# leggedrobotics/open3d_slam

Hardware: NVIDIA H100
Metric: scan-to-map ICP registrations/sec (64x1024-pt clouds) (higher is better)
Workload: dtype f64

## Files before the change

### include/b2s.h

```cpp
#ifndef B2S_H_
#define B2S_H_

#include <stddef.h>
#include <stdint.h>

#ifdef __cplusplus
extern "C" {
#endif
#if defined(__GNUC__)
#pragma GCC visibility push(default)
#endif

#define B2S_OK 0
#define B2S_E_INVALID (-1)
#define B2S_E_CUDA (-2)
#define B2S_E_EMPTY (-3)
#define B2S_E_NO_NORMALS (-4)
#define B2S_E_CAPACITY (-5)
#define B2S_E_UNSUPPORTED (-6)

typedef struct b2s_handle b2s_handle;
typedef struct b2s_cloud b2s_cloud;
typedef struct b2s_submap b2s_submap;

// ... 15 lines not shown
  int32_t knn;
  double knn_radius;
  double rel_fitness, rel_rmse;
} b2s_icp_params;

typedef struct b2s_scan_params {
  double voxel_size;
  double downsampling_ratio;
  uint32_t seed;
  b2s_cropper map_builder_cropper;
  b2s_cropper scan_matcher_cropper;
} b2s_scan_params;

typedef struct b2s_config {
  b2s_icp_params icp;
  b2s_scan_params scan;
  double map_voxel_size;
  double dense_voxel_size;
  double nn_cell_size;
  int32_t icp_cluster_ctas;
  int32_t reserved_;
} b2s_config;

typedef struct b2s_result {
  double T[16];
  double fitness;
  double inlier_rmse;
  int32_t n_corr;
  int32_t iters;
} b2s_result;

void b2s_default_config(b2s_config* cfg);

int32_t b2s_create(const b2s_config* cfg, int32_t device, void* cuda_stream_or_null, b2s_handle** out);
void b2s_destroy(b2s_handle* h);
int32_t b2s_set_config(b2s_handle* h, const b2s_config* cfg);
int32_t b2s_synchronize(b2s_handle* h);
const char* b2s_last_error(void);
const char* b2s_version(void);
int32_t b2s_device_count(void);
int64_t b2s_launch_count(const b2s_handle* h);
int64_t b2s_graph_capture_count(const b2s_handle* h);

#define B2S_PROFILE_KINDS 8
int32_t b2s_profile_enable(b2s_handle* h, int32_t on);
int32_t b2s_profile_read(b2s_handle* h, double* ms_by_kind, int64_t* count_by_kind, int32_t n_kinds);
int32_t b2s_debug_icp_clocks(b2s_handle* h, int32_t enable, long long* out_1024);

int32_t b2s_cloud_create(b2s_handle* h, b2s_cloud** out);
void b2s_cloud_destroy(b2s_cloud* c);
int32_t b2s_cloud_upload_f64(b2s_handle* h, b2s_cloud* c, const double* xyz, const double* normals_or_null, size_t n);
int32_t b2s_cloud_upload_f32(b2s_handle* h, b2s_cloud* c, const void* xyz, size_t n, size_t stride_bytes);
int32_t b2s_cloud_size(b2s_handle* h, const b2s_cloud* c, size_t* n, int32_t* has_normals);
int32_t b2s_cloud_download(b2s_handle* h, const b2s_cloud* c, double* xyz, double* normals_or_null, size_t capacity, size_t* n);
int32_t b2s_cloud_copy(b2s_handle* h, const b2s_cloud* src, b2s_cloud* dst);

int32_t b2s_crop(b2s_handle* h, const b2s_cloud* in, const b2s_cropper* cropper, b2s_cloud* out);
int32_t b2s_voxel_down_sample(b2s_handle* h, const b2s_cloud* in, double voxel_size, b2s_cloud* out);
int32_t b2s_estimate_normals(b2s_handle* h, b2s_cloud* cloud, int32_t knn, double radius);
int32_t b2s_debug_estimate_normals(b2s_handle* h, b2s_cloud* cloud, int32_t knn, double radius, double cell_hint, const int32_t* flags_host,
                                   int32_t with_prior, double* rec_out, int32_t* path_out, double* sel_out);
int32_t b2s_random_down_sample(b2s_handle* h, const b2s_cloud* in, double ratio, uint32_t seed, b2s_cloud* out);
int32_t b2s_transform(b2s_handle* h, const b2s_cloud* in, const double T[16], b2s_cloud* out);
int32_t b2s_process_scan(b2s_handle* h, const b2s_cloud* raw, b2s_cloud* merge, b2s_cloud* match);
int32_t b2s_register(b2s_handle* h, const b2s_cloud* source, const b2s_cloud* target, const double init[16], b2s_result* out);
int32_t b2s_register_batch(b2s_handle* h, int32_t n, const b2s_cloud* const* sources, const b2s_cloud* const* targets,
                           const double* inits , b2s_result* out );
int32_t b2s_nearest_neighbors(b2s_handle* h, const b2s_cloud* queries, const b2s_cloud* target, double max_correspondence_distance,
                              const double T_or_null[16], int32_t* index_out, double* d2_out_or_null, size_t capacity, size_t* n_queries);
int32_t b2s_register_host(b2s_handle* h, const double* src_xyz, size_t n_src, const double* tgt_xyz, const double* tgt_normals,
                          size_t n_tgt, const double init[16], b2s_result* out);

int32_t b2s_submap_create(b2s_handle* h, size_t capacity_points, b2s_submap** out);
void b2s_submap_destroy(b2s_submap* sm);
int32_t b2s_submap_insert(b2s_handle* h, b2s_submap* sm, const b2s_cloud* preprocessed_scan, const double map_to_sensor[16]);
typedef struct b2s_carving_params {
  double voxel_size;
  double max_raytracing_length;
  double truncation_distance;
  double min_dot_product_with_normal;
  double neighborhood_radius_dense_map;
} b2s_carving_params;
int32_t b2s_submap_carve(b2s_handle* h, b2s_submap* sm, const b2s_cloud* raw_scan, const double map_to_sensor[16],
                         const double cropper_pose[16], const b2s_carving_params* params, size_t* n_removed);
int32_t b2s_undistort(b2s_handle* h, const b2s_cloud* in, const double linear_velocity[3], const double angular_velocity_rpy[3],
                      double scan_duration, int32_t is_spinning_clockwise, b2s_cloud* out);
int32_t b2s_overlap(b2s_handle* h, const b2s_cloud* source, const b2s_cloud* target, const double source_to_target[16], double voxel_size,
                    int32_t min_points_per_voxel, b2s_cloud* source_overlap, b2s_cloud* target_overlap);
int32_t b2s_information_matrix(b2s_handle* h, const b2s_cloud* source, const b2s_cloud* target, double max_correspondence_distance,
                               const double transformation[16], double info_out[36]);
int32_t b2s_dense_carve(b2s_handle* h, b2s_submap* sm, const b2s_cloud* scan, const double sensor_position[3],
                        const b2s_carving_params* params, size_t* n_removed);
int32_t b2s_submap_insert_dense(b2s_handle* h, b2s_submap* sm, const b2s_cloud* raw_scan, const double map_to_sensor[16],
                                const b2s_cropper* dense_cropper);
int32_t b2s_dense_query(b2s_handle* h, const b2s_submap* sm, const b2s_cloud* points, int32_t* counts, double* means_xyz, size_t capacity);
int32_t b2s_dense_remove(b2s_handle* h, b2s_submap* sm, const b2s_cloud* points);
int32_t b2s_dense_size(b2s_handle* h, const b2s_submap* sm, size_t* n_voxels);
int32_t b2s_dense_clear(b2s_handle* h, b2s_submap* sm);
int32_t b2s_submap_transform(b2s_handle* h, b2s_submap* sm, const double T[16]);
int32_t b2s_cloud_transform_inplace(b2s_handle* h, b2s_cloud* c, const double T[16]);
int32_t b2s_submap_size(b2s_handle* h, const b2s_submap* sm, size_t* n);
int32_t b2s_submap_download(b2s_handle* h, const b2s_submap* sm, double* xyz, double* normals, size_t capacity, size_t* n);
int32_t b2s_submap_to_cloud(b2s_handle* h, const b2s_submap* sm, b2s_cloud* out);
int32_t b2s_submap_dense_download(b2s_handle* h, const b2s_submap* sm, double* xyz, double* normals, int32_t* keys, size_t capacity,
                                  size_t* n);
int32_t b2s_submap_set_cloud(b2s_handle* h, b2s_submap* sm, const b2s_cloud* cloud);
int32_t b2s_register_to_submap(b2s_handle* h, const b2s_cloud* scan, const b2s_submap* sm, const double map_to_sensor[16],
                               const double init[16], b2s_result* out);

int32_t b2s_submap_set_pose(b2s_handle* h, b2s_submap* sm, const double map_to_sensor[16]);
int32_t b2s_submap_get_pose(b2s_handle* h, const b2s_submap* sm, double map_to_sensor[16]);
int32_t b2s_mapper_step_async(b2s_handle* h, b2s_submap* sm, const b2s_cloud* raw_scan, const double odometry_motion[16],
                              double min_refinement_fitness, int32_t ignore_min_fitness, int32_t slot );
int32_t b2s_scan_result_fetch(b2s_handle* h, int32_t slot, b2s_result* out);
int32_t b2s_mapper_step_host(b2s_handle* h, b2s_submap* sm, const void* xyz_f32, size_t n, size_t stride_bytes,
                             const double odometry_motion[16], double min_refinement_fitness, int32_t ignore_min_fitness,
                             b2s_result* out);
int32_t b2s_mapper_step_host_async(b2s_handle* h, b2s_submap* sm, const void* xyz_f32, size_t n, size_t stride_bytes,
                                   const double odometry_motion[16], double min_refinement_fitness, int32_t ignore_min_fitness,
                                   b2s_result* out_pinned);
int32_t b2s_mapper_graph_enable(b2s_handle* h, b2s_submap* sm, size_t raw_capacity_points, double min_refinement_fitness,
                                int32_t ignore_min_fitness, b2s_cloud** staging_out);

typedef struct b2s_mapper_options {
  double min_movement_between_mapping_steps;
  int32_t carve_enabled;
  int32_t carve_every_n_scans;
  b2s_carving_params carving;
  int32_t dense_enabled;
  int32_t dense_carve_every_n_scans;
  b2s_carving_params dense_carving;
  b2s_cropper dense_cropper;
} b2s_mapper_options;
void b2s_default_mapper_options(b2s_mapper_options* o);
int32_t b2s_submap_set_mapper_options(b2s_handle* h, b2s_submap* sm, const b2s_mapper_options* o);
typedef struct b2s_mapper_counters {
  int64_t steps;
  int64_t accepted;
  int64_t inserted_map;
  int64_t inserted_dense;
  int64_t carve_runs;
  int64_t carved_points_total;
  int64_t dense_carve_runs;
  int64_t carved_voxels_total;
} b2s_mapper_counters;
int32_t b2s_submap_get_mapper_counters(b2s_handle* h, const b2s_submap* sm, b2s_mapper_counters* out);

int32_t b2s_submap_set_initial_map(b2s_handle* h, b2s_submap* sm, const b2s_cloud* cloud, double map_voxel_size);
int32_t b2s_submap_set_initial_transform(b2s_handle* h, b2s_submap* sm, const double map_to_sensor[16]);
int32_t b2s_submap_set_merge_scans(b2s_handle* h, b2s_submap* sm, int32_t on);
int32_t b2s_debug_nn_index(b2s_handle* h, double origin_cell[4], int32_t dims_n[5], int32_t* cell_start, size_t cap_cells, int32_t* orig,
                           size_t cap_pts);
int32_t b2s_debug_submap_bbox(b2s_handle* h, const b2s_submap* sm, double box[6]);

typedef struct b2s_global_localization_params {
  double x_min, x_max, y_min, y_max;
  double step;
  double z0, z_step;
  int32_t n_z;
  int32_t n_yaw;
  double yaw0, yaw_step;
  double roll, pitch;
  double score_voxel;
  int32_t n_candidates;
  int32_t reserved_;
  double nms_distance, nms_yaw;
} b2s_global_localization_params;
void b2s_default_global_localization_params(b2s_global_localization_params* p);
typedef struct b2s_global_localization_candidate {
  double T_hypothesis[16];
  int32_t hypothesis;
  int32_t hits;
  b2s_result icp;
} b2s_global_localization_candidate;
typedef struct b2s_global_localization_result {
  double T[16];
  double fitness, inlier_rmse;
  double runner_up_fitness;
  int64_t n_hypotheses;
  int32_t found;
  int32_t winner_rank;
  int32_t n_query;
  int32_t n_candidates;
} b2s_global_localization_result;
int32_t b2s_submap_global_localization(b2s_handle* h, const b2s_submap* sm, const b2s_cloud* raw_scan, const b2s_global_localization_params* p,
                                       double min_refinement_fitness, b2s_global_localization_candidate* candidates_or_null, int32_t capacity,
                                       b2s_global_localization_result* out);
int32_t b2s_debug_global_localization_scores(b2s_handle* h, const b2s_submap* sm, const b2s_cloud* raw_scan, const b2s_global_localization_params* p,
                                             int32_t* hits_out, size_t capacity, size_t* n_hypotheses, double* query_out_or_null,
                                             size_t query_capacity, size_t* n_query);

int32_t b2s_submaps_global_localization(b2s_handle* h, const b2s_submap* const* sms, int32_t n_submaps, const double* centers,
                                        const b2s_cloud* raw_scan, const b2s_global_localization_params* p, double min_refinement_fitness,
                                        b2s_global_localization_candidate* candidates_or_null, int32_t capacity,
                                        int32_t* candidate_submaps_or_null, b2s_global_localization_result* out, int32_t* winner_submap);
int32_t b2s_debug_submaps_global_localization_scores(b2s_handle* h, const b2s_submap* const* sms, int32_t n_submaps, const b2s_cloud* raw_scan,
                                                     const b2s_global_localization_params* p, int32_t* hits_out, size_t capacity,
                                                     size_t* n_hypotheses, double* query_out_or_null, size_t query_capacity, size_t* n_query);

typedef struct b2s_odometry_params {
  b2s_icp_params icp;
  double voxel_size;
  double downsampling_ratio;
  uint32_t seed;
  b2s_cropper cropper;
  double min_fitness;
  int32_t buffer_size;
} b2s_odometry_params;
void b2s_default_odometry_params(b2s_odometry_params* p);
enum { B2S_ODOM_INIT = 0, B2S_ODOM_OK = 1, B2S_ODOM_FAILED = 2, B2S_ODOM_FAILED_KEPT_PREV = 3 };
typedef struct b2s_odometry b2s_odometry;
int32_t b2s_odometry_create(b2s_handle* h, const b2s_odometry_params* p, size_t capacity_points, b2s_odometry** out);
void b2s_odometry_destroy(b2s_odometry* od);
int32_t b2s_odometry_set_params(b2s_handle* h, b2s_odometry* od, const b2s_odometry_params* p);
int32_t b2s_odometry_set_initial_transform(b2s_handle* h, b2s_odometry* od, const double T[16]);
int32_t b2s_odometry_step_async(b2s_handle* h, b2s_odometry* od, const b2s_cloud* raw, int64_t t, int32_t slot);
typedef struct b2s_odometry_result {
  b2s_result registration;
  double odom_to_range_sensor[16];
  int32_t outcome;
  int32_t n_preprocessed;
} b2s_odometry_result;
int32_t b2s_odometry_result_fetch(b2s_handle* h, b2s_odometry* od, int32_t slot, b2s_odometry_result* out);
int32_t b2s_odometry_lookup(b2s_handle* h, const b2s_odometry* od, int64_t t, double T[16], int32_t* has);
int32_t b2s_odometry_preprocessed(b2s_handle* h, const b2s_odometry* od, b2s_cloud* out);

typedef struct b2s_slam_result {
  b2s_odometry_result odometry;
  b2s_result mapper;
  int32_t odom_used;
  int32_t mapper_accepted;
} b2s_slam_result;
int32_t b2s_slam_step_async(b2s_handle* h, b2s_submap* sm, b2s_odometry* od, const b2s_cloud* raw, int64_t t, double min_refinement_fitness,
                            int32_t ignore_min_fitness, int32_t slot);
int32_t b2s_slam_result_fetch(b2s_handle* h, b2s_odometry* od, int32_t slot, b2s_slam_result* out);
int32_t b2s_slam_step_host_async(b2s_handle* h, b2s_submap* sm, b2s_odometry* od, const void* xyz_f32, size_t n, size_t stride_bytes, int64_t t,
                                 double min_refinement_fitness, int32_t ignore_min_fitness, b2s_slam_result* out_pinned);
int32_t b2s_slam_graph_enable(b2s_handle* h, b2s_odometry* od, size_t raw_capacity_points, b2s_cloud** staging_out);

typedef struct b2s_motion_compensation_params {
  int32_t enabled;
  int32_t spinning_clockwise;
  double scan_duration;
  int32_t num_poses_velocity_estimation;
} b2s_motion_compensation_params;
void b2s_default_motion_compensation_params(b2s_motion_compensation_params* p);
int32_t b2s_odometry_set_motion_compensation(b2s_handle* h, b2s_odometry* od, const b2s_motion_compensation_params* p);
int32_t b2s_slam_map_pose_push(b2s_handle* h, b2s_odometry* od, int64_t t, const double T[16]);
int32_t b2s_slam_map_lookup(b2s_handle* h, const b2s_odometry* od, int64_t t, double T[16], int32_t* has);
typedef struct b2s_motion_compensation_result {
  double odometry_linear_velocity[3];
  double odometry_angular_velocity_rpy[3];
  double map_linear_velocity[3];
  double map_angular_velocity_rpy[3];
  int32_t odometry_applied;
  int32_t map_applied;
} b2s_motion_compensation_result;
int32_t b2s_slam_motion_fetch(b2s_handle* h, b2s_odometry* od, int32_t slot, b2s_motion_compensation_result* out);
int32_t b2s_slam_undistorted(b2s_handle* h, const b2s_odometry* od, b2s_cloud* odo_out, b2s_cloud* map_out);

#define B2S_VOXEL_MAP_LAYERS 4
typedef struct b2s_voxel_map b2s_voxel_map;
int32_t b2s_voxel_map_create(b2s_handle* h, const double voxel_size[3], size_t capacity_voxels, b2s_voxel_map** out);
void b2s_voxel_map_destroy(b2s_voxel_map* vm);
int32_t b2s_voxel_map_clear(b2s_handle* h, b2s_voxel_map* vm);
int32_t b2s_voxel_map_insert_cloud(b2s_handle* h, b2s_voxel_map* vm, int32_t layer, const b2s_cloud* cloud);
int32_t b2s_voxel_map_size(b2s_handle* h, const b2s_voxel_map* vm, size_t* n_voxels);
int32_t b2s_voxel_map_has_voxel(b2s_handle* h, const b2s_voxel_map* vm, const b2s_cloud* points, const double T_or_null[16],
                                int32_t* flags_or_null, size_t capacity, size_t* n_hits);
int32_t b2s_voxel_map_indices_in_voxel(b2s_handle* h, const b2s_voxel_map* vm, int32_t layer, const b2s_cloud* points, int32_t* offsets,
                                       size_t offsets_capacity, int32_t* indices, size_t indices_capacity, size_t* n_indices);
int32_t b2s_mapper_processed_scan(b2s_handle* h, b2s_cloud* merge_out, b2s_cloud* match_out);

#define B2S_FEATURE_DIM 33
#define B2S_FEATURE_MAX_KNN 128
typedef struct b2s_feature b2s_feature;
int32_t b2s_feature_create(b2s_handle* h, b2s_feature** out);
void b2s_feature_destroy(b2s_feature* f);
int32_t b2s_feature_size(b2s_handle* h, const b2s_feature* f, size_t* n);
int32_t b2s_feature_download(b2s_handle* h, const b2s_feature* f, double* data, size_t capacity_points, size_t* n);
int32_t b2s_feature_upload(b2s_handle* h, b2s_feature* f, const double* data, size_t n);
int32_t b2s_compute_fpfh(b2s_handle* h, const b2s_cloud* cloud, double radius, int32_t knn, b2s_feature* feature);

typedef struct b2s_feature_params {
  double feature_voxel_size;
  double normal_estimation_radius;
  int32_t normal_knn;
  double feature_radius;
  int32_t feature_knn;
} b2s_feature_params;
void b2s_default_feature_params(b2s_feature_params* p);
int32_t b2s_submap_compute_features(b2s_handle* h, b2s_submap* sm, const b2s_feature_params* params, b2s_cloud* sparse_out,
                                    b2s_feature* feature_out);

#define B2S_RANSAC_MAX_N 8
typedef struct b2s_ransac_params {
  int32_t mutual_filter;
  int32_t ransac_n;
  double max_correspondence_distance;
  double checker_distance;
  double checker_edge_length;
  int64_t max_iteration;
  double confidence;
  uint64_t seed;
} b2s_ransac_params;
void b2s_default_ransac_params(b2s_ransac_params* p);
// ... 183 lines not shown
```

### open3d_slam_b200/_lib.py

```python
from __future__ import annotations

import ctypes as C
import os

_HERE = os.path.dirname(os.path.abspath(__file__))
LIB_PATH = os.environ.get("B2S_LIB") or os.path.join(_HERE, "libb2s.so")

OK, E_INVALID, E_CUDA, E_EMPTY, E_NO_NORMALS, E_CAPACITY, E_UNSUPPORTED = 0, -1, -2, -3, -4, -5, -6
CROP_NONE, CROP_MAX_RADIUS, CROP_MIN_RADIUS, CROP_MINMAX_RADIUS, CROP_CYLINDER = 0, 1, 2, 3, 4
CROPPER_NAMES = {"None": 0, "MaxRadius": 1, "MinRadius": 2, "MinMaxRadius": 3, "Cylinder": 4}
REG_POINT_TO_PLANE, REG_POINT_TO_POINT, REG_GENERALIZED = 0, 1, 2


class Cropper(C.Structure):
    _fields_ = [("kind", C.c_int32), ("invert", C.c_int32), ("rmin", C.c_double), ("rmax", C.c_double),
                ("zmin", C.c_double), ("zmax", C.c_double), ("center", C.c_double * 3)]


class IcpParams(C.Structure):
    _fields_ = [("reg_type", C.c_int32), ("max_iter", C.c_int32), ("max_corr_dist", C.c_double), ("knn", C.c_int32),
                ("knn_radius", C.c_double), ("rel_fitness", C.c_double), ("rel_rmse", C.c_double)]


class ScanParams(C.Structure):
# ... 6 lines not shown
                ("nn_cell_size", C.c_double), ("icp_cluster_ctas", C.c_int32), ("reserved_", C.c_int32)]


class Result(C.Structure):
    _fields_ = [("T", C.c_double * 16), ("fitness", C.c_double), ("inlier_rmse", C.c_double), ("n_corr", C.c_int32),
                ("iters", C.c_int32)]


class CarvingParams(C.Structure):
    _fields_ = [("voxel_size", C.c_double), ("max_raytracing_length", C.c_double), ("truncation_distance", C.c_double),
                ("min_dot_product_with_normal", C.c_double), ("neighborhood_radius_dense_map", C.c_double)]


class MapperOptions(C.Structure):
    _fields_ = [("min_movement_between_mapping_steps", C.c_double), ("carve_enabled", C.c_int32), ("carve_every_n_scans", C.c_int32),
                ("carving", CarvingParams), ("dense_enabled", C.c_int32), ("dense_carve_every_n_scans", C.c_int32),
                ("dense_carving", CarvingParams), ("dense_cropper", Cropper)]


class FeatureParams(C.Structure):
    _fields_ = [("feature_voxel_size", C.c_double), ("normal_estimation_radius", C.c_double), ("normal_knn", C.c_int32),
                ("feature_radius", C.c_double), ("feature_knn", C.c_int32)]


class RansacParams(C.Structure):
    _fields_ = [("mutual_filter", C.c_int32), ("ransac_n", C.c_int32), ("max_correspondence_distance", C.c_double),
                ("checker_distance", C.c_double), ("checker_edge_length", C.c_double), ("max_iteration", C.c_int64),
                ("confidence", C.c_double), ("seed", C.c_uint64)]


class RansacResult(C.Structure):
    _fields_ = [("result", Result), ("hypotheses", C.c_int64), ("validations", C.c_int64), ("best_hypothesis", C.c_int64), ("n_feature_corr", C.c_int32),
                ("used_mutual", C.c_int32)]


class OdometryParams(C.Structure):
    _fields_ = [("icp", IcpParams), ("voxel_size", C.c_double), ("downsampling_ratio", C.c_double), ("seed", C.c_uint32), ("cropper", Cropper),
                ("min_fitness", C.c_double), ("buffer_size", C.c_int32)]


class OdometryResult(C.Structure):
    _fields_ = [("registration", Result), ("odom_to_range_sensor", C.c_double * 16), ("outcome", C.c_int32), ("n_preprocessed", C.c_int32)]


class SlamResult(C.Structure):
    _fields_ = [("odometry", OdometryResult), ("mapper", Result), ("odom_used", C.c_int32), ("mapper_accepted", C.c_int32)]


class MotionCompensationParams(C.Structure):
    _fields_ = [("enabled", C.c_int32), ("spinning_clockwise", C.c_int32), ("scan_duration", C.c_double),
                ("num_poses_velocity_estimation", C.c_int32)]


class MotionCompensationResult(C.Structure):
    _fields_ = [("odometry_linear_velocity", C.c_double * 3), ("odometry_angular_velocity_rpy", C.c_double * 3),
                ("map_linear_velocity", C.c_double * 3), ("map_angular_velocity_rpy", C.c_double * 3),
                ("odometry_applied", C.c_int32), ("map_applied", C.c_int32)]


ODOM_INIT, ODOM_OK, ODOM_FAILED, ODOM_FAILED_KEPT_PREV = 0, 1, 2, 3


class OdometryConstraintParams(C.Structure):
    _fields_ = [("map_voxel_size", C.c_double), ("voxel_if_zero", C.c_double), ("overlap_factor", C.c_double), ("icp_factor", C.c_double),
                ("min_points_per_voxel", C.c_int32), ("refine", C.c_int32), ("max_iter", C.c_int32), ("rel_fitness", C.c_double),
                ("rel_rmse", C.c_double)]


class OdometryConstraint(C.Structure):
    _fields_ = [("T", C.c_double * 16), ("information", C.c_double * 36), ("n_source_overlap", C.c_int64), ("n_target_overlap", C.c_int64),
                ("refined", C.c_int32), ("icp", Result)]


class LoopClosureRefinementParams(C.Structure):
    _fields_ = [("map_voxel_size", C.c_double), ("voxel_if_zero", C.c_double), ("overlap_factor", C.c_double), ("min_points_per_voxel", C.c_int32),
                ("max_iter", C.c_int32), ("max_corr_dist", C.c_double), ("rel_fitness", C.c_double), ("rel_rmse", C.c_double),
                ("min_refinement_fitness", C.c_double), ("reg_type", C.c_int32)]


class LoopClosureRefinement(C.Structure):
    _fields_ = [("icp", Result), ("information", C.c_double * 36), ("n_source_overlap", C.c_int64), ("n_target_overlap", C.c_int64),
                ("accepted", C.c_int32)]


class PoseGraphEdge(C.Structure):
    _fields_ = [("source", C.c_int32), ("target", C.c_int32), ("uncertain", C.c_int32), ("reserved_", C.c_int32), ("T", C.c_double * 16),
                ("information", C.c_double * 36)]


class GlobalOptimizationParams(C.Structure):
    _fields_ = [("max_correspondence_distance", C.c_double), ("edge_prune_threshold", C.c_double), ("preference_loop_closure", C.c_double),
                ("reference_node", C.c_int32), ("max_iteration", C.c_int32), ("min_relative_increment", C.c_double),
                ("min_relative_residual_increment", C.c_double), ("min_right_term", C.c_double), ("min_residual", C.c_double),
                ("max_iteration_lm", C.c_int32), ("reserved_", C.c_int32), ("upper_scale_factor", C.c_double), ("lower_scale_factor", C.c_double)]


class GlobalOptimizationStats(C.Structure):
    _fields_ = [("valid", C.c_int32), ("n_edges", C.c_int32), ("outer_iterations", C.c_int32), ("lm_tries", C.c_int32), ("accepted_steps", C.c_int32),
                ("stop_reason", C.c_int32), ("initial_residual", C.c_double), ("final_residual", C.c_double), ("final_lambda", C.c_double)]


LM_STOP_REASONS = ["none", "right_term", "relative_increment", "relative_residual_increment", "max_iteration_lm", "residual", "max_iteration"]


class MapperCounters(C.Structure):
    _fields_ = [(n, C.c_int64) for n in ("steps", "accepted", "inserted_map", "inserted_dense", "carve_runs", "carved_points_total",
                                         "dense_carve_runs", "carved_voxels_total")]


class GlobalLocalizationParams(C.Structure):
    _fields_ = [("x_min", C.c_double), ("x_max", C.c_double), ("y_min", C.c_double), ("y_max", C.c_double), ("step", C.c_double),
                ("z0", C.c_double), ("z_step", C.c_double), ("n_z", C.c_int32), ("n_yaw", C.c_int32), ("yaw0", C.c_double),
                ("yaw_step", C.c_double), ("roll", C.c_double), ("pitch", C.c_double), ("score_voxel", C.c_double),
                ("n_candidates", C.c_int32), ("reserved_", C.c_int32), ("nms_distance", C.c_double), ("nms_yaw", C.c_double)]


class GlobalLocalizationCandidate(C.Structure):
    _fields_ = [("T_hypothesis", C.c_double * 16), ("hypothesis", C.c_int32), ("hits", C.c_int32), ("icp", Result)]


class GlobalLocalizationResult(C.Structure):
    _fields_ = [("T", C.c_double * 16), ("fitness", C.c_double), ("inlier_rmse", C.c_double), ("runner_up_fitness", C.c_double),
                ("n_hypotheses", C.c_int64), ("found", C.c_int32), ("winner_rank", C.c_int32), ("n_query", C.c_int32),
                ("n_candidates", C.c_int32)]


SYMBOLS = [
    "b2s_default_config", "b2s_create", "b2s_destroy", "b2s_set_config", "b2s_synchronize", "b2s_last_error", "b2s_version",
    "b2s_device_count", "b2s_launch_count", "b2s_graph_capture_count", "b2s_cloud_create", "b2s_cloud_destroy", "b2s_cloud_upload_f64", "b2s_cloud_upload_f32",
    "b2s_cloud_size", "b2s_cloud_download", "b2s_cloud_copy", "b2s_crop", "b2s_voxel_down_sample", "b2s_estimate_normals",
    "b2s_random_down_sample", "b2s_transform", "b2s_process_scan", "b2s_register", "b2s_register_batch", "b2s_register_host",
    "b2s_submap_create", "b2s_submap_destroy", "b2s_submap_insert", "b2s_submap_insert_dense", "b2s_submap_size", "b2s_submap_download",
    "b2s_submap_dense_download", "b2s_submap_set_cloud", "b2s_register_to_submap", "b2s_submap_set_pose", "b2s_submap_get_pose",
    "b2s_mapper_step_async", "b2s_scan_result_fetch", "b2s_profile_enable", "b2s_profile_read", "b2s_mapper_graph_enable", "b2s_debug_icp_clocks",
    "b2s_mapper_step_host", "b2s_mapper_step_host_async", "b2s_submap_carve", "b2s_overlap", "b2s_information_matrix", "b2s_undistort",
    "b2s_dense_query", "b2s_dense_remove", "b2s_dense_size", "b2s_dense_clear", "b2s_dense_carve", "b2s_submap_transform",
    "b2s_default_mapper_options", "b2s_submap_set_mapper_options", "b2s_submap_get_mapper_counters",
    "b2s_voxel_map_create", "b2s_voxel_map_destroy", "b2s_voxel_map_clear", "b2s_voxel_map_insert_cloud", "b2s_voxel_map_size",
    "b2s_voxel_map_has_voxel", "b2s_voxel_map_indices_in_voxel", "b2s_mapper_processed_scan",
    "b2s_cloud_export_device", "b2s_cloud_import_device", "b2s_submap_to_cloud", "b2s_nearest_neighbors",
    "b2s_feature_create", "b2s_feature_destroy", "b2s_feature_size", "b2s_feature_download", "b2s_feature_upload", "b2s_compute_fpfh",
    "b2s_default_feature_params", "b2s_submap_compute_features",
    "b2s_default_ransac_params", "b2s_ransac_feature_matching", "b2s_feature_correspondences",
    "b2s_default_odometry_params", "b2s_odometry_create", "b2s_odometry_destroy", "b2s_odometry_set_params", "b2s_odometry_set_initial_transform",
    "b2s_odometry_step_async", "b2s_odometry_result_fetch", "b2s_odometry_lookup", "b2s_odometry_preprocessed",
    "b2s_slam_step_async", "b2s_slam_result_fetch", "b2s_slam_step_host_async", "b2s_slam_graph_enable",
    "b2s_default_motion_compensation_params", "b2s_odometry_set_motion_compensation", "b2s_slam_map_pose_push", "b2s_slam_map_lookup",
    "b2s_slam_motion_fetch", "b2s_slam_undistorted",
    "b2s_default_odometry_constraint_params", "b2s_submap_odometry_constraints",
    "b2s_default_loop_closure_refinement_params", "b2s_submap_loop_closure_refinement",
    "b2s_default_global_optimization_params", "b2s_global_optimization", "b2s_cloud_transform_inplace",
    "b2s_submap_set_initial_map", "b2s_submap_set_initial_transform", "b2s_submap_set_merge_scans", "b2s_debug_nn_index",
    "b2s_assemble_map", "b2s_assemble_colored_map", "b2s_debug_pose_graph_solve", "b2s_debug_pose_graph_linearize",
    "b2s_debug_estimate_normals", "b2s_debug_submap_bbox",
    "b2s_default_global_localization_params", "b2s_submap_global_localization", "b2s_debug_global_localization_scores",
    "b2s_submaps_global_localization", "b2s_debug_submaps_global_localization_scores",
    "b2s_assemble_dense_maps",
    "b2s_submaps_export_state", "b2s_submap_import_state", "b2s_odometry_export_state", "b2s_odometry_import_state",
]
FEATURE_DIM, FEATURE_MAX_KNN = 33, 128
ASSEMBLY_MAX_SUBMAPS = 65535
STATE_VERSION, STATE_BYTE_ORDER = 1, 0x0102030405060708
STATE_MAGIC_SUBMAP, STATE_MAGIC_ODOMETRY = 0x314D425553533242, 0x314D4F444F533242
STATE_HEADER_BYTES, STATE_MSTATE_WORDS, STATE_POSE_SLOTS = 256, 32, 8
STATE_W_MAGIC, STATE_W_VERSION, STATE_W_BYTE_ORDER, STATE_W_TOTAL_BYTES, STATE_W_MAP_VOXEL, STATE_W_N_SECTIONS, STATE_W_SECTIONS, STATE_W_PARAMS = \
    0, 1, 2, 3, 4, 5, 6, 20
STATE_SUBMAP_SECTIONS = ["pose", "options", "mstate", "bbox", "map_xyz", "map_normals", "vnext", "pstamp", "wflag", "dups", "wlist", "voxels",
                         "dense_used", "dense"]
STATE_SUBMAP_PARAMS = ["capacity", "vcap", "stage_cap", "dense_cap", "dense_voxel", "flags", "dn", "n_voxels", "n_dups", "n_wlist", "n_dense"]
STATE_ODOMETRY_SECTIONS = ["params", "motion", "state", "ring_times", "ring_poses", "map_times", "map_poses", "prev_xyz", "prev_normals"]
STATE_ODOMETRY_PARAMS = ["capacity", "buffer_size", "n_prev", "host_step", "has_t", "last_t"]
STATE_F_HAS_NORMALS, STATE_F_NO_NORMALS, STATE_F_MERGE_SCANS, STATE_F_DENSE_HAS_NORMALS = 1, 2, 4, 8


class StateVoxelRecord(C.Structure):
    _fields_ = [("key", C.c_uint64), ("slot", C.c_int32), ("head", C.c_int32), ("stamp", C.c_int32), ("reserved_", C.c_int32)]


class StateDenseRecord(C.Structure):
    _fields_ = [("key", C.c_uint64), ("sum", C.c_double * 6), ("slot", C.c_int32), ("count", C.c_int32)]
PROFILE_KINDS = ["icp", "normals", "radix_sort", "nn_grid_build", "voxel", "fuse", "select", "crop"]

_lib = None


class B2SError(RuntimeError):

    def __init__(self, code, msg):
        super().__init__(f"b2s error {code}: {msg}")
        self.code = code


def lib():
    global _lib
    if _lib is None:
        if not os.path.exists(LIB_PATH):
            raise ImportError(f"{LIB_PATH} is missing: build it with __graft_entry__.build() (nvcc, sm_90a). "
                              "There is no CPU fallback.")
        L = C.CDLL(LIB_PATH)
        L.b2s_last_error.restype = C.c_char_p
        L.b2s_version.restype = C.c_char_p
        L.b2s_launch_count.restype = C.c_int64
        L.b2s_launch_count.argtypes = [C.c_void_p]
        L.b2s_graph_capture_count.restype = C.c_int64
        L.b2s_graph_capture_count.argtypes = [C.c_void_p]
        L.b2s_destroy.restype = None
        L.b2s_cloud_destroy.restype = None
        L.b2s_submap_destroy.restype = None
        L.b2s_default_config.restype = None
        L.b2s_default_mapper_options.restype = None
        L.b2s_default_feature_params.restype = None
        L.b2s_default_ransac_params.restype = None
        L.b2s_destroy.argtypes = [C.c_void_p]
        L.b2s_cloud_destroy.argtypes = [C.c_void_p]
        L.b2s_submap_destroy.argtypes = [C.c_void_p]
        L.b2s_voxel_map_destroy.restype = None
        L.b2s_voxel_map_destroy.argtypes = [C.c_void_p]
        L.b2s_feature_destroy.restype = None
        L.b2s_feature_destroy.argtypes = [C.c_void_p]
        L.b2s_odometry_destroy.restype = None
        L.b2s_odometry_destroy.argtypes = [C.c_void_p]
        L.b2s_default_odometry_params.restype = None
        L.b2s_default_motion_compensation_params.restype = None
        L.b2s_default_odometry_constraint_params.restype = None
        L.b2s_default_loop_closure_refinement_params.restype = None
        L.b2s_default_global_optimization_params.restype = None
        L.b2s_default_global_localization_params.restype = None
        _lib = L
    return _lib


def check(code):
    if code != OK:
        raise B2SError(code, lib().b2s_last_error().decode("utf-8", "replace"))
```

### open3d_slam_b200/csrc/c_api.cu

```cuda
#include <math.h>
#include <stdlib.h>

#include "common.cuh"

using namespace b2s;

namespace b2s {
int32_t pose_to_device(b2s_handle* h, const double* T, double* dst);
int32_t dense_to_cloud(b2s_handle* h, b2s_submap* sm, double* d_xyz, int32_t* d_keys, int32_t* d_out_n);

__global__ void f32_to_f64_kernel(const unsigned char* __restrict__ src, size_t stride, int n, double* __restrict__ dst) {
  pdl_wait();
  for (int i = blockIdx.x * blockDim.x + threadIdx.x; i < n; i += gridDim.x * blockDim.x) {
    const float* p = reinterpret_cast<const float*>(src + (size_t)i * stride);
    dst[3 * i] = (double)p[0]; dst[3 * i + 1] = (double)p[1]; dst[3 * i + 2] = (double)p[2];
  }
}

__global__ void write_i32_kernel(int32_t* p, int32_t v) {
  pdl_wait(); *p = v; }

__global__ void empty_check_kernel(const int32_t* a, const int32_t* b, uint32_t* status) {
  pdl_wait();
  if (*a <= 0 || *b <= 0) atomicOr(status, ST_EMPTY);
}

__global__ void compose_kernel(const double* __restrict__ A, const double* __restrict__ B, double* __restrict__ C, const int32_t* __restrict__ ms) {
  pdl_wait();
  const int i = threadIdx.x >> 2, j = threadIdx.x & 3;
  const bool hold = ms[MS_NEWINIT] || ms[MS_IGNODOM];
  if (threadIdx.x < 16) {
    double s = 0.0;
    for (int k = 0; k < 4; k++) s += A[4 * i + k] * B[4 * k + j];
    C[4 * i + j] = hold ? A[4 * i + j] : s;
  }
}

struct GateArgs {
  double min_fitness, min_move;
  int ignore_fitness, carve_on, carve_n, dense_on, dcarve_n, merge_on;
};
__global__ void mapper_gate_kernel(const b2s_result* __restrict__ res, GateArgs a, double* pose, int32_t* ms, const int32_t* __restrict__ map_n,
                                   b2s_result* slots, const int32_t* __restrict__ gstate) {
  pdl_wait();
  if (threadIdx.x != 0) return;
  const int init = ms[MS_NEWINIT];
  ms[MS_NEWINIT] = 0; ms[MS_IGNODOM] = init; ms[MS_INITSTEP] = init;
  const bool accepted = init || a.ignore_fitness || !(res->fitness < a.min_fitness);
  if (accepted && !init) for (int i = 0; i < 16; i++) pose[i] = res->T[i];
  bool insert = accepted && !init && a.merge_on;
  if (insert && a.min_move > 0.0) {
    const double* L = pose + 5 * 16;
    const double* P = pose;
    double it[3], m[3];
    for (int i = 0; i < 3; i++) it[i] = -(L[i] * L[3] + L[4 + i] * L[7] + L[8 + i] * L[11]);
    for (int i = 0; i < 3; i++) m[i] = (L[i] * P[3] + L[4 + i] * P[7] + L[8 + i] * P[11]) + it[i];
    const double moved = sqrt(m[0] * m[0] + m[1] * m[1] + m[2] * m[2]);
    insert = !(moved < a.min_move);
  }
  const bool carve = insert && a.carve_on && a.carve_n > 0 && *map_n > 0 && (ms[MS_NINS] % a.carve_n == 1);
  const bool dense = accepted && a.dense_on;
  const bool dcarve = dense && a.dcarve_n > 0 && (ms[MS_NDENSE] % a.dcarve_n == 1);
  ms[MS_ACCEPT] = accepted; ms[MS_INSERT] = insert; ms[MS_CARVE] = carve; ms[MS_DENSE] = dense; ms[MS_DCARVE] = dcarve;
  ms[MS_NSTEPS] += 1; ms[MS_NACCEPT] += accepted ? 1 : 0;
  if (slots) slots[gstate[1]] = *res;
}
__global__ void mapper_post_kernel(int32_t* ms) {
  pdl_wait();
  if (threadIdx.x == 0 && ms[MS_DENSE]) ms[MS_NDENSE] += 1;
}

double nn_cell(const b2s_handle* h, double max_corr) {
  if (h->cfg.nn_cell_size > 0.0) return h->cfg.nn_cell_size;
  return max_corr * 0.25;
}

int32_t check_icp_params(const b2s_icp_params& p) {
  B2S_REQUIRE(p.reg_type == B2S_REG_POINT_TO_PLANE || p.reg_type == B2S_REG_POINT_TO_POINT || p.reg_type == B2S_REG_GENERALIZED,
              B2S_E_UNSUPPORTED, "unknown registration type %d", (int)p.reg_type);
  B2S_REQUIRE(p.max_corr_dist > 0.0, B2S_E_INVALID, "[RegistrationICP] Invalid max_correspondence_distance.");
  B2S_REQUIRE(p.max_iter >= 0, B2S_E_INVALID, "max_iter must be >= 0");
  return B2S_OK;
}

size_t icp_work_bytes(size_t n) { return (n + 1) * 24 + (n + 1) * 4 + 16; }

void fill_problem(IcpProblem* P, const b2s_icp_params& icp, const b2s_cloud* src, const GridIndex* g, const b2s_cloud* tgt, const double* init_host,
                  const double* init_dev, double* work, b2s_result* out_dev) {
  memset(P, 0, sizeof(*P));
  P->src_xyz = src->xyz.as<double>();
  P->src_n = src->dn.as<int32_t>();
  P->ghdr = g->hdr.as<GridHeader>();
  P->cell_start = grid_starts(g);
  P->tgt_pts = g->pts.as<double>();
  P->tgt_nrm = tgt->has_normals ? tgt->nrm.as<double>() : nullptr;
  P->work_xyz = work;
  P->work_prev = reinterpret_cast<int32_t*>(work + 3 * (src->n_max + 1));
  P->init_dev = init_dev;
  if (init_host) memcpy(P->init, init_host, 128);
  P->max_corr = icp.max_corr_dist;
  P->rel_fitness = icp.rel_fitness;
  P->rel_rmse = icp.rel_rmse;
  P->max_iter = icp.max_iter;
  P->src_n_max = (int32_t)src->n_max;
  P->estimator = icp.reg_type;
  P->src_nrm = src->has_normals ? src->nrm.as<double>() : nullptr;
  P->gicp_eps = 1e-3;
  P->out = out_dev;
}

int32_t preprocess_scan(b2s_handle* h, const b2s_cloud* raw, const b2s_cropper& cropper, double voxel_size, double ratio, uint32_t seed,
                        const b2s_icp_params& icp, b2s_cloud* t0, b2s_cloud* out) {
  b2s_cropper c0 = cropper;
  c0.center[0] = c0.center[1] = c0.center[2] = 0.0;
  CropDev wide = make_crop(&c0);
  const bool has_crop = c0.kind != B2S_CROP_NONE || c0.invert;
  if (voxel_size > 0.0) B2S_TRY(op_voxel_down_sample(h, raw, has_crop ? &wide : nullptr, voxel_size, t0));
  else if (has_crop) B2S_TRY(op_crop(h, raw, wide, t0));
  else B2S_TRY(op_voxel_down_sample(h, raw, nullptr, 0.0, t0));
  static const double cell_factor = getenv("B2S_NORMALS_CELL_FACTOR") ? atof(getenv("B2S_NORMALS_CELL_FACTOR")) : 4.0;
  const double cell_hint = voxel_size > 0.0 ? cell_factor * voxel_size : 0.0;
  if (ratio < 1.0) {
    B2S_REQUIRE(ratio >= 0.0, B2S_E_INVALID, "[RandomDownSample] sampling_ratio must be in [0, 1]");
    B2S_TRY(select_flags(h, t0, ratio, seed));
    B2S_TRY(op_estimate_normals(h, t0, icp.knn, icp.knn_radius, cell_hint, h->flags.as<int32_t>()));
    B2S_TRY(select_compact(h, t0, ratio, out));
  } else {
    B2S_TRY(op_estimate_normals(h, t0, icp.knn, icp.knn_radius, cell_hint));
    B2S_TRY(op_random_down_sample(h, t0, ratio, seed, out));
  }
  return B2S_OK;
}

int32_t process_scan_impl(b2s_handle* h, const b2s_cloud* raw, b2s_cloud* merge, b2s_cloud* match) {
  const b2s_scan_params& sp = h->cfg.scan;
  B2S_TRY(preprocess_scan(h, raw, sp.map_builder_cropper, sp.voxel_size, sp.downsampling_ratio, sp.seed, h->cfg.icp, h->t0.get(), merge));
  b2s_cropper c1 = sp.scan_matcher_cropper;
  c1.center[0] = c1.center[1] = c1.center[2] = 0.0;
  B2S_TRY(op_crop(h, merge, make_crop(&c1), match));
  launch_pdl(empty_check_kernel, 1, 1, 0, h->stream, merge->dn.as<int32_t>(), match->dn.as<int32_t>(), h->status.as<uint32_t>());
  h->launches++;
  return B2S_OK;
}

__global__ void graph_begin_kernel(const double* __restrict__ ring, int32_t* gstate, double* __restrict__ odom) {
  pdl_wait();
  const int step = gstate[0];
  if (threadIdx.x < 16) odom[threadIdx.x] = ring[(step & 63) * 16 + threadIdx.x];
  __syncthreads();
  if (threadIdx.x == 0) { gstate[0] = step + 1; gstate[1] = step & 255; }
}

int32_t mapper_chain_tail(b2s_handle* h, b2s_submap* sm, const b2s_cloud* raw_scan, const b2s_cloud* merge, const b2s_result* res,
                          double min_fitness, int ignore_fitness, b2s_result* slots, const int32_t* gstate) {
  const b2s_mapper_options& o = sm->opts;
  double* pose_state = sm->pose.as<double>();
  int32_t* ms = sm->mstate.as<int32_t>();
  GateArgs ga;
  ga.min_fitness = min_fitness; ga.min_move = o.min_movement_between_mapping_steps; ga.ignore_fitness = ignore_fitness;
  ga.carve_on = o.carve_enabled; ga.carve_n = o.carve_every_n_scans; ga.dense_on = o.dense_enabled; ga.dcarve_n = o.dense_carve_every_n_scans;
  ga.merge_on = sm->merge_scans ? 1 : 0;
  launch_pdl(mapper_gate_kernel, 1, 32, 0, h->stream, res, ga, pose_state, ms, sm->cloud[0]->dn.as<int32_t>(), slots, gstate);
  h->launches++;
  if (sm->merge_scans) {
    if (o.carve_enabled) {
      B2S_REQUIRE(o.carving.voxel_size > 0.0, B2S_E_INVALID, "carving voxel size must be > 0");
      CropDev crop = make_crop(&h->cfg.scan.map_builder_cropper, pose_state + 5 * 16);
      B2S_TRY(op_submap_carve(h, sm, raw_scan, pose_state, crop, o.carving, nullptr, ms + MS_CARVE));
    }
    B2S_TRY(op_submap_insert(h, sm, merge, pose_state, ms + MS_INSERT));
  }
  if (o.dense_enabled) {
    if (sm->dense_cap == 0) {
      B2S_REQUIRE(h->cfg.dense_voxel_size > 0.0, B2S_E_INVALID, "dense_voxel_size must be > 0");
      B2S_TRY(dense_init(h, sm, (size_t)1 << 22, h->cfg.dense_voxel_size));
    }
    B2S_TRY(op_dense_insert(h, sm, raw_scan, nullptr, pose_state, &o.dense_cropper, ms + MS_DENSE));
    if (o.dense_carve_every_n_scans > 0)
      B2S_TRY(op_dense_carve(h, sm, raw_scan, nullptr, pose_state, o.dense_carving.neighborhood_radius_dense_map, o.dense_carving.truncation_distance,
                             o.dense_carving.max_raytracing_length, ms + MS_TMP + 1, ms + MS_DCARVE));
    launch_pdl(mapper_post_kernel, 1, 32, 0, h->stream, ms);
    h->launches++;
  }
  return B2S_OK;
}

static int32_t mapper_chain_graphable(void* ctx) {
  b2s_submap* sm = static_cast<b2s_submap*>(ctx);
  b2s_handle* h = sm->h;
  double* pose_state = sm->pose.as<double>();
  double* odom = pose_state + 32;
  double* guess = pose_state + 48;
  int32_t* gstate = sm->gstate.as<int32_t>();
  b2s_result* res = h->results.as<b2s_result>();
  double* ring_dev = nullptr;
  B2S_CUDA(cudaHostGetDevicePointer(&ring_dev, sm->odom_ring.p, 0));
  launch_pdl(graph_begin_kernel, 1, 32, 0, h->stream, ring_dev, gstate, odom);
  h->launches++;
  B2S_TRY(process_scan_impl(h, sm->staging.get(), h->t1.get(), h->t2.get()));
  launch_pdl(compose_kernel, 1, 32, 0, h->stream, pose_state, odom, guess, static_cast<const int32_t*>(sm->mstate.as<int32_t>()));
  h->launches++;
  B2S_TRY(register_to_submap_async(h, h->t2.get(), sm, nullptr, pose_state, nullptr, guess, res));
  return mapper_chain_tail(h, sm, sm->staging.get(), h->t1.get(), res, sm->g_min_fitness, sm->g_ignore_fitness, h->slots.as<b2s_result>(), gstate);
}

static std::mutex g_live_mu;
static std::unordered_set<unsigned long long> g_live_submaps;
void submap_register(unsigned long long uid) { std::lock_guard<std::mutex> lk(g_live_mu); g_live_submaps.insert(uid); }
void submap_forget(unsigned long long uid) { std::lock_guard<std::mutex> lk(g_live_mu); g_live_submaps.erase(uid); }
bool submap_alive(unsigned long long uid) { std::lock_guard<std::mutex> lk(g_live_mu); return g_live_submaps.count(uid) != 0; }

int32_t graph_drop(b2s_handle* h, GraphCache* g) {
  if (!g->exec) return B2S_OK;
  B2S_CUDA(cudaStreamSynchronize(h->stream));
  cudaGraphExecDestroy(g->exec);
  g->exec = nullptr;
  g->warm = 1;
  return B2S_OK;
}

int32_t graph_step(b2s_handle* h, GraphCache* g, unsigned long long key, int32_t (*chain)(void*), void* ctx) {
  if (g->alloc_gen != __atomic_load_n(&g_alloc_generation, __ATOMIC_RELAXED) || g->cfg_gen != h->cfg_gen || g->key != key) B2S_TRY(graph_drop(h, g));
  if (g->exec) {
    B2S_CUDA(cudaGraphLaunch(g->exec, h->stream));
    h->launches += g->kernels;
    return B2S_OK;
  }
  if (g->warm > 0) {
    g->warm--;
    return chain(ctx);
  }
  const int64_t l0 = h->launches;
  g_capturing = true; g_capture_broken = false;
  cudaError_t ce = cudaStreamBeginCapture(h->stream, cudaStreamCaptureModeThreadLocal);
  int32_t rc = B2S_E_CUDA;
  cudaGraph_t graph = nullptr;
  if (ce == cudaSuccess) {
    rc = chain(ctx);
    ce = cudaStreamEndCapture(h->stream, &graph);
  }
  g_capturing = false;
  const int64_t captured_kernels = h->launches - l0;
  h->launches = l0;
  if (ce != cudaSuccess || rc != B2S_OK || g_capture_broken || !graph) {
    if (graph) cudaGraphDestroy(graph);
    cudaGetLastError();
    g->warm = 1 << 30;
    return chain(ctx);
  }
  ce = cudaGraphInstantiate(&g->exec, graph, 0);
  cudaGraphDestroy(graph);
  if (ce != cudaSuccess) { g->exec = nullptr; g->warm = 1 << 30; cudaGetLastError(); return chain(ctx); }
  g->kernels = captured_kernels;
  h->captures++;
  g->alloc_gen = __atomic_load_n(&g_alloc_generation, __ATOMIC_RELAXED);
  g->cfg_gen = h->cfg_gen;
  g->key = key;
  B2S_CUDA(cudaGraphLaunch(g->exec, h->stream));
  h->launches += g->kernels;
  return B2S_OK;
}

static int32_t mapper_step_graph(b2s_handle* h, b2s_submap* sm, const b2s_cloud* raw_scan, const double* odometry_motion, int32_t slot) {
  B2S_REQUIRE(raw_scan == sm->staging.get(), B2S_E_INVALID, "graph mode: the scan must be uploaded into the staging cloud of b2s_mapper_graph_enable");
  B2S_REQUIRE(slot == (int32_t)(sm->host_step & 255), B2S_E_INVALID, "graph mode: slot must be (step count %% 256) = %d", (int)(sm->host_step & 255));
  B2S_TRY(h->results.ensure(sizeof(b2s_result), h->stream));
  if ((sm->host_step & 31) == 0) B2S_CUDA(cudaStreamSynchronize(h->stream));
  memcpy(sm->odom_ring.as<double>() + (sm->host_step & 63) * 16, odometry_motion, 128);
  sm->host_step++;
  return graph_step(h, &sm->graph, 0, mapper_chain_graphable, sm);
}

static int32_t make_cloud(b2s_handle* h, size_t capacity, bool normals, bool fixed, bool tracked, b2s_cloud** out) {
  return create_object(out, [&](b2s_cloud* c) -> int32_t {
    c->h = h;
    c->device = h->device;
    c->xyz.tracked = c->nrm.tracked = c->dn.tracked = tracked;
    if (fixed) c->fixed_cap = capacity;
    B2S_TRY(cloud_reserve(h, c, capacity, normals));
    return cloud_set_count(h, c, 0);
  });
// ... 977 lines not shown
    B2S_REQUIRE(nts[k] == tgt_fs[k]->n, B2S_E_INVALID, "target %d: the feature has %zu points, its cloud %zu", k, tgt_fs[k]->n, nts[k]);
  }
  if (n == 0) return B2S_OK;
  B2S_TRY(op_ransac(h, src, ns, src_f, n, tgts, nts.data(), tgt_fs, *p, out));
  return check_status(h);
}

int32_t b2s_feature_correspondences(b2s_handle* h, const b2s_feature* src_f, const b2s_feature* tgt_f, int32_t* s2t, size_t s_cap, int32_t* t2s,
                                    size_t t_cap) {
  B2S_REQUIRE(h && src_f && tgt_f && (s2t || src_f->n == 0) && (t2s || tgt_f->n == 0), B2S_E_INVALID, "null argument");
  B2S_REQUIRE(src_f->h == h && tgt_f->h == h, B2S_E_INVALID, "the feature belongs to another handle");
  B2S_REQUIRE(src_f->n <= s_cap && tgt_f->n <= t_cap, B2S_E_CAPACITY, "output arrays hold %zu / %zu entries, the features have %zu / %zu points",
              s_cap, t_cap, src_f->n, tgt_f->n);
  LOCK(h);
  B2S_TRY(h->tmp_i32.ensure((src_f->n + tgt_f->n + 1) * 4, h->stream));
  int32_t* d_s2t = h->tmp_i32.as<int32_t>();
  int32_t* d_t2s = d_s2t + src_f->n;
  B2S_TRY(op_feature_correspondences(h, src_f, 1, &tgt_f, &d_s2t, &d_t2s));
  if (src_f->n) B2S_CUDA(cudaMemcpyAsync(s2t, d_s2t, src_f->n * 4, cudaMemcpyDeviceToHost, h->stream));
  if (tgt_f->n) B2S_CUDA(cudaMemcpyAsync(t2s, d_t2s, tgt_f->n * 4, cudaMemcpyDeviceToHost, h->stream));
  return check_status(h);
}

void b2s_default_odometry_constraint_params(b2s_odometry_constraint_params* p) {
  memset(p, 0, sizeof(*p));
  p->map_voxel_size = 0.1; p->voxel_if_zero = 0.04; p->overlap_factor = 20.0; p->icp_factor = 1.5; p->min_points_per_voxel = 1;
  p->refine = 0; p->max_iter = 100; p->rel_fitness = 1e-6; p->rel_rmse = 1e-6;
}

int32_t b2s_submap_odometry_constraints(b2s_handle* h, int32_t n, const b2s_submap* const* sources, const b2s_submap* const* targets,
                                        const b2s_odometry_constraint_params* p, b2s_cloud* const* so, b2s_cloud* const* to,
                                        b2s_odometry_constraint* out) {
  B2S_REQUIRE(h && p && n >= 0, B2S_E_INVALID, "bad argument");
  if (n == 0) return B2S_OK;
  B2S_REQUIRE(sources && targets && out, B2S_E_INVALID, "null argument");
  const double voxel = fabs(p->map_voxel_size) <= 1e-3 ? p->voxel_if_zero : p->map_voxel_size;
  B2S_REQUIRE(voxel > 0.0, B2S_E_INVALID, "map voxel size %g after getMapVoxelSize: must be > 0", voxel);
  B2S_REQUIRE(p->overlap_factor > 0.0 && p->icp_factor > 0.0, B2S_E_INVALID, "overlap_factor and icp_factor must be > 0");
  B2S_REQUIRE(p->min_points_per_voxel >= 1, B2S_E_INVALID, "minNumPointsPerVoxel must be >= 1");
  B2S_REQUIRE(p->max_iter >= 0, B2S_E_INVALID, "max_iter must be >= 0");
  for (int32_t k = 0; k < n; k++) {
    B2S_REQUIRE(sources[k] && targets[k], B2S_E_INVALID, "null submap in pair %d", k);
    B2S_REQUIRE(sources[k]->h == h && targets[k]->h == h, B2S_E_INVALID, "pair %d: a submap belongs to another handle", k);
    for (b2s_cloud* const* c : {so, to})
      if (c) {
        B2S_REQUIRE(c[k] && c[k]->h == h, B2S_E_INVALID, "pair %d: an overlap cloud is null or belongs to another handle", k);
        B2S_REQUIRE(!c[k]->fixed_cap, B2S_E_INVALID, "pair %d: an overlap cloud must not be a fixed-capacity staging cloud", k);
      }
    B2S_REQUIRE(!so || !to || so[k] != to[k], B2S_E_INVALID, "pair %d: the two overlap clouds are the same object", k);
  }
  for (int32_t k = 0; k < n; k++)
    B2S_REQUIRE(!p->refine || !targets[k]->no_normals, B2S_E_NO_NORMALS,
                "[RegistrationICP] pair %d: TransformationEstimationPointToPlane requires target normals, the child map has none", k);
  LOCK(h);
  return op_odometry_constraints(h, n, sources, targets, *p, voxel, so, to, out);
}

void b2s_default_loop_closure_refinement_params(b2s_loop_closure_refinement_params* p) {
  memset(p, 0, sizeof(*p));
  p->map_voxel_size = 0.1; p->voxel_if_zero = 0.04; p->overlap_factor = 20.0; p->min_points_per_voxel = 1; p->max_iter = 100;
  p->max_corr_dist = 0.3; p->rel_fitness = 1e-6; p->rel_rmse = 1e-6; p->min_refinement_fitness = 0.7;
  p->reg_type = B2S_REG_POINT_TO_PLANE;
}

int32_t b2s_submap_loop_closure_refinement(b2s_handle* h, const b2s_submap* source, int32_t n, const b2s_submap* const* targets, const double* inits,
                                           const b2s_loop_closure_refinement_params* p, b2s_cloud* const* so, b2s_cloud* const* to,
                                           b2s_loop_closure_refinement* out) {
  B2S_REQUIRE(h && source && p && n >= 0, B2S_E_INVALID, "bad argument");
  B2S_REQUIRE(source->h == h, B2S_E_INVALID, "the source submap belongs to another handle");
  if (n == 0) return B2S_OK;
  B2S_REQUIRE(targets && inits && out, B2S_E_INVALID, "null argument");
  const double voxel = fabs(p->map_voxel_size) <= 1e-3 ? p->voxel_if_zero : p->map_voxel_size;
  B2S_REQUIRE(voxel > 0.0, B2S_E_INVALID, "map voxel size %g after getMapVoxelSize: must be > 0", voxel);
  B2S_REQUIRE(p->overlap_factor > 0.0, B2S_E_INVALID, "overlap_factor must be > 0");
  B2S_REQUIRE(p->max_corr_dist > 0.0, B2S_E_INVALID, "[RegistrationICP] Invalid max_correspondence_distance.");
  B2S_REQUIRE(p->min_points_per_voxel >= 1, B2S_E_INVALID, "minNumPointsPerVoxel must be >= 1");
  B2S_REQUIRE(p->max_iter >= 0, B2S_E_INVALID, "max_iter must be >= 0");
  for (int32_t k = 0; k < n; k++) {
    B2S_REQUIRE(targets[k], B2S_E_INVALID, "null target submap %d", k);
    B2S_REQUIRE(targets[k]->h == h, B2S_E_INVALID, "target %d belongs to another handle", k);
    for (b2s_cloud* const* c : {so, to})
      if (c) {
        B2S_REQUIRE(c[k] && c[k]->h == h, B2S_E_INVALID, "target %d: an overlap cloud is null or belongs to another handle", k);
        B2S_REQUIRE(!c[k]->fixed_cap, B2S_E_INVALID, "target %d: an overlap cloud must not be a fixed-capacity staging cloud", k);
      }
    B2S_REQUIRE(!so || !to || so[k] != to[k], B2S_E_INVALID, "target %d: the two overlap clouds are the same object", k);
  }
  B2S_REQUIRE(p->reg_type == B2S_REG_POINT_TO_PLANE || p->reg_type == B2S_REG_POINT_TO_POINT || p->reg_type == B2S_REG_GENERALIZED,
              B2S_E_UNSUPPORTED, "unknown registration type %d", (int)p->reg_type);
  B2S_REQUIRE(p->reg_type != B2S_REG_GENERALIZED || !source->no_normals, B2S_E_NO_NORMALS,
              "GeneralizedIcp on the device derives the covariances from normals: the source map has none");
  for (int32_t k = 0; k < n; k++)
    B2S_REQUIRE(p->reg_type == B2S_REG_POINT_TO_POINT || !targets[k]->no_normals, B2S_E_NO_NORMALS,
                "[RegistrationICP] target %d: the %s estimator requires target normals, the map has none", k,
                p->reg_type == B2S_REG_GENERALIZED ? "GeneralizedIcp" : "TransformationEstimationPointToPlane");
  LOCK(h);
  return op_loop_closure_refinement(h, source, n, targets, inits, *p, voxel, so, to, out);
}

void b2s_default_global_optimization_params(b2s_global_optimization_params* p) {
  memset(p, 0, sizeof(*p));
  p->max_correspondence_distance = 1000.0; p->edge_prune_threshold = 0.2; p->preference_loop_closure = 2.0; p->reference_node = 0;
  p->max_iteration = 100; p->min_relative_increment = 1e-6; p->min_relative_residual_increment = 1e-6; p->min_right_term = 1e-6;
  p->min_residual = 1e-6; p->max_iteration_lm = 20; p->upper_scale_factor = 2.0 / 3.0; p->lower_scale_factor = 1.0 / 3.0;
}

int32_t b2s_global_optimization(b2s_handle* h, int32_t n_nodes, double* node_poses, int32_t n_edges, const b2s_pose_graph_edge* edges,
                                const b2s_global_optimization_params* p, int32_t* edge_kept_out, double* edge_confidence_out,
                                b2s_global_optimization_stats* stats_out) {
  B2S_REQUIRE(h && p && node_poses, B2S_E_INVALID, "null argument");
  B2S_REQUIRE(n_nodes >= 1 && n_edges >= 0, B2S_E_INVALID, "n_nodes %d must be >= 1 and n_edges %d >= 0", (int)n_nodes, (int)n_edges);
  B2S_REQUIRE(n_edges == 0 || edges, B2S_E_INVALID, "null edges");
  B2S_REQUIRE(p->min_relative_increment > 0.0 && p->min_relative_residual_increment > 0.0 && p->min_right_term > 0.0 && p->min_residual > 0.0,
              B2S_E_INVALID, "the convergence tolerances must be > 0");
  B2S_REQUIRE(p->max_iteration >= 1 && p->max_iteration_lm >= 1, B2S_E_INVALID, "max_iteration and max_iteration_lm must be >= 1");
  for (int32_t e = 0; e < n_edges; e++)
    B2S_REQUIRE(edges[e].source >= 0 && edges[e].source < n_nodes && edges[e].target >= 0 && edges[e].target < n_nodes, B2S_E_INVALID,
                "edge %d: node ids (%d, %d) outside [0, %d)", (int)e, (int)edges[e].source, (int)edges[e].target, (int)n_nodes);
  LOCK(h);
  return op_global_optimization(h, n_nodes, node_poses, n_edges, edges, *p, edge_kept_out, edge_confidence_out, stats_out);
}

int32_t b2s_debug_pose_graph_solve(b2s_handle* h, int32_t n_nodes, const double* A, const double* b, double lambda, double* delta_out,
                                   double* d_out, double* L_out) {
  B2S_REQUIRE(h && A && b && delta_out, B2S_E_INVALID, "null argument");
  B2S_REQUIRE(n_nodes >= 1, B2S_E_INVALID, "n_nodes %d must be >= 1", (int)n_nodes);
  LOCK(h);
  return op_debug_pose_graph_solve(h, n_nodes, A, b, lambda, delta_out, d_out, L_out);
}

int32_t b2s_debug_pose_graph_linearize(b2s_handle* h, int32_t n_nodes, const double* poses, int32_t n_edges, const b2s_pose_graph_edge* edges,
                                       const b2s_global_optimization_params* p, const double* conf_in, double* conf_out, double* H_out,
                                       double* b_out, double rec_out[4]) {
  B2S_REQUIRE(h && poses && p && H_out && b_out && rec_out, B2S_E_INVALID, "null argument");
  B2S_REQUIRE(n_nodes >= 1 && n_edges >= 0, B2S_E_INVALID, "n_nodes %d must be >= 1 and n_edges %d >= 0", (int)n_nodes, (int)n_edges);
  B2S_REQUIRE(n_edges == 0 || (edges && conf_in && conf_out), B2S_E_INVALID, "null edges or confidences");
  for (int32_t e = 0; e < n_edges; e++)
    B2S_REQUIRE(edges[e].source >= 0 && edges[e].source < n_nodes && edges[e].target >= 0 && edges[e].target < n_nodes, B2S_E_INVALID,
                "edge %d: node ids (%d, %d) outside [0, %d)", (int)e, (int)edges[e].source, (int)edges[e].target, (int)n_nodes);
  LOCK(h);
  return op_debug_pose_graph_linearize(h, n_nodes, poses, n_edges, edges, *p, conf_in, conf_out, H_out, b_out, rec_out);
}

int32_t b2s_debug_submap_bbox(b2s_handle* h, const b2s_submap* sm, double box[6]) {
  B2S_REQUIRE(h && sm && box, B2S_E_INVALID, "null argument");
  B2S_REQUIRE(sm->h == h, B2S_E_INVALID, "the submap belongs to another handle");
  LOCK(h);
  unsigned long long w[6];
  const int32_t rc = read_back(h, {{w, sm->bbox.p, sizeof(w)}});
  for (int d = 0; d < 6; d++) box[d] = ord_decode(w[d]);
  return rc;
}

static int32_t check_assembly_args(b2s_handle* h, int32_t n, const b2s_submap* const* submaps, const b2s_cloud* out) {
  B2S_REQUIRE(h && out, B2S_E_INVALID, "null argument");
  B2S_REQUIRE(n >= 0, B2S_E_INVALID, "n_submaps must be >= 0");
  B2S_REQUIRE(n == 0 || submaps, B2S_E_INVALID, "null submap array");
  B2S_REQUIRE(out->h == h, B2S_E_INVALID, "the output cloud belongs to another handle");
  B2S_REQUIRE(!out->fixed_cap, B2S_E_INVALID, "the output cloud must not be a fixed-capacity staging cloud");
  for (int32_t k = 0; k < n; k++) {
    B2S_REQUIRE(submaps[k], B2S_E_INVALID, "null submap %d", k);
    B2S_REQUIRE(submaps[k]->h == h, B2S_E_INVALID, "submap %d belongs to another handle", k);
  }
  B2S_REQUIRE(n <= B2S_ASSEMBLY_MAX_SUBMAPS, B2S_E_UNSUPPORTED, "%d submaps: one assembly takes at most %d", n, B2S_ASSEMBLY_MAX_SUBMAPS);
  return B2S_OK;
}

int32_t b2s_assemble_map(b2s_handle* h, int32_t n, const b2s_submap* const* submaps, double voxel_size, b2s_cloud* out) {
  B2S_TRY(check_assembly_args(h, n, submaps, out));
  LOCK(h);
  return op_assemble_map(h, n, submaps, voxel_size, out, false, nullptr, 0, nullptr);
}

int32_t b2s_assemble_colored_map(b2s_handle* h, int32_t n, const b2s_submap* const* submaps, double voxel_size, b2s_cloud* out, double* rgb,
                                 size_t capacity, size_t* n_out) {
  B2S_TRY(check_assembly_args(h, n, submaps, out));
  LOCK(h);
  return op_assemble_map(h, n, submaps, voxel_size, out, true, rgb, capacity, n_out);
}

int32_t b2s_assemble_dense_maps(b2s_handle* h, int32_t n, const b2s_submap* const* submaps, b2s_cloud* out, int64_t* offsets) {
  B2S_TRY(check_assembly_args(h, n, submaps, out));
  LOCK(h);
  return op_assemble_dense_maps(h, n, submaps, out, offsets);
}

int32_t b2s_debug_nn_index(b2s_handle* h, double origin_cell[4], int32_t dims_n[5], int32_t* cell_start, size_t cap_cells, int32_t* orig,
                           size_t cap_pts) {
  B2S_REQUIRE(h && origin_cell && dims_n, B2S_E_INVALID, "null argument");
  LOCK(h);
  B2S_REQUIRE(h->grid_a.hdr.p, B2S_E_INVALID, "no NN index has been built yet");
  GridHeader gh;
  B2S_TRY(read_back(h, {{&gh, h->grid_a.hdr.p, sizeof(gh)}}));
  for (int d = 0; d < 3; d++) { origin_cell[d] = gh.origin[d]; dims_n[d] = gh.dims[d]; }
  origin_cell[3] = gh.cell; dims_n[3] = gh.ncell; dims_n[4] = gh.n;
  if (cell_start && cap_cells >= (size_t)gh.ncell + 1)
    B2S_CUDA(cudaMemcpy(cell_start, grid_starts(&h->grid_a), ((size_t)gh.ncell + 1) * 4, cudaMemcpyDeviceToHost));
  if (orig && cap_pts >= (size_t)gh.n && gh.n > 0) {
    std::vector<double> p4((size_t)gh.n * 4);
    B2S_CUDA(cudaMemcpy(p4.data(), h->grid_a.pts.p, p4.size() * 8, cudaMemcpyDeviceToHost));
    for (int32_t k = 0; k < gh.n; k++) { long long v; memcpy(&v, &p4[4 * (size_t)k + 3], 8); orig[k] = (int32_t)v; }
  }
  return B2S_OK;
}

}
```

### open3d_slam_b200/csrc/common.cuh

```cuda
#pragma once
#include <cuda_runtime.h>
#include <stdint.h>
#include <stdio.h>
#include <string.h>
#include <memory>
#include <mutex>
#include <unordered_set>
#include <new>
#include <string>
#include <utility>
#include <vector>

#include "../../include/b2s.h"

namespace b2s {

void set_error(const char* fmt, ...);
const char* get_error();

#define B2S_CUDA(expr)                                                                            \
  do {                                                                                            \
    cudaError_t _e = (expr);                                                                      \
    if (_e != cudaSuccess) {                                                                      \
      ::b2s::set_error("CUDA error %s at %s:%d: %s", cudaGetErrorName(_e), __FILE__, __LINE__, cudaGetErrorString(_e)); \
// ... 186 lines not shown
  DevBuf tables;
  DevBuf slots;
  DevBuf labels;
  DevBuf rgb;
  PinnedBuf stage;
  b2s_cloud cloud;
  VoxelScratch vox;
  DevBuf blob;
  AssemblyScratch() {
    for (DevBuf* b : {&tables, &slots, &labels, &rgb, &cloud.xyz, &cloud.nrm, &cloud.dn, &blob}) b->tracked = false;
  }
};
}

struct b2s_feature {
  b2s_handle* h = nullptr;
  int device = 0;
  b2s::DevBuf data;
  size_t n = 0;
  b2s::DevBuf nb_idx, nb_d2, nb_cnt, spfh;
};

namespace b2s {
enum MapperStateWord {
  MS_ACCEPT = 0,
  MS_INSERT = 1,
  MS_CARVE = 2,
  MS_DENSE = 3,
  MS_DCARVE = 4,
  MS_NINS = 5,
  MS_NDENSE = 6,
  MS_NSTEPS = 7, MS_NACCEPT = 8, MS_NCARVE = 9, MS_CARVED = 10, MS_NDCARVE = 11, MS_DCARVED = 12,
  MS_CARVE_N = 13,
  MS_TMP = 14,
  MS_NDEAD = 16,
  MS_STAMP = 17,
  MS_NTOUCHED = 18,
  MS_DUPSEL = 19,
  MS_NDUP = 20,
  MS_VUSED = 22,
  MS_TICKET2 = 23,
  MS_WSEL = 24,
  MS_NW = 25,
  MS_NEWINIT = 27,
  MS_IGNODOM = 28,
  MS_INITSTEP = 29,
  MS_WORDS = 32
};
extern unsigned long long g_alloc_generation;
enum ProfKind { PK_ICP = 0, PK_NORMALS, PK_SORT, PK_GRID, PK_VOXEL, PK_FUSE, PK_SELECT, PK_CROP, PK_COUNT };
struct ProfRec { int kind; cudaEvent_t a, b; };
}

namespace b2s {
extern thread_local bool g_capturing;
extern thread_local bool g_capture_broken;
}

struct b2s_handle {
  ~b2s_handle() {
    for (auto& r : prof_recs) { cudaEventDestroy(r.a); cudaEventDestroy(r.b); }
    for (cudaEvent_t e : prof_pool) cudaEventDestroy(e);
    if (own_stream && stream) cudaStreamDestroy(stream);
  }
  bool prof_enabled = false;
  b2s::DevBuf icp_dbg;
  std::vector<b2s::ProfRec> prof_recs;
  std::vector<cudaEvent_t> prof_pool;
  int device = 0;
  cudaStream_t stream = nullptr;
  bool own_stream = false;
  std::recursive_mutex mu;
  b2s_config cfg;
  unsigned long long cfg_gen = 1;
  int64_t launches = 0;
  int64_t captures = 0;

  b2s::DevBuf status;
  b2s::ScanScratch scan;
  b2s::SortScratch sort;
  b2s::GridIndex grid_a, grid_b;
  b2s::DevBuf keys, vals, flags, offs, tmp_i32, tmp_f64, misc, work_xyz;
  b2s::DevBuf problems;
  b2s::DevBuf results;
  b2s::DevBuf slots;
  b2s::DevBuf poses;
  b2s::PinnedBuf pinned;
  std::unique_ptr<b2s_cloud> t0, t1, t2, t3;
  std::vector<std::unique_ptr<b2s::GridIndex>> batch_grids;
  b2s::DevBuf batch_jobs;
  std::vector<unsigned char> batch_jobs_host;
  b2s::DevBuf lc;
  b2s::DevBuf odo, odo_info;
  b2s::PinnedBuf odo_stage;
  std::vector<std::unique_ptr<b2s_cloud>> odo_clouds;
  b2s::DevBuf pg_A, pg_F, pg_W, pg_vec, pg_nodes, pg_edges;
  int32_t pg_edge_cap = 0;
  b2s::GraphCache pg_graph;
  b2s::AssemblyScratch assembly;
};

#define LOCK(h) std::lock_guard<std::recursive_mutex> _lk((h)->mu); cudaSetDevice((h)->device)

namespace b2s {

enum StatusWord : int { SW_REMOVED = 8, SW_DENSE_SIZE = 12, SW_NN_CHUNK = 14 };
enum PoseSlot : int { PS_VOXEL_MAP = 61, PS_CALL = 62, PS_TRANSFORM = 63 };

struct ProfScope {
  b2s_handle* h; int idx;
  ProfScope(b2s_handle* h_, int kind);
  ~ProfScope();
};
int32_t check_status(b2s_handle* h);
struct ReadBack { void* dst; const void* src; size_t bytes; };
int32_t read_back(b2s_handle* h, std::initializer_list<ReadBack> copies);

struct Layout {
  unsigned char* base = nullptr;
  size_t size = 0;
  size_t off(size_t bytes) { const size_t o = size; size += (bytes + 255) & ~(size_t)255; return o; }
  template <typename T>
  T* take(size_t count) { const size_t o = off(count * sizeof(T)); return base ? reinterpret_cast<T*>(base + o) : nullptr; }
};
template <typename F>
int32_t carve(DevBuf& buf, cudaStream_t s, F&& place) {
  Layout L;
  place(L);
  B2S_TRY(buf.ensure(L.size, s));
  L = Layout{buf.as<unsigned char>()};
  place(L);
  return B2S_OK;
}

int32_t scan_exclusive_i32(b2s_handle* h, const int32_t* in, int32_t* out, const int32_t* d_n, size_t n_max, int32_t* d_total,
                           DevBuf* state = nullptr);
void scan_bind_state(Layout& L, ScanJob& j, size_t n_max);
int32_t scan_exclusive_i32_batch(b2s_handle* h, const ScanJob* jobs_dev, int njobs, size_t n_max);
int32_t radix_sort_pairs_u32(b2s_handle* h, uint32_t*& keys, uint32_t*& vals, uint32_t*& keys_alt, uint32_t*& vals_alt,
                             const int32_t* d_n, size_t n_max, int key_bits, VoxelScratch* own = nullptr);
int32_t radix_sort_pairs_u64(b2s_handle* h, uint64_t*& keys, uint32_t*& vals, uint64_t*& keys_alt, uint32_t*& vals_alt,
                             const int32_t* d_n, size_t n_max, int key_bits, VoxelScratch* own = nullptr);
inline const int32_t* grid_starts(const GridIndex* g) { return g->cell_start.as<int32_t>() + g->cap_cells + 4; }

struct CropDev {
  int32_t kind, invert;
  double rmin, rmax, zmin, zmax;
  double cx, cy, cz;
  const double* pose_dev;
};
CropDev make_crop(const b2s_cropper* c, const double* pose_dev = nullptr);
int32_t grid_build(b2s_handle* h, GridIndex* g, const b2s_cloud* cloud, double cell, const CropDev* patch, const int32_t* orig = nullptr,
                   const unsigned long long* map_box = nullptr, const CropDev* map_crop = nullptr);
int32_t box_reset(b2s_handle* h, unsigned long long* box);
bool tile_patch_usable(const b2s_submap* sm, const CropDev& crop);
int32_t tile_patch_build(b2s_handle* h, b2s_submap* sm, const CropDev& crop, double cell, GridIndex* g);
int32_t tile_drop(b2s_handle* h, b2s_submap* sm);
constexpr double TILE_EDGE = 2.0;
constexpr int TILE_MARGIN = 1;
int32_t grid_build_batch(b2s_handle* h, GridIndex* const* g, const b2s_cloud* const* clouds, int n, double cell);

int32_t pose_to_device(b2s_handle* h, const double* T, double* dst);
int32_t cloud_reserve(b2s_handle* h, b2s_cloud* c, size_t n, bool normals);
int32_t cloud_set_count(b2s_handle* h, b2s_cloud* c, size_t n);

int32_t op_crop(b2s_handle* h, const b2s_cloud* in, const CropDev& crop, b2s_cloud* out);
int32_t op_voxel_down_sample(b2s_handle* h, const b2s_cloud* in, const CropDev* crop, double voxel, b2s_cloud* out, int fixed_key_bits = 0,
                             VoxelScratch* own = nullptr, const int32_t* labels = nullptr, const double* palette = nullptr,
                             double* rgb_out = nullptr);
int voxel_key_bits(double extent, double voxel);
int32_t bbox_reduce(b2s_handle* h, const double* xyz, const int32_t* d_n, size_t n_max, const CropDev* crop, unsigned long long* bbox);
int32_t op_assemble_map(b2s_handle* h, int n, const b2s_submap* const* submaps, double voxel, b2s_cloud* out, bool colored, double* rgb,
                        size_t capacity, size_t* n_out);
int32_t op_assemble_dense_maps(b2s_handle* h, int n, const b2s_submap* const* submaps, b2s_cloud* out, int64_t* offsets);
struct NormalsDebug { double* rec; int32_t* path; double* sel; };
int32_t op_estimate_normals(b2s_handle* h, b2s_cloud* c, int knn, double radius, double cell_hint, const int32_t* flags = nullptr,
                            bool with_prior = false, const NormalsDebug* dbg = nullptr);
int32_t select_flags(b2s_handle* h, const b2s_cloud* in, double ratio, uint32_t seed);
int32_t select_compact(b2s_handle* h, const b2s_cloud* in, double ratio, b2s_cloud* out);
int32_t op_random_down_sample(b2s_handle* h, const b2s_cloud* in, double ratio, uint32_t seed, b2s_cloud* out);
int32_t op_transform(b2s_handle* h, const b2s_cloud* in, const double* T_host, b2s_cloud* out);

struct IcpProblem {
  const double* src_xyz;
  const int32_t* src_n;
  const GridHeader* ghdr;
  const int32_t* cell_start;
  const double* tgt_pts;
  const double* tgt_nrm;
  double* work_xyz;
  int32_t* work_prev;
  const double* init_dev;
  double init[16];
  double max_corr;
  double rel_fitness, rel_rmse;
  int32_t max_iter;
  int32_t src_n_max;
  int32_t estimator;
  int32_t pad;
  b2s_result* out;
  double* info_out;
  const double* src_nrm;
  double gicp_eps;
  int32_t* corr_index;
  double* corr_d2;
};
constexpr int EST_INFORMATION = 3;
constexpr int EST_CORRESPONDENCES = 4;
int32_t icp_launch(b2s_handle* h, const IcpProblem* single_host, const IcpProblem* problems_dev, int n_problems, size_t max_src_points,
                   int batch_estimator = -1);

int32_t op_submap_insert(b2s_handle* h, b2s_submap* sm, const b2s_cloud* scan, const double* T_dev, const int32_t* gate_dev);
constexpr int FUSE_STAGE_BASE = 1 << 30;
constexpr int FUSE_DUP_CAP = 1 << 16;
int32_t fuse_reserve(b2s_handle* h, b2s_submap* sm);
int32_t fuse_rehash(b2s_handle* h, b2s_submap* sm, const int32_t* enable_dev = nullptr);
int32_t dense_init(b2s_handle* h, b2s_submap* sm, size_t cap, double voxel);
size_t fuse_table_slots(const b2s_submap* sm);
int32_t submap_init(b2s_handle* h, b2s_submap* sm, size_t capacity);
int32_t submap_compact_view(b2s_handle* h, b2s_submap* sm, b2s_cloud** view);
int32_t op_dense_query(b2s_handle* h, const b2s_submap* sm, const b2s_cloud* pts, int32_t* count_dev, double* mean_dev);
int32_t op_dense_remove(b2s_handle* h, b2s_submap* sm, const b2s_cloud* pts);
int32_t op_dense_count(b2s_handle* h, const b2s_submap* sm, int32_t* out_dev);
int32_t op_dense_carve(b2s_handle* h, b2s_submap* sm, const b2s_cloud* scan, const double* sensor, const double* sensor_dev, double radius,
                       double trunc, double max_len, int32_t* removed_dev, const int32_t* enable_dev = nullptr);
int32_t op_submap_transform(b2s_handle* h, b2s_submap* sm, const double* T_host);
int32_t op_cloud_transform(b2s_handle* h, b2s_cloud* c, const double* T_host);
int32_t op_undistort(b2s_handle* h, const b2s_cloud* in, const double* lin_vel, const double* ang_vel_rpy, double scan_duration, int clockwise,
                     b2s_cloud* out);
int32_t op_overlap(b2s_handle* h, const b2s_cloud* source, const b2s_cloud* target, const double* T_dev, double voxel, int min_pts,
                   b2s_cloud* source_overlap, b2s_cloud* target_overlap);
struct OverlapTables { size_t jobs, scan, T, end; };
OverlapTables overlap_tables(Layout& stage, int n);
int32_t op_overlap_batch(b2s_handle* h, int n, const b2s_submap* const* maps, const double* inits, double voxel, int min_pts,
                         b2s_cloud* const* outs, unsigned char* stage, const OverlapTables& tb);
int32_t op_odometry_constraints(b2s_handle* h, int n, const b2s_submap* const* sources, const b2s_submap* const* targets,
                                const b2s_odometry_constraint_params& p, double voxel, b2s_cloud* const* so_out, b2s_cloud* const* to_out,
                                b2s_odometry_constraint* out);
int32_t op_loop_closure_refinement(b2s_handle* h, const b2s_submap* source, int n, const b2s_submap* const* targets, const double* inits,
                                   const b2s_loop_closure_refinement_params& p, double voxel, b2s_cloud* const* so_out, b2s_cloud* const* to_out,
                                   b2s_loop_closure_refinement* out);
int32_t op_global_optimization(b2s_handle* h, int n_nodes, double* poses, int n_edges, const b2s_pose_graph_edge* edges,
                               const b2s_global_optimization_params& p, int32_t* kept_out, double* conf_out, b2s_global_optimization_stats* stats);
int32_t op_debug_pose_graph_solve(b2s_handle* h, int n_nodes, const double* A, const double* b, double lambda, double* delta_out, double* d_out,
                                  double* L_out);
int32_t op_debug_pose_graph_linearize(b2s_handle* h, int n_nodes, const double* poses, int n_edges, const b2s_pose_graph_edge* edges,
                                      const b2s_global_optimization_params& p, const double* conf_in, double* conf_out, double* H_out,
                                      double* b_out, double* rec_out);
int32_t op_compute_fpfh(b2s_handle* h, const b2s_cloud* c, size_t n, double radius, int knn, b2s_feature* f);
int32_t op_feature_correspondences(b2s_handle* h, const b2s_feature* src, int n, const b2s_feature* const* tgts, int32_t* const* s2t,
                                   int32_t* const* t2s);
int32_t op_ransac(b2s_handle* h, const b2s_cloud* src, size_t ns, const b2s_feature* src_f, int n, const b2s_cloud* const* tgts, const size_t* nts,
                  const b2s_feature* const* tgt_fs, const b2s_ransac_params& p, b2s_ransac_result* out);
int32_t op_submap_carve(b2s_handle* h, b2s_submap* sm, const b2s_cloud* raw_scan, const double* T_dev, const CropDev& crop,
                        const b2s_carving_params& prm, int32_t* removed_dev, const int32_t* enable_dev = nullptr);
int32_t op_dense_insert(b2s_handle* h, b2s_submap* sm, const b2s_cloud* raw, const double* T_host, const double* T_dev, const b2s_cropper* crop,
                        const int32_t* enable_dev = nullptr);

int32_t check_icp_params(const b2s_icp_params& p);
double nn_cell(const b2s_handle* h, double max_corr);
size_t icp_work_bytes(size_t n);
void fill_problem(IcpProblem* P, const b2s_icp_params& icp, const b2s_cloud* src, const GridIndex* g, const b2s_cloud* tgt, const double* init_host,
                  const double* init_dev, double* work, b2s_result* out_dev);
int32_t preprocess_scan(b2s_handle* h, const b2s_cloud* raw, const b2s_cropper& cropper, double voxel_size, double ratio, uint32_t seed,
                        const b2s_icp_params& icp, b2s_cloud* scratch, b2s_cloud* out);
int32_t process_scan_impl(b2s_handle* h, const b2s_cloud* raw, b2s_cloud* merge, b2s_cloud* match);
int32_t register_to_submap_async(b2s_handle* h, const b2s_cloud* scan, const b2s_submap* sm, const double* sensor_pose_host,
                                 const double* sensor_pose_dev, const double* init_host, const double* init_dev, b2s_result* out_dev);
int32_t mapper_chain_tail(b2s_handle* h, b2s_submap* sm, const b2s_cloud* raw_scan, const b2s_cloud* merge, const b2s_result* res,
                          double min_fitness, int ignore_fitness, b2s_result* slots, const int32_t* gstate);
int32_t make_cloud(b2s_handle* h, size_t capacity, bool normals, bool fixed, std::unique_ptr<b2s_cloud>* out);
int32_t graph_step(b2s_handle* h, GraphCache* g, unsigned long long key, int32_t (*chain)(void*), void* ctx);
int32_t graph_drop(b2s_handle* h, GraphCache* g);

int device_sms();
int grid_cap();
struct WideGridScope {
  explicit WideGridScope(size_t n);
  ~WideGridScope();
  bool on;
};
inline int grid_for(size_t n, int threads, int max_blocks = 0) {
  if (max_blocks <= 0) max_blocks = grid_cap();
  size_t b = (n + (size_t)threads - 1) / (size_t)threads;
  if (b < 1) b = 1;
  if (b > (size_t)max_blocks) b = (size_t)max_blocks;
  return (int)b;
}

bool pdl_enabled();
struct PdlScope {
  PdlScope();
  ~PdlScope();
};

#ifdef __CUDACC__
template <typename... KArgs, typename... Args>
inline void launch_pdl(void (*kernel)(KArgs...), dim3 grid, dim3 block, size_t smem, cudaStream_t stream, Args&&... args) {
  cudaLaunchConfig_t cfg;
  memset(&cfg, 0, sizeof(cfg));
  cfg.gridDim = grid; cfg.blockDim = block; cfg.dynamicSmemBytes = smem; cfg.stream = stream;
  cudaLaunchAttribute attr[1];
  attr[0].id = cudaLaunchAttributeProgrammaticStreamSerialization;
  attr[0].val.programmaticStreamSerializationAllowed = 1;
  cfg.attrs = attr;
  cfg.numAttrs = pdl_enabled() ? 1 : 0;
  (void)cudaLaunchKernelEx(&cfg, kernel, KArgs(static_cast<Args&&>(args))...);
}
#endif

}

#ifdef __CUDACC__
namespace b2s {

__device__ __forceinline__ void pdl_wait() { asm volatile("griddepcontrol.wait;" ::: "memory"); }

__host__ __device__ inline unsigned long long ord_encode(double v) {
  unsigned long long u;
#ifdef __CUDA_ARCH__
  u = (unsigned long long)__double_as_longlong(v);
#else
  memcpy(&u, &v, 8);
#endif
  return (u & 0x8000000000000000ull) ? ~u : (u | 0x8000000000000000ull);
}
__host__ __device__ inline double ord_decode(unsigned long long u) {
  u = (u & 0x8000000000000000ull) ? (u & 0x7FFFFFFFFFFFFFFFull) : ~u;
#ifdef __CUDA_ARCH__
  return __longlong_as_double((long long)u);
// ... 392 lines not shown
```

### open3d_slam_b200/csrc/grid_index.cu

```cuda
#include <stdlib.h>

#include "common.cuh"

namespace b2s {

constexpr int GB_THREADS = 256;

__global__ void grid_bbox_init_kernel(unsigned long long* bbox) {
  pdl_wait();
  int t = threadIdx.x;
  if (t < 3) bbox[t] = ord_encode(INFINITY);
  else if (t < 6) bbox[t] = ord_encode(-INFINITY);
}

__device__ __forceinline__ void grid_bbox_body(const double* __restrict__ xyz, const int32_t* __restrict__ d_n, const CropDev& crop,
                                               int use_crop, unsigned long long* bbox) {
  const int n = *d_n;
  double mn[3] = {INFINITY, INFINITY, INFINITY}, mx[3] = {-INFINITY, -INFINITY, -INFINITY};
  for (int i = blockIdx.x * blockDim.x + threadIdx.x; i < n; i += gridDim.x * blockDim.x) {
    double x = xyz[3 * i], y = xyz[3 * i + 1], z = xyz[3 * i + 2];
    if (use_crop && !crop_within(crop, x, y, z)) continue;
    if (!(x == x && y == y && z == z)) continue;
    mn[0] = fmin(mn[0], x); mn[1] = fmin(mn[1], y); mn[2] = fmin(mn[2], z);
    mx[0] = fmax(mx[0], x); mx[1] = fmax(mx[1], y); mx[2] = fmax(mx[2], z);
// ... 26 lines not shown
  hdr->inv_cell = 1.0 / cell;
  hdr->ncell = dims[0] * dims[1] * dims[2];
  hdr->n = 0;
}

__device__ void grid_header_body(const unsigned long long* bbox, double cell, int cap_cells, GridHeader* hdr) {
  double mn[3], mx[3];
  for (int d = 0; d < 3; d++) { mn[d] = ord_decode(bbox[d]); mx[d] = ord_decode(bbox[3 + d]); }
  grid_header_of(mn, mx, cell, cap_cells, hdr);
}

__global__ void grid_header_kernel(const unsigned long long* bbox, double cell, int cap_cells, GridHeader* hdr) {
  pdl_wait();
  if (threadIdx.x != 0 || blockIdx.x != 0) return;
  grid_header_body(bbox, cell, cap_cells, hdr);
}

__device__ __forceinline__ bool crop_aabb(const CropDev& crop, double* lo, double* hi) {
  double c[3] = {crop.cx, crop.cy, crop.cz};
  if (crop.pose_dev) { c[0] = crop.pose_dev[3]; c[1] = crop.pose_dev[7]; c[2] = crop.pose_dev[11]; }
  for (int d = 0; d < 3; d++) { lo[d] = c[d] - crop.rmax; hi[d] = c[d] + crop.rmax; }
  if (crop.kind == B2S_CROP_CYLINDER) { lo[2] = crop.zmin; hi[2] = crop.zmax; }
  return !crop.invert && (crop.kind == B2S_CROP_MAX_RADIUS || crop.kind == B2S_CROP_MINMAX_RADIUS || crop.kind == B2S_CROP_CYLINDER);
}

__device__ __forceinline__ int grid_cell_of(const GridHeader& g, double x, double y, double z) {
  return (grid_axis_cell(z, g.origin[2], g.inv_cell, g.dims[2]) * g.dims[1] + grid_axis_cell(y, g.origin[1], g.inv_cell, g.dims[1])) * g.dims[0] +
         grid_axis_cell(x, g.origin[0], g.inv_cell, g.dims[0]);
}

__global__ void grid_zero_kernel(const GridHeader* hdr, int32_t* counts) {
  pdl_wait();
  const int nc = hdr->ncell + 1;
  for (int i = blockIdx.x * blockDim.x + threadIdx.x; i < nc; i += gridDim.x * blockDim.x) counts[i] = 0;
}

__device__ __forceinline__ void grid_count_body(const double* __restrict__ xyz, const int32_t* __restrict__ d_n, const CropDev& crop,
                                                int use_crop, const GridHeader* __restrict__ hdr, int32_t* counts,
                                                int32_t* __restrict__ rank) {
  const int n = *d_n;
  __shared__ GridHeader g;
  if (threadIdx.x == 0) g = *hdr;
  __syncthreads();
  for (int i = blockIdx.x * blockDim.x + threadIdx.x; i < n; i += gridDim.x * blockDim.x) {
    double x = xyz[3 * i], y = xyz[3 * i + 1], z = xyz[3 * i + 2];
    int r = -1;
    if ((x == x && y == y && z == z) && (!use_crop || crop_within(crop, x, y, z))) r = atomicAdd(&counts[grid_cell_of(g, x, y, z)], 1);
    rank[i] = r;
  }
}

__global__ void __launch_bounds__(GB_THREADS) grid_count_kernel(const double* __restrict__ xyz, const int32_t* __restrict__ d_n,
                                                                CropDev crop, int use_crop, const GridHeader* __restrict__ hdr,
                                                                int32_t* counts, int32_t* __restrict__ rank) {
  pdl_wait();
  grid_count_body(xyz, d_n, crop, use_crop, hdr, counts, rank);
}

__device__ __forceinline__ void grid_scatter_body(const double* __restrict__ xyz, const int32_t* __restrict__ d_n, GridHeader* hdr,
                                                  const int32_t* __restrict__ cell_start, const int32_t* __restrict__ rank,
                                                  double4* __restrict__ pts, const int32_t* __restrict__ orig) {
  const int n = *d_n;
  __shared__ GridHeader g;
  if (threadIdx.x == 0) g = *hdr;
  __syncthreads();
  if (blockIdx.x == 0 && threadIdx.x == 0) hdr->n = cell_start[g.ncell];
  for (int i = blockIdx.x * blockDim.x + threadIdx.x; i < n; i += gridDim.x * blockDim.x) {
    int r = rank[i];
    if (r < 0) continue;
    double x = xyz[3 * i], y = xyz[3 * i + 1], z = xyz[3 * i + 2];
    int slot = cell_start[grid_cell_of(g, x, y, z)] + r;
    pts[slot] = make_double4(x, y, z, __longlong_as_double((long long)(orig ? orig[i] : i)));
  }
}

__global__ void __launch_bounds__(GB_THREADS) grid_scatter_kernel(const double* __restrict__ xyz, const int32_t* __restrict__ d_n,
                                                                  GridHeader* hdr, const int32_t* __restrict__ cell_start,
                                                                  const int32_t* __restrict__ rank, double4* __restrict__ pts,
                                                                  const int32_t* __restrict__ orig) {
  pdl_wait();
  grid_scatter_body(xyz, d_n, hdr, cell_start, rank, pts, orig);
}

__global__ void grid_header_box_kernel(const unsigned long long* __restrict__ map_box, CropDev crop, double cell, int cap_cells, GridHeader* hdr) {
  pdl_wait();
  if (threadIdx.x != 0 || blockIdx.x != 0) return;
  double mn[3], mx[3], lo[3], hi[3];
  for (int d = 0; d < 3; d++) { mn[d] = ord_decode(map_box[d]); mx[d] = ord_decode(map_box[3 + d]); }
  if (crop_aabb(crop, lo, hi))
    for (int d = 0; d < 3; d++) { mn[d] = fmax(mn[d], lo[d]); mx[d] = fmin(mx[d], hi[d]); }
  grid_header_of(mn, mx, cell, cap_cells, hdr);
}

struct GridJob {
  const double* xyz; const int32_t* d_n;
  unsigned long long* bbox; GridHeader* hdr; int32_t* counts; int32_t* starts; int32_t* rank; double4* pts;
  int32_t cap_cells; int32_t pad;
};

__global__ void gridb_init_kernel(const GridJob* __restrict__ jobs, int njobs) {
  pdl_wait();
  const int j = blockIdx.x * blockDim.x + threadIdx.x;
  if (j >= njobs * 6) return;
  const int t = j % 6;
  jobs[j / 6].bbox[t] = t < 3 ? ord_encode(INFINITY) : ord_encode(-INFINITY);
}
__global__ void __launch_bounds__(GB_THREADS) gridb_bbox_kernel(const GridJob* __restrict__ jobs) {
  pdl_wait();
  const GridJob j = jobs[blockIdx.y];
  CropDev none; none.kind = 0; none.invert = 0; none.pose_dev = nullptr;
  grid_bbox_body(j.xyz, j.d_n, none, 0, j.bbox);
}
__global__ void gridb_header_kernel(const GridJob* __restrict__ jobs, int njobs, double cell) {
  pdl_wait();
  const int j = blockIdx.x * blockDim.x + threadIdx.x;
  if (j < njobs) grid_header_body(jobs[j].bbox, cell, jobs[j].cap_cells, jobs[j].hdr);
}
__global__ void gridb_zero_kernel(const GridJob* __restrict__ jobs) {
  pdl_wait();
  const GridJob j = jobs[blockIdx.y];
  const int nc = j.hdr->ncell + 1;
  for (int i = blockIdx.x * blockDim.x + threadIdx.x; i < nc; i += gridDim.x * blockDim.x) j.counts[i] = 0;
}
__global__ void __launch_bounds__(GB_THREADS) gridb_count_kernel(const GridJob* __restrict__ jobs) {
  pdl_wait();
  const GridJob j = jobs[blockIdx.y];
  CropDev none; none.kind = 0; none.invert = 0; none.pose_dev = nullptr;
  grid_count_body(j.xyz, j.d_n, none, 0, j.hdr, j.counts, j.rank);
}
__global__ void __launch_bounds__(GB_THREADS) gridb_scatter_kernel(const GridJob* __restrict__ jobs) {
  pdl_wait();
  const GridJob j = jobs[blockIdx.y];
  grid_scatter_body(j.xyz, j.d_n, j.hdr, j.starts, j.rank, j.pts, nullptr);
}

int32_t box_reset(b2s_handle* h, unsigned long long* box) {
  launch_pdl(grid_bbox_init_kernel, 1, 32, 0, h->stream, box);
  h->launches++;
  B2S_CUDA(cudaGetLastError());
  return B2S_OK;
}

CropDev make_crop(const b2s_cropper* c, const double* pose_dev) {
  CropDev d;
  memset(&d, 0, sizeof(d));
  if (c) {
    d.kind = c->kind; d.invert = c->invert; d.rmin = c->rmin; d.rmax = c->rmax; d.zmin = c->zmin; d.zmax = c->zmax;
    d.cx = c->center[0]; d.cy = c->center[1]; d.cz = c->center[2];
  }
  d.pose_dev = pose_dev;
  return d;
}

int32_t grid_build(b2s_handle* h, GridIndex* g, const b2s_cloud* cloud, double cell, const CropDev* patch, const int32_t* orig,
                   const unsigned long long* map_box, const CropDev* map_crop) {
  B2S_REQUIRE(cell > 0.0, B2S_E_INVALID, "grid_build: cell size must be > 0");
  static const bool bbox_pass = getenv("B2S_GRID_BBOX_PASS") && atoi(getenv("B2S_GRID_BBOX_PASS")) != 0;
  const bool from_box = map_box && map_crop && !bbox_pass;
  const size_t n_max = cloud->n_max > 0 ? cloud->n_max : 1;
  size_t n_alloc = cloud->xyz.cap / 24;
  if (n_alloc < n_max) n_alloc = n_max;
  size_t want = n_alloc * 8 + 4096;
  if (want > (size_t)1 << 21) want = (size_t)1 << 21;
  if (want < (size_t)1 << 16) want = (size_t)1 << 16;
  if ((size_t)g->cap_cells < want) {
    B2S_TRY(g->cell_start.ensure((want + 8) * 4 * 2, h->stream));
    g->cap_cells = (int32_t)want;
  }
  B2S_TRY(g->hdr.ensure(sizeof(GridHeader), h->stream));
  B2S_TRY(g->bbox.ensure(64, h->stream));
  B2S_TRY(g->rank.ensure(n_alloc * 4, h->stream));
  B2S_TRY(g->pts.ensure(n_alloc * 32, h->stream));
  CropDev cd = patch ? *patch : make_crop(nullptr);
  const int use_crop = patch ? 1 : 0;
  const int blocks = grid_for(n_max, GB_THREADS);
  int32_t* counts = g->cell_start.as<int32_t>();
  int32_t* starts = counts + g->cap_cells + 4;
  const int32_t* d_n = cloud->dn.as<int32_t>();
  GridHeader* hdr = g->hdr.as<GridHeader>();
  ProfScope prof(h, PK_GRID);
  if (from_box) {
    launch_pdl(grid_header_box_kernel, 1, 32, 0, h->stream, map_box, *map_crop, cell, g->cap_cells, hdr);
    h->launches++;
  } else {
    launch_pdl(grid_bbox_init_kernel, 1, 32, 0, h->stream, g->bbox.as<unsigned long long>());
    launch_pdl(grid_bbox_kernel, blocks, GB_THREADS, 0, h->stream, cloud->xyz.as<double>(), d_n, cd, use_crop, g->bbox.as<unsigned long long>());
    launch_pdl(grid_header_kernel, 1, 32, 0, h->stream, g->bbox.as<unsigned long long>(), cell, g->cap_cells, hdr);
    h->launches += 3;
  }
  launch_pdl(grid_zero_kernel, 4 * device_sms(), 256, 0, h->stream, hdr, counts);
  launch_pdl(grid_count_kernel, blocks, GB_THREADS, 0, h->stream, cloud->xyz.as<double>(), d_n, cd, use_crop, hdr, counts, g->rank.as<int32_t>());
  h->launches += 2;
  B2S_TRY(scan_exclusive_i32(h, counts, starts, &hdr->ncell, (size_t)g->cap_cells, nullptr));
  launch_pdl(grid_scatter_kernel, blocks, GB_THREADS, 0, h->stream, cloud->xyz.as<double>(), d_n, hdr, starts, g->rank.as<int32_t>(),
             g->pts.as<double4>(), orig);
  h->launches++;
  B2S_CUDA(cudaGetLastError());
  return B2S_OK;
}


static int32_t grid_reserve(b2s_handle* h, GridIndex* g, const b2s_cloud* cloud, size_t* n_alloc_out) {
  const size_t n_max = cloud->n_max > 0 ? cloud->n_max : 1;
  size_t n_alloc = cloud->xyz.cap / 24;
  if (n_alloc < n_max) n_alloc = n_max;
  size_t want = n_alloc * 8 + 4096;
  if (want > (size_t)1 << 21) want = (size_t)1 << 21;
  if (want < (size_t)1 << 16) want = (size_t)1 << 16;
  if ((size_t)g->cap_cells < want) {
    B2S_TRY(g->cell_start.ensure((want + 8) * 4 * 2, h->stream));
    g->cap_cells = (int32_t)want;
  }
  B2S_TRY(g->hdr.ensure(sizeof(GridHeader), h->stream));
  B2S_TRY(g->bbox.ensure(64, h->stream));
  B2S_TRY(g->rank.ensure(n_alloc * 4, h->stream));
  B2S_TRY(g->pts.ensure(n_alloc * 32, h->stream));
  *n_alloc_out = n_alloc;
  return B2S_OK;
}

int32_t grid_build_batch(b2s_handle* h, GridIndex* const* g, const b2s_cloud* const* clouds, int n, double cell) {
  B2S_REQUIRE(cell > 0.0, B2S_E_INVALID, "grid_build: cell size must be > 0");
  if (n <= 0) return B2S_OK;
  size_t max_pts = 1, max_cells = 1;
  for (int i = 0; i < n; i++) {
    size_t n_alloc;
    B2S_TRY(grid_reserve(h, g[i], clouds[i], &n_alloc));
    if (clouds[i]->n_max > max_pts) max_pts = clouds[i]->n_max;
    if ((size_t)g[i]->cap_cells > max_cells) max_cells = (size_t)g[i]->cap_cells;
  }
  Layout T;
  const size_t o_jobs = T.off((size_t)n * sizeof(GridJob)), o_scan = T.off((size_t)n * sizeof(ScanJob)), staged = T.size;
  h->batch_jobs_host.assign(staged, 0);
  GridJob* gj = reinterpret_cast<GridJob*>(h->batch_jobs_host.data() + o_jobs);
  ScanJob* sj = reinterpret_cast<ScanJob*>(h->batch_jobs_host.data() + o_scan);
  size_t state_end = 0;
  B2S_TRY(carve(h->batch_jobs, h->stream, [&](Layout& D) {
    D.off(staged);
    for (int i = 0; i < n; i++) scan_bind_state(D, sj[i], max_cells);
    state_end = D.size;
  }));
  unsigned char* dev = h->batch_jobs.as<unsigned char>();
  for (int i = 0; i < n; i++) {
    int32_t* counts = g[i]->cell_start.as<int32_t>();
    int32_t* starts = counts + g[i]->cap_cells + 4;
    GridHeader* hdr = g[i]->hdr.as<GridHeader>();
    gj[i].xyz = clouds[i]->xyz.as<double>();
    gj[i].d_n = clouds[i]->dn.as<int32_t>();
    gj[i].bbox = g[i]->bbox.as<unsigned long long>();
    gj[i].hdr = hdr; gj[i].counts = counts; gj[i].starts = starts; gj[i].rank = g[i]->rank.as<int32_t>();
    gj[i].pts = g[i]->pts.as<double4>();
    gj[i].cap_cells = g[i]->cap_cells;
    sj[i].in = counts; sj[i].out = starts; sj[i].d_n = &hdr->ncell;
  }
  B2S_CUDA(cudaMemcpyAsync(dev, h->batch_jobs_host.data(), staged, cudaMemcpyHostToDevice, h->stream));
  B2S_CUDA(cudaMemsetAsync(dev + staged, 0, state_end - staged, h->stream));
  const GridJob* dj = reinterpret_cast<const GridJob*>(dev + o_jobs);
  const ScanJob* ds = reinterpret_cast<const ScanJob*>(dev + o_scan);
  int bx = grid_for(max_pts, GB_THREADS, 2 * device_sms());
  const dim3 gpts((unsigned)bx, (unsigned)n);
  ProfScope prof(h, PK_GRID);
  launch_pdl(gridb_init_kernel, (n * 6 + 127) / 128, 128, 0, h->stream, dj, n);
  launch_pdl(gridb_bbox_kernel, gpts, GB_THREADS, 0, h->stream, dj);
  launch_pdl(gridb_header_kernel, (n + 127) / 128, 128, 0, h->stream, dj, n, cell);
  launch_pdl(gridb_zero_kernel, dim3((unsigned)device_sms(), (unsigned)n), 256, 0, h->stream, dj);
  launch_pdl(gridb_count_kernel, gpts, GB_THREADS, 0, h->stream, dj);
  h->launches += 5;
  B2S_TRY(scan_exclusive_i32_batch(h, ds, n, max_cells));
  launch_pdl(gridb_scatter_kernel, gpts, GB_THREADS, 0, h->stream, dj);
  h->launches++;
  B2S_CUDA(cudaGetLastError());
  return B2S_OK;
}

__global__ void tile_zero_kernel(int32_t* n) {
  pdl_wait();
  if (threadIdx.x == 0) *n = 0;
}

__device__ __forceinline__ void tile_box(const GridHeader& g, const CropDev& crop, int* box) {
  double lo[3], hi[3];
  crop_aabb(crop, lo, hi);
  for (int d = 0; d < 3; d++) {
    const double a = fmax(floor((lo[d] - g.origin[d]) * g.inv_cell) - TILE_MARGIN, 0.0);
    const double b = fmin(floor((hi[d] - g.origin[d]) * g.inv_cell) + TILE_MARGIN, (double)(g.dims[d] - 1));
    const bool ok = a <= b;
    box[d] = ok ? (int)a : 1;
    box[3 + d] = ok ? (int)b : 0;
  }
}

__global__ void __launch_bounds__(GB_THREADS) tile_gather_kernel(const GridHeader* __restrict__ thdr, const int32_t* __restrict__ tstart,
                                                                 const double4* __restrict__ tpts, CropDev crop, double* __restrict__ out_xyz,
                                                                 int32_t* __restrict__ out_idx, int32_t* __restrict__ out_n) {
  pdl_wait();
  __shared__ GridHeader g;
  __shared__ int box[6];
  if (threadIdx.x == 0) { g = *thdr; tile_box(g, crop, box); }
  __syncthreads();
  if (box[0] > box[3] || box[1] > box[4] || box[2] > box[5]) return;
  const int ny = box[4] - box[1] + 1, nz = box[5] - box[2] + 1;
  const int lane = threadIdx.x & 31;
  for (int r = blockIdx.x; r < ny * nz; r += gridDim.x) {
    const int row = ((box[2] + r / ny) * g.dims[1] + (box[1] + r % ny)) * g.dims[0];
    const int s0 = tstart[row + box[0]], s1 = tstart[row + box[3] + 1];
    for (int j0 = s0; j0 < s1; j0 += blockDim.x) {
      const int j = j0 + threadIdx.x;
      double4 q = make_double4(0.0, 0.0, 0.0, 0.0);
      bool pass = false;
      if (j < s1) { q = tpts[j]; pass = crop_within(crop, q.x, q.y, q.z); }
      const unsigned m = __ballot_sync(0xffffffffu, pass);
      int base = 0;
      if (lane == 0 && m) base = atomicAdd(out_n, __popc(m));
      base = __shfl_sync(0xffffffffu, base, 0);
      if (pass) {
        const int o = base + __popc(m & ((1u << lane) - 1u));
        out_xyz[3 * o] = q.x; out_xyz[3 * o + 1] = q.y; out_xyz[3 * o + 2] = q.z;
        out_idx[o] = (int32_t)__double_as_longlong(q.w);
      }
    }
  }
}

bool tile_patch_usable(const b2s_submap* sm, const CropDev& crop) {
  static const bool full = getenv("B2S_PATCH_FULL") && atoi(getenv("B2S_PATCH_FULL")) != 0;
  const bool bounded = !crop.invert && (crop.kind == B2S_CROP_MAX_RADIUS || crop.kind == B2S_CROP_MINMAX_RADIUS || crop.kind == B2S_CROP_CYLINDER);
  return !full && !sm->merge_scans && bounded;
}

int32_t tile_drop(b2s_handle* h, b2s_submap* sm) {
  if (!sm->tile_valid) return B2S_OK;
  sm->tile_valid = false;
  sm->opts_gen++;
  return graph_drop(h, &sm->graph);
}

int32_t tile_patch_build(b2s_handle* h, b2s_submap* sm, const CropDev& crop, double cell, GridIndex* g) {
  const b2s_cloud* map = sm->cloud[0].get();
  const size_t map_alloc = map->xyz.cap / 24;
  if (!sm->patch) B2S_TRY(make_cloud(h, map_alloc, false, false, &sm->patch));
  b2s_cloud* pc = sm->patch.get();
  B2S_TRY(cloud_reserve(h, pc, map_alloc, false));
  B2S_TRY(sm->patch_idx.ensure(map_alloc * 4 + 16, h->stream));
  if (!sm->tile_valid) {
    B2S_TRY(grid_build(h, &sm->tile, map, TILE_EDGE, nullptr));
    sm->tile_valid = true;
  }
  pc->n_max = map->n_max; pc->n_known = -1; pc->has_normals = false;
  {
    launch_pdl(tile_zero_kernel, 1, 32, 0, h->stream, pc->dn.as<int32_t>());
    launch_pdl(tile_gather_kernel, 2 * device_sms(), GB_THREADS, 0, h->stream, static_cast<const GridHeader*>(sm->tile.hdr.as<GridHeader>()),
               grid_starts(&sm->tile), static_cast<const double4*>(sm->tile.pts.as<double4>()), crop, pc->xyz.as<double>(),
               sm->patch_idx.as<int32_t>(), pc->dn.as<int32_t>());
    h->launches += 2;
  }
  return grid_build(h, g, pc, cell, nullptr, sm->patch_idx.as<int32_t>(), sm->bbox.as<unsigned long long>(), &crop);
}

}
```

### open3d_slam_b200/csrc/normals.cu

```cuda
#include "common.cuh"

namespace b2s {

constexpr int NK_THREADS = 128;

__device__ __forceinline__ void cross3d(const double* a, const double* b, double* o) {
  o[0] = a[1] * b[2] - a[2] * b[1]; o[1] = a[2] * b[0] - a[0] * b[2]; o[2] = a[0] * b[1] - a[1] * b[0];
}
__device__ __forceinline__ double dot3d(const double* a, const double* b) { return a[0] * b[0] + a[1] * b[1] + a[2] * b[2]; }

__device__ void eigvec0_dev(const double* A, double eval0, double* out) {
  double row0[3] = {A[0] - eval0, A[1], A[2]}, row1[3] = {A[1], A[4] - eval0, A[5]}, row2[3] = {A[2], A[5], A[8] - eval0};
  double r01[3], r02[3], r12[3];
  cross3d(row0, row1, r01); cross3d(row0, row2, r02); cross3d(row1, row2, r12);
  const double d0 = dot3d(r01, r01), d1 = dot3d(r02, r02), d2 = dot3d(r12, r12);
  double dmax = d0; int imax = 0;
  if (d1 > dmax) { dmax = d1; imax = 1; }
  if (d2 > dmax) { imax = 2; }
  const double* v = imax == 0 ? r01 : (imax == 1 ? r02 : r12);
  const double s = sqrt(imax == 0 ? d0 : (imax == 1 ? d1 : d2));
  out[0] = v[0] / s; out[1] = v[1] / s; out[2] = v[2] / s;
}

__device__ void eigvec1_dev(const double* A, const double* e0, double eval1, double* out) {
// ... 290 lines not shown
        if (t < total) {
          int lo = 0, hi = side * side;
          while (lo < hi) { const int mid = (lo + hi) >> 1; if (s_rp[wib][mid] > t) hi = mid; else lo = mid + 1; }
          const int r = lo - 1;
          j = s_ra[wib][r] + (t - s_rp[wib][r]);
          const double4 p = pts[j];
          dd = dist2_exact(qx, qy, qz, p.x, p.y, p.z);
          ii = (int)__double_as_longlong(p.w);
        }
        const bool ok = j >= 0 && dd < lim2;
        const unsigned m = __ballot_sync(0xffffffffu, ok);
        const int pos = nc + __popc(m & lt_mask);
        if (ok && pos < NS2_CAP) { s_d[wib][pos] = dd; s_i[wib][pos] = ii; s_s[wib][pos] = j; }
        nc += __popc(m);
      }
      __syncwarp();
      if (nc > NS2_CAP) {
        if (kDebug && lane == 0) { dbg_path[s] = NPATH_OVER_CAPACITY; dbg_sel[4 * (size_t)s] = nc; dbg_sel[4 * (size_t)s + 1] = -1; dbg_sel[4 * (size_t)s + 2] = 0; dbg_sel[4 * (size_t)s + 3] = lim2; }
        break;
      }
      const int nch = (nc + 31) >> 5;
      double d[NS2_CHUNKS]; int idx[NS2_CHUNKS];
#pragma unroll
      for (int c = 0; c < NS2_CHUNKS; c++) {
        if (c >= nch) break;
        const int t = c * 32 + lane;
        d[c] = INFINITY; idx[c] = 0x7fffffff;
        if (t < nc) { d[c] = s_d[wib][t]; idx[c] = s_i[wib][t]; }
      }
      __syncwarp();
      need = min(knn, nc);
      double td = INFINITY; int ti = 0x7fffffff;
      int dbg_bin = -1, dbg_nb = 0;
      if (nc > knn) {
        const double scale = lim2 > 0.0 ? 32.0 / lim2 : 0.0;
        s_hist[wib][lane] = 0;
        __syncwarp();
#pragma unroll
        for (int c = 0; c < NS2_CHUNKS; c++) {
          if (c >= nch) break;
          if (c * 32 + lane < nc) atomicAdd(&s_hist[wib][min(31, (int)(d[c] * scale))], 1);
        }
        __syncwarp();
        int cumh = s_hist[wib][lane];
#pragma unroll
        for (int o = 1; o < 32; o <<= 1) { const int t = __shfl_up_sync(0xffffffffu, cumh, o); if (lane >= o) cumh += t; }
        const int B = __ffs(__ballot_sync(0xffffffffu, cumh >= need)) - 1;
        const int below = B > 0 ? __shfl_sync(0xffffffffu, cumh, B - 1) : 0;
        const int m = need - below;
        int nb = 0;
#pragma unroll
        for (int c = 0; c < NS2_CHUNKS; c++) {
          if (c >= nch) break;
          const bool in_bin = c * 32 + lane < nc && min(31, (int)(d[c] * scale)) == B;
          const unsigned bm = __ballot_sync(0xffffffffu, in_bin);
          if (in_bin) { const int pos = nb + __popc(bm & lt_mask); s_d[wib][pos] = d[c]; s_i[wib][pos] = idx[c]; }
          nb += __popc(bm);
        }
        __syncwarp();
        if (kDebug) { dbg_bin = B; dbg_nb = nb; }
        for (int base = 0; base < nb; base += 32) {
          const int t = base + lane;
          double md = INFINITY; int mi = 0x7fffffff, rank = -1;
          if (t < nb) {
            md = s_d[wib][t]; mi = s_i[wib][t]; rank = 0;
            for (int u = 0; u < nb; u++) { const double od = s_d[wib][u]; const int oi = s_i[wib][u]; rank += (od < md || (od == md && oi < mi)) ? 1 : 0; }
          }
          const unsigned hit = __ballot_sync(0xffffffffu, rank == m - 1);
          if (hit) { const int src = __ffs(hit) - 1; td = __shfl_sync(0xffffffffu, md, src); ti = __shfl_sync(0xffffffffu, mi, src); break; }
        }
        __syncwarp();
      }
      if (!(nc >= knn || b2 > r2)) {
        if (last_try) {
          if (kDebug && lane == 0) { dbg_path[s] = NPATH_NOT_CERTIFIED; dbg_sel[4 * (size_t)s] = nc; dbg_sel[4 * (size_t)s + 1] = dbg_bin; dbg_sel[4 * (size_t)s + 2] = dbg_nb; dbg_sel[4 * (size_t)s + 3] = lim2; }
          break;
        }
        continue;
      }
#pragma unroll
      for (int c = 0; c < NS2_CHUNKS; c++) {
        if (c >= nch) break;
        const int t = c * 32 + lane;
        if (t < nc && (d[c] < td || (d[c] == td && idx[c] <= ti))) {
          const double4 p = pts[s_s[wib][t]];
          c9[0] += p.x; c9[1] += p.y; c9[2] += p.z;
          c9[3] += p.x * p.x; c9[4] += p.x * p.y; c9[5] += p.x * p.z;
          c9[6] += p.y * p.y; c9[7] += p.y * p.z; c9[8] += p.z * p.z;
        }
      }
      warp_sum9_transposed(c9, lane);
      resolved = true;
      if (kDebug && lane == 0) { dbg_path[s] = R <= NS2_RMAX ? R : NPATH_FULL_BLOCK; dbg_sel[4 * (size_t)s] = nc; dbg_sel[4 * (size_t)s + 1] = dbg_bin; dbg_sel[4 * (size_t)s + 2] = dbg_nb; dbg_sel[4 * (size_t)s + 3] = lim2; }
    }
    if (!resolved) {
      if (lane == 0) { queue[atomicAdd(queue_n, 1)] = s; cum[10 * (size_t)tq + 9] = -1.0; }
      continue;
    }
    {
      const int slot = lane >> 1;
      if (!(lane & 1) && slot < 10) cum[10 * (size_t)tq + slot] = slot < 9 ? c9[0] : (double)need;
    }
  }
}

template <bool kDebug>
__global__ void __launch_bounds__(NK_THREADS) normals_finish_kernel(const GridHeader* __restrict__ hdr, const double4* __restrict__ pts,
                                                                    const int32_t* __restrict__ qlist, const int32_t* __restrict__ qcount,
                                                                    const double* __restrict__ cum, const double* prior_nrm, double* out_nrm,
                                                                    double* __restrict__ dbg_rec) {
  pdl_wait();
  const int nq = qlist ? *qcount : hdr->n;
  for (int tq = blockIdx.x * blockDim.x + threadIdx.x; tq < nq; tq += gridDim.x * blockDim.x) {
    const double kkd = cum[10 * (size_t)tq + 9];
    if (kkd < 0.0) continue;
    double c9[9];
#pragma unroll
    for (int t = 0; t < 9; t++) c9[t] = cum[10 * (size_t)tq + t];
    const double4 qp = pts[qlist ? qlist[tq] : tq];
    const size_t qi = (size_t)(int)__double_as_longlong(qp.w);
    if (kDebug) {
#pragma unroll
      for (int t = 0; t < 9; t++) dbg_rec[10 * qi + t] = c9[t];
      dbg_rec[10 * qi + 9] = kkd;
    }
    double nr[3];
    finish_normal(c9, (int)kkd, qp.x, qp.y, qp.z, prior_nrm ? prior_nrm + 3 * qi : nullptr, nr);
    out_nrm[3 * qi] = nr[0]; out_nrm[3 * qi + 1] = nr[1]; out_nrm[3 * qi + 2] = nr[2];
  }
}


__global__ void zero_i32_kernel(int32_t* p) {
  pdl_wait(); p[0] = 0; p[1] = 0; }

__global__ void __launch_bounds__(NK_THREADS) normals_qlist_kernel(const GridHeader* __restrict__ hdr, const double4* __restrict__ pts,
                                                                   const int32_t* __restrict__ flags, int32_t* __restrict__ qlist,
                                                                   int32_t* qcount) {
  pdl_wait();
  const int n = hdr->n;
  const int lane = threadIdx.x & 31;
  const int n_round = (n + 31) & ~31;
  for (int s = blockIdx.x * blockDim.x + threadIdx.x; s < n_round; s += gridDim.x * blockDim.x) {
    bool take = false;
    if (s < n) take = flags[(int)__double_as_longlong(pts[s].w)] != 0;
    const unsigned m = __ballot_sync(0xffffffffu, take);
    int base = 0;
    if (lane == 0 && m) base = atomicAdd(qcount, __popc(m));
    base = __shfl_sync(0xffffffffu, base, 0);
    if (take) qlist[base + __popc(m & ((1u << lane) - 1u))] = s;
  }
}

int32_t op_estimate_normals(b2s_handle* h, b2s_cloud* c, int knn, double radius, double cell_hint, const int32_t* flags, bool with_prior,
                            const NormalsDebug* dbg) {
  B2S_REQUIRE(radius > 0.0, B2S_E_INVALID, "maxRadiusNormalEstimation_ must be > 0");
  B2S_REQUIRE(knn > 0, B2S_E_INVALID, "knnNormalEstimation_ must be > 0");
  B2S_REQUIRE(knn <= 32, B2S_E_UNSUPPORTED, "knn > 32 is not supported by the register-resident k-best list yet");
  B2S_REQUIRE(!with_prior || c->has_normals, B2S_E_NO_NORMALS, "prior normals requested for a cloud without normals");
  double cell = cell_hint > 0.0 ? cell_hint : radius / 4.0;
  if (cell < radius / 16.0) cell = radius / 16.0;
  B2S_TRY(grid_build(h, &h->grid_b, c, cell, nullptr));
  const size_t n_max = c->n_max > 0 ? c->n_max : 1;
  B2S_TRY(c->nrm.ensure(n_max * 24, h->stream, with_prior));
  int blocks = (int)((n_max + NK_THREADS - 1) / NK_THREADS);
  if (blocks > 16 * device_sms()) blocks = 16 * device_sms();
  if (blocks < 1) blocks = 1;
  B2S_TRY(h->tmp_i32.ensure((2 * n_max + 64) * 4, h->stream));
  int32_t* qn = h->tmp_i32.as<int32_t>() + 8;
  int32_t* queue = h->tmp_i32.as<int32_t>() + 16;
  int32_t* qlist = flags ? queue + n_max : nullptr;
  const int32_t* qcount = flags ? qn + 1 : nullptr;
  ProfScope prof(h, PK_NORMALS);
  const GridHeader* hdr = h->grid_b.hdr.as<GridHeader>();
  const int32_t* cs = grid_starts(&h->grid_b);
  const double4* pts = h->grid_b.pts.as<double4>();
  double* out = c->nrm.as<double>();
  const double* prior = with_prior ? out : nullptr;
  launch_pdl(zero_i32_kernel, 1, 1, 0, h->stream, qn);
  if (flags) {
    launch_pdl(normals_qlist_kernel, blocks, NK_THREADS, 0, h->stream, hdr, pts, flags, qlist, qn + 1);
    h->launches++;
  }
  static const int ns2_grid_env = getenv("B2S_NS2_GRID") ? atoi(getenv("B2S_NS2_GRID")) : 0;
  const int ns2_cap = ns2_grid_env > 0 ? ns2_grid_env : 16 * device_sms();
  int wblocks = (int)((n_max + (NK_THREADS / 32) - 1) / (NK_THREADS / 32));
  if (wblocks > ns2_cap) wblocks = ns2_cap;
  if (wblocks < 1) wblocks = 1;
  B2S_TRY(h->tmp_f64.ensure((n_max + 1) * 80, h->stream));
  double* cum = h->tmp_f64.as<double>();
  if (dbg) launch_pdl(normals_select2_kernel<true>, wblocks, NK_THREADS, 0, h->stream, hdr, cs, pts, knn, radius, qlist, qcount, queue, qn,
                      cum, dbg->path, dbg->sel);
  else launch_pdl(normals_select2_kernel<false>, wblocks, NK_THREADS, 0, h->stream, hdr, cs, pts, knn, radius, qlist, qcount, queue, qn, cum,
                  nullptr, nullptr);
  if (dbg) launch_pdl(normals_finish_kernel<true>, blocks, NK_THREADS, 0, h->stream, hdr, pts, qlist, qcount, cum, prior, out, dbg->rec);
  else launch_pdl(normals_finish_kernel<false>, blocks, NK_THREADS, 0, h->stream, hdr, pts, qlist, qcount, cum, prior, out, nullptr);
  if (dbg) launch_pdl(normals_phase2_kernel<true>, 4 * device_sms(), NK_THREADS, 0, h->stream, hdr, cs, pts, knn, radius, queue, qn, prior, out,
                      dbg->rec);
  else launch_pdl(normals_phase2_kernel<false>, 4 * device_sms(), NK_THREADS, 0, h->stream, hdr, cs, pts, knn, radius, queue, qn, prior, out,
                  nullptr);
  h->launches += 4;
  c->has_normals = true;
  B2S_CUDA(cudaGetLastError());
  return B2S_OK;
}

}
```

### open3d_slam_b200/csrc/runtime.cu

```cuda
#include <cooperative_groups.h>
#include <stdarg.h>
#include <stdlib.h>

#include "common.cuh"

namespace b2s {

static thread_local char g_err[1024] = {0};

void set_error(const char* fmt, ...) {
  va_list ap;
  va_start(ap, fmt);
  vsnprintf(g_err, sizeof(g_err), fmt, ap);
  va_end(ap);
}
const char* get_error() { return g_err; }

unsigned long long g_alloc_generation = 1;
static int g_device_sms[64] = {0};
int device_sms() {
  int d = 0;
  if (cudaGetDevice(&d) != cudaSuccess || d < 0 || d >= 64) d = 0;
  int v = __atomic_load_n(&g_device_sms[d], __ATOMIC_RELAXED);
  if (v <= 0) {
// ... 110 lines not shown
  for (const ReadBack& c : copies) { memcpy(c.dst, stage, c.bytes); stage += c.bytes; }
  return rc;
}

constexpr int SCAN_THREADS = 256;
constexpr int SCAN_ITEMS = 16;
constexpr int SCAN_TILE = SCAN_THREADS * SCAN_ITEMS;
#define FLAG_AGG (1ull << 62)
#define FLAG_PREFIX (2ull << 62)

__device__ __forceinline__ void scan_lookback_body(const int32_t* __restrict__ in, int32_t* __restrict__ out,
                                                   const int32_t* __restrict__ d_n, int32_t n_host, unsigned long long* state,
                                                   int32_t* tile_counter, int32_t* d_total) {
  __shared__ int s_tile;
  __shared__ int s_warp[SCAN_THREADS / 32];
  __shared__ int s_prefix;
  if (threadIdx.x == 0) s_tile = atomicAdd(tile_counter, 1);
  __syncthreads();
  const int tile = s_tile;
  const int n = d_n ? *d_n : n_host;
  const int ntiles = (n + SCAN_TILE - 1) / SCAN_TILE;
  if (tile >= ntiles) {
    if (tile == 0 && threadIdx.x == 0) { out[0] = 0; if (d_total) *d_total = 0; }
    return;
  }
  const int base = tile * SCAN_TILE + threadIdx.x * SCAN_ITEMS;
  int v[SCAN_ITEMS];
  const bool vec_ok = ((((size_t)in | (size_t)out) & 15) == 0);
  if (vec_ok && base + SCAN_ITEMS <= n) {
    const int4* p = reinterpret_cast<const int4*>(in + base);
#pragma unroll
    for (int k = 0; k < SCAN_ITEMS / 4; k++) { int4 q = p[k]; v[4 * k] = q.x; v[4 * k + 1] = q.y; v[4 * k + 2] = q.z; v[4 * k + 3] = q.w; }
  } else {
#pragma unroll
    for (int k = 0; k < SCAN_ITEMS; k++) v[k] = (base + k < n) ? in[base + k] : 0;
  }
  int tsum = 0;
#pragma unroll
  for (int k = 0; k < SCAN_ITEMS; k++) tsum += v[k];
  const int lane = threadIdx.x & 31, warp = threadIdx.x >> 5;
  int inc = tsum;
#pragma unroll
  for (int o = 1; o < 32; o <<= 1) { int t = __shfl_up_sync(0xffffffffu, inc, o); if (lane >= o) inc += t; }
  if (lane == 31) s_warp[warp] = inc;
  __syncthreads();
  int woff = 0, agg = 0;
#pragma unroll
  for (int w = 0; w < SCAN_THREADS / 32; w++) { int t = s_warp[w]; if (w < warp) woff += t; agg += t; }
  int texcl = woff + inc - tsum;
  if (warp == 0) {
    volatile unsigned long long* vs = state;
    if (tile == 0) {
      if (lane == 0) { vs[0] = FLAG_PREFIX | (unsigned long long)(unsigned)agg; s_prefix = 0; }
    } else {
      if (lane == 0) vs[tile] = FLAG_AGG | (unsigned long long)(unsigned)agg;
      int look = tile - 1, excl = 0;
      while (true) {
        int idx = look - lane;
        unsigned long long s = (idx >= 0) ? vs[idx] : FLAG_PREFIX;
        unsigned flag = (unsigned)(s >> 62);
        if (__any_sync(0xffffffffu, flag == 0)) continue;
        unsigned pmask = __ballot_sync(0xffffffffu, flag == 2);
        int val = (int)(unsigned)(s & 0xffffffffull);
        if (pmask) {
          int first = __ffs(pmask) - 1;
          excl += warp_sum_i(lane <= first ? val : 0);
          excl = __shfl_sync(0xffffffffu, excl, 0);
          break;
        }
        excl += warp_sum_i(val);
        excl = __shfl_sync(0xffffffffu, excl, 0);
        look -= 32;
      }
      if (lane == 0) { vs[tile] = FLAG_PREFIX | (unsigned long long)(unsigned)(excl + agg); s_prefix = excl; }
    }
  }
  __syncthreads();
  int run = s_prefix + texcl;
  if (vec_ok && base + SCAN_ITEMS <= n) {
    int o[SCAN_ITEMS];
#pragma unroll
    for (int k = 0; k < SCAN_ITEMS; k++) { o[k] = run; run += v[k]; }
    int4* p = reinterpret_cast<int4*>(out + base);
#pragma unroll
    for (int k = 0; k < SCAN_ITEMS / 4; k++) p[k] = make_int4(o[4 * k], o[4 * k + 1], o[4 * k + 2], o[4 * k + 3]);
  } else {
#pragma unroll
    for (int k = 0; k < SCAN_ITEMS; k++) { if (base + k < n) out[base + k] = run; run += v[k]; }
  }
  if (tile == ntiles - 1 && threadIdx.x == SCAN_THREADS - 1) {
    out[n] = s_prefix + agg;
    if (d_total) *d_total = s_prefix + agg;
  }
}

__global__ void __launch_bounds__(SCAN_THREADS) scan_lookback_kernel(const int32_t* __restrict__ in, int32_t* __restrict__ out,
                                                                     const int32_t* __restrict__ d_n, int32_t n_host,
                                                                     unsigned long long* state, int32_t* tile_counter,
                                                                     int32_t* d_total) {
  pdl_wait();
  scan_lookback_body(in, out, d_n, n_host, state, tile_counter, d_total);
}

__global__ void __launch_bounds__(SCAN_THREADS) scan_lookback_batch_kernel(const ScanJob* __restrict__ jobs) {
  pdl_wait();
  const ScanJob j = jobs[blockIdx.y];
  scan_lookback_body(j.in, j.out, j.d_n, 0, j.state, j.counter, nullptr);
}

static int scan_tiles(size_t n_max) {
  const size_t ntiles = (n_max + SCAN_TILE - 1) / SCAN_TILE;
  return ntiles < 1 ? 1 : (int)ntiles;
}
static size_t scan_state_bytes(size_t n_max) { return (size_t)scan_tiles(n_max) * 8 + 64; }
static int32_t* scan_counter(unsigned long long* state, size_t n_max) { return reinterpret_cast<int32_t*>(state + scan_tiles(n_max)); }

void scan_bind_state(Layout& L, ScanJob& j, size_t n_max) {
  unsigned char* s = L.take<unsigned char>(scan_state_bytes(n_max));
  if (!s) return;
  j.state = reinterpret_cast<unsigned long long*>(s);
  j.counter = scan_counter(j.state, n_max);
}

int32_t scan_exclusive_i32_batch(b2s_handle* h, const ScanJob* jobs_dev, int njobs, size_t n_max) {
  launch_pdl(scan_lookback_batch_kernel, dim3(scan_tiles(n_max), njobs), SCAN_THREADS, 0, h->stream, jobs_dev);
  h->launches++;
  B2S_CUDA(cudaGetLastError());
  return B2S_OK;
}

static int32_t scan_impl(b2s_handle* h, const int32_t* in, int32_t* out, const int32_t* d_n, int32_t n_host, size_t n_max,
                         int32_t* d_total, DevBuf* state) {
  const int ntiles = scan_tiles(n_max);
  DevBuf& sb = state ? *state : h->scan.state;
  B2S_TRY(sb.ensure(scan_state_bytes(n_max), h->stream));
  B2S_CUDA(cudaMemsetAsync(sb.p, 0, scan_state_bytes(n_max), h->stream));
  unsigned long long* st = sb.as<unsigned long long>();
  int32_t* counter = scan_counter(st, n_max);
  launch_pdl(scan_lookback_kernel, ntiles, SCAN_THREADS, 0, h->stream, in, out, d_n, n_host, st, counter, d_total);
  h->launches++;
  B2S_CUDA(cudaGetLastError());
  return B2S_OK;
}

int32_t scan_exclusive_i32(b2s_handle* h, const int32_t* in, int32_t* out, const int32_t* d_n, size_t n_max, int32_t* d_total, DevBuf* state) {
  return scan_impl(h, in, out, d_n, (int32_t)n_max, n_max, d_total, state);
}

constexpr int RS_THREADS = 256;
constexpr int RS_ITEMS = 8;
constexpr int RS_TILE = RS_THREADS * RS_ITEMS;
constexpr int RS_WARPS = RS_THREADS / 32;

template <typename K>
__global__ void __launch_bounds__(RS_THREADS) rs_hist_kernel(const K* __restrict__ keys, const int32_t* __restrict__ d_n, int shift,
                                                             int32_t* __restrict__ hist, int nblocks) {
  pdl_wait();
  __shared__ int s_h[256];
  s_h[threadIdx.x] = 0;
  __syncthreads();
  const int n = *d_n;
  const int base = blockIdx.x * RS_TILE;
#pragma unroll
  for (int k = 0; k < RS_ITEMS; k++) {
    int i = base + k * RS_THREADS + threadIdx.x;
    if (i < n) atomicAdd(&s_h[(int)((keys[i] >> shift) & 0xFF)], 1);
  }
  __syncthreads();
  hist[threadIdx.x * nblocks + blockIdx.x] = s_h[threadIdx.x];
}

template <typename K>
__global__ void __launch_bounds__(RS_THREADS) rs_scatter_kernel(const K* __restrict__ keys_in, const uint32_t* __restrict__ vals_in,
                                                                K* __restrict__ keys_out, uint32_t* __restrict__ vals_out,
                                                                const int32_t* __restrict__ d_n, int shift,
                                                                const int32_t* __restrict__ offs, int nblocks) {
  pdl_wait();
  __shared__ int s_cnt[RS_WARPS][256];
  __shared__ int s_base[256];
  const int lane = threadIdx.x & 31, warp = threadIdx.x >> 5;
  for (int i = threadIdx.x; i < RS_WARPS * 256; i += RS_THREADS) (&s_cnt[0][0])[i] = 0;
  __syncthreads();
  const int n = *d_n;
  const int wbase = blockIdx.x * RS_TILE + warp * 32 * RS_ITEMS;
  K key[RS_ITEMS];
  int lrank[RS_ITEMS];
#pragma unroll
  for (int k = 0; k < RS_ITEMS; k++) {
    int i = wbase + k * 32 + lane;
    bool valid = i < n;
    key[k] = valid ? keys_in[i] : (K)0;
    int d = valid ? (int)((key[k] >> shift) & 0xFF) : 256 + lane;
    unsigned peers = __match_any_sync(0xffffffffu, d);
    int prior = valid ? s_cnt[warp][d] : 0;
    __syncwarp();
    lrank[k] = prior + __popc(peers & ((1u << lane) - 1u));
    if (valid && (peers & ((1u << lane) - 1u)) == 0) s_cnt[warp][d] = prior + __popc(peers);
    __syncwarp();
  }
  __syncthreads();
  {
    const int d = threadIdx.x;
    int run = offs[d * nblocks + blockIdx.x];
#pragma unroll
    for (int w = 0; w < RS_WARPS; w++) { int c = s_cnt[w][d]; s_cnt[w][d] = run; run += c; }
  }
  __syncthreads();
#pragma unroll
  for (int k = 0; k < RS_ITEMS; k++) {
    int i = wbase + k * 32 + lane;
    if (i < n) {
      int d = (int)((key[k] >> shift) & 0xFF);
      int pos = s_cnt[warp][d] + lrank[k];
      keys_out[pos] = key[k];
      vals_out[pos] = vals_in[i];
    }
  }
  (void)s_base;
}

constexpr int CS_CTAS = 8;
constexpr int CS_THREADS = 1024;
constexpr int CS_WARPS = CS_THREADS / 32;
constexpr int CS_ITEMS = 8;
constexpr int CS_TILE = CS_THREADS * CS_ITEMS;

template <typename K>
__global__ void __cluster_dims__(CS_CTAS, 1, 1) __launch_bounds__(CS_THREADS, 1)
    cluster_sort_kernel(K* __restrict__ keys_a, uint32_t* __restrict__ vals_a, K* __restrict__ keys_b, uint32_t* __restrict__ vals_b,
                        const int32_t* __restrict__ d_n, int passes) {
  pdl_wait();
  namespace cg = cooperative_groups;
  cg::cluster_group cluster = cg::this_cluster();
  const int rank = (int)cluster.block_rank();
  extern __shared__ int cs_smem[];
  int* s_hist = cs_smem;
  int* s_base = s_hist + 256;
  int* s_scan = s_base + 256;
  int* s_cnt = s_scan + CS_WARPS;
  const int tid = threadIdx.x, lane = tid & 31, warp = tid >> 5;
  const int n = *d_n;
  const int tiles_total = (n + CS_TILE - 1) / CS_TILE;
  const int tiles_per = (tiles_total + CS_CTAS - 1) / CS_CTAS;
  const int lo = min(rank * tiles_per * CS_TILE, n), hi = min(lo + tiles_per * CS_TILE, n);
  for (int p = 0; p < passes; ++p) {
    const K* kin = (p & 1) ? keys_b : keys_a;
    const uint32_t* vin = (p & 1) ? vals_b : vals_a;
    K* kout = (p & 1) ? keys_a : keys_b;
    uint32_t* vout = (p & 1) ? vals_a : vals_b;
    const int shift = 8 * p;
    if (tid < 256) s_hist[tid] = 0;
    __syncthreads();
    for (int i = lo + tid; i < hi; i += CS_THREADS) atomicAdd(&s_hist[(int)((kin[i] >> shift) & 0xFF)], 1);
    cluster.sync();
    {
      int tot = 0, mine = 0;
      if (tid < 256) {
        for (int r = 0; r < CS_CTAS; ++r) {
          const int c = cluster.map_shared_rank(s_hist, r)[tid];
          if (r < rank) mine += c;
          tot += c;
        }
      }
      int inc = tot;
#pragma unroll
      for (int o = 1; o < 32; o <<= 1) { const int t = __shfl_up_sync(0xffffffffu, inc, o); if (lane >= o) inc += t; }
      if (lane == 31 && warp < 8) s_scan[warp] = inc;
      __syncthreads();
      if (tid < 256) {
        int woff = 0;
        for (int w = 0; w < warp; ++w) woff += s_scan[w];
        s_base[tid] = woff + inc - tot + mine;
      }
    }
    __syncthreads();
    for (int t0 = lo; t0 < hi; t0 += CS_TILE) {
      for (int i = tid; i < CS_WARPS * 256; i += CS_THREADS) s_cnt[i] = 0;
      __syncthreads();
      const int wbase = t0 + warp * 32 * CS_ITEMS;
      K key[CS_ITEMS];
      int lrank[CS_ITEMS];
#pragma unroll
      for (int k = 0; k < CS_ITEMS; k++) {
        const int i = wbase + k * 32 + lane;
        key[k] = (i < hi) ? kin[i] : (K)0;
      }
#pragma unroll
      for (int k = 0; k < CS_ITEMS; k++) {
        const int i = wbase + k * 32 + lane;
        const bool valid = i < hi;
        const int d = valid ? (int)((key[k] >> shift) & 0xFF) : 256 + lane;
        const unsigned peers = __match_any_sync(0xffffffffu, d);
        const int prior = valid ? s_cnt[warp * 256 + d] : 0;
        __syncwarp();
        lrank[k] = prior + __popc(peers & ((1u << lane) - 1u));
        if (valid && (peers & ((1u << lane) - 1u)) == 0) s_cnt[warp * 256 + d] = prior + __popc(peers);
        __syncwarp();
      }
      __syncthreads();
      if (tid < 256) {
        int run = s_base[tid];
        for (int w = 0; w < CS_WARPS; w++) { const int c = s_cnt[w * 256 + tid]; s_cnt[w * 256 + tid] = run; run += c; }
        s_base[tid] = run;
      }
      __syncthreads();
#pragma unroll
      for (int k = 0; k < CS_ITEMS; k++) {
        const int i = wbase + k * 32 + lane;
        if (i < hi) {
          const int d = (int)((key[k] >> shift) & 0xFF);
          const int pos = s_cnt[warp * 256 + d] + lrank[k];
          kout[pos] = key[k];
          vout[pos] = vin[i];
        }
      }
      __syncthreads();
    }
    __threadfence();
    cluster.sync();
  }
}

static bool g_cs_attr32 = false, g_cs_attr64 = false;

template <typename K>
static int32_t cluster_sort_impl(b2s_handle* h, K*& keys, uint32_t*& vals, K*& keys_alt, uint32_t*& vals_alt, const int32_t* d_n, int key_bits) {
  int passes = (key_bits + 7) / 8;
  if (passes < 1) passes = 1;
  const size_t smem = (size_t)(256 + 256 + CS_WARPS + CS_WARPS * 256) * sizeof(int);
  bool& attr = sizeof(K) == 4 ? g_cs_attr32 : g_cs_attr64;
  if (!attr) {
    B2S_CUDA(cudaFuncSetAttribute(cluster_sort_kernel<K>, cudaFuncAttributeMaxDynamicSharedMemorySize, (int)smem));
    attr = true;
  }
  ProfScope prof(h, PK_SORT);
  launch_pdl(cluster_sort_kernel<K>, CS_CTAS, CS_THREADS, smem, h->stream, keys, vals, keys_alt, vals_alt, d_n, passes);
  h->launches++;
  B2S_CUDA(cudaGetLastError());
  if (passes & 1) {
    K* tk = keys; keys = keys_alt; keys_alt = tk;
    uint32_t* tv = vals; vals = vals_alt; vals_alt = tv;
  }
  return B2S_OK;
}

static bool use_multi_kernel_sort() {
  static const bool v = getenv("B2S_SORT") && strcmp(getenv("B2S_SORT"), "multi") == 0;
  return v;
}

template <typename K>
static int32_t radix_sort_impl(b2s_handle* h, K*& keys, uint32_t*& vals, K*& keys_alt, uint32_t*& vals_alt, const int32_t* d_n,
                               size_t n_max, int key_bits, VoxelScratch* own) {
  if (!use_multi_kernel_sort() && n_max <= ((size_t)3 << 18)) return cluster_sort_impl<K>(h, keys, vals, keys_alt, vals_alt, d_n, key_bits);
  int nblocks = (int)((n_max + RS_TILE - 1) / RS_TILE);
  if (nblocks < 1) nblocks = 1;
  size_t hist_n = (size_t)256 * nblocks;
  DevBuf& hb = own ? own->sort_hist : h->sort.hist;
  B2S_TRY(hb.ensure((hist_n + 8) * 4 * 2, h->stream));
  int32_t* hist = hb.as<int32_t>();
  int32_t* offs = hist + ((hist_n + 4) & ~(size_t)3);
  int passes = (key_bits + 7) / 8;
  if (passes < 1) passes = 1;
  ProfScope prof(h, PK_SORT);
  for (int p = 0; p < passes; p++) {
    int shift = 8 * p;
    launch_pdl(rs_hist_kernel<K>, nblocks, RS_THREADS, 0, h->stream, keys, d_n, shift, hist, nblocks);
    h->launches++;
    B2S_TRY(scan_impl(h, hist, offs, nullptr, (int32_t)hist_n, hist_n, nullptr, own ? &own->scan_state : nullptr));
    launch_pdl(rs_scatter_kernel<K>, nblocks, RS_THREADS, 0, h->stream, keys, vals, keys_alt, vals_alt, d_n, shift, offs, nblocks);
    h->launches++;
    K* tk = keys; keys = keys_alt; keys_alt = tk;
    uint32_t* tv = vals; vals = vals_alt; vals_alt = tv;
  }
  B2S_CUDA(cudaGetLastError());
  return B2S_OK;
}

int32_t radix_sort_pairs_u32(b2s_handle* h, uint32_t*& keys, uint32_t*& vals, uint32_t*& keys_alt, uint32_t*& vals_alt,
                             const int32_t* d_n, size_t n_max, int key_bits, VoxelScratch* own) {
  return radix_sort_impl<uint32_t>(h, keys, vals, keys_alt, vals_alt, d_n, n_max, key_bits, own);
}
int32_t radix_sort_pairs_u64(b2s_handle* h, uint64_t*& keys, uint32_t*& vals, uint64_t*& keys_alt, uint32_t*& vals_alt,
                             const int32_t* d_n, size_t n_max, int key_bits, VoxelScratch* own) {
  return radix_sort_impl<uint64_t>(h, keys, vals, keys_alt, vals_alt, d_n, n_max, key_bits, own);
}

}
```

### open3d_slam_b200/csrc/voxel.cu

```cuda
#include "common.cuh"

namespace b2s {

constexpr int VX_THREADS = 256;

__global__ void bbox_init_kernel(unsigned long long* bbox, int32_t* kept) {
  pdl_wait();
  int t = threadIdx.x;
  if (t < 3) bbox[t] = ord_encode(INFINITY);
  else if (t < 6) bbox[t] = ord_encode(-INFINITY);
  if (t == 6 && kept) *kept = 0;
}

__global__ void __launch_bounds__(VX_THREADS) bbox_kernel(const double* __restrict__ xyz, const int32_t* __restrict__ d_n, CropDev crop,
                                                          int use_crop, unsigned long long* bbox) {
  pdl_wait();
  const int n = *d_n;
  double mn[3] = {INFINITY, INFINITY, INFINITY}, mx[3] = {-INFINITY, -INFINITY, -INFINITY};
  for (int i = blockIdx.x * blockDim.x + threadIdx.x; i < n; i += gridDim.x * blockDim.x) {
    double x = xyz[3 * i], y = xyz[3 * i + 1], z = xyz[3 * i + 2];
    if (!(x == x && y == y && z == z)) continue;
    if (use_crop && !crop_within(crop, x, y, z)) continue;
    mn[0] = fmin(mn[0], x); mn[1] = fmin(mn[1], y); mn[2] = fmin(mn[2], z);
    mx[0] = fmax(mx[0], x); mx[1] = fmax(mx[1], y); mx[2] = fmax(mx[2], z);
  }
  __shared__ double s[6][VX_THREADS / 32];
  const int lane = threadIdx.x & 31, warp = threadIdx.x >> 5;
#pragma unroll
  for (int d = 0; d < 3; d++) { mn[d] = warp_min(mn[d]); mx[d] = warp_max(mx[d]); }
  if (lane == 0) { for (int d = 0; d < 3; d++) { s[d][warp] = mn[d]; s[3 + d][warp] = mx[d]; } }
  __syncthreads();
  if (threadIdx.x < 6) {
    int d = threadIdx.x;
    double v = s[d][0];
    for (int w = 1; w < VX_THREADS / 32; w++) v = d < 3 ? fmin(v, s[d][w]) : fmax(v, s[d][w]);
    if (d < 3) atomicMin(&bbox[d], ord_encode(v)); else atomicMax(&bbox[d], ord_encode(v));
  }
}

int32_t bbox_reduce(b2s_handle* h, const double* xyz, const int32_t* d_n, size_t n_max, const CropDev* crop, unsigned long long* bbox) {
  CropDev cd = crop ? *crop : make_crop(nullptr);
  launch_pdl(bbox_init_kernel, 1, 32, 0, h->stream, bbox, nullptr);
  launch_pdl(bbox_kernel, grid_for(n_max, VX_THREADS), VX_THREADS, 0, h->stream, xyz, d_n, cd, crop ? 1 : 0, bbox);
  h->launches += 2;
  B2S_CUDA(cudaGetLastError());
  return B2S_OK;
}

__global__ void set_count_kernel(int32_t* dn, int32_t n) {
  pdl_wait(); *dn = n; }

int32_t cloud_reserve(b2s_handle* h, b2s_cloud* c, size_t n, bool normals) {
  size_t m = n > 0 ? n : 1;
  B2S_TRY(c->xyz.ensure(m * 24, h->stream, true));
  if (normals) B2S_TRY(c->nrm.ensure(m * 24, h->stream, true));
  B2S_TRY(c->dn.ensure(4, h->stream, true));
  return B2S_OK;
}
int32_t cloud_set_count(b2s_handle* h, b2s_cloud* c, size_t n) {
  B2S_TRY(c->dn.ensure(4, h->stream, true));
  launch_pdl(set_count_kernel, 1, 1, 0, h->stream, c->dn.as<int32_t>(), (int32_t)n);
  h->launches++;
  c->n_known = (long long)n;
  c->n_max = c->fixed_cap ? c->fixed_cap : n;
  return B2S_OK;
}

__global__ void __launch_bounds__(VX_THREADS) crop_flags_kernel(const double* __restrict__ xyz, const int32_t* __restrict__ d_n,
                                                                CropDev crop, int32_t* __restrict__ flags) {
  pdl_wait();
  const int n = *d_n;
  for (int i = blockIdx.x * blockDim.x + threadIdx.x; i < n; i += gridDim.x * blockDim.x)
    flags[i] = crop_within(crop, xyz[3 * i], xyz[3 * i + 1], xyz[3 * i + 2]) ? 1 : 0;
}

__global__ void __launch_bounds__(VX_THREADS) compact_kernel(const double* __restrict__ xyz, const double* __restrict__ nrm,
                                                             const int32_t* __restrict__ d_n, const int32_t* __restrict__ flags,
                                                             const int32_t* __restrict__ offs, double* __restrict__ oxyz,
                                                             double* __restrict__ onrm, int32_t* out_n) {
  pdl_wait();
  const int n = *d_n;
  if (blockIdx.x == 0 && threadIdx.x == 0) *out_n = offs[n];
  for (int i = blockIdx.x * blockDim.x + threadIdx.x; i < n; i += gridDim.x * blockDim.x) {
    if (!flags[i]) continue;
    const int o = offs[i];
    oxyz[3 * o] = xyz[3 * i]; oxyz[3 * o + 1] = xyz[3 * i + 1]; oxyz[3 * o + 2] = xyz[3 * i + 2];
    if (nrm) { onrm[3 * o] = nrm[3 * i]; onrm[3 * o + 1] = nrm[3 * i + 1]; onrm[3 * o + 2] = nrm[3 * i + 2]; }
  }
}

int32_t compact_cloud(b2s_handle* h, const b2s_cloud* in, const int32_t* flags, b2s_cloud* out, const int32_t* d_n_override = nullptr);
int32_t compact_cloud(b2s_handle* h, const b2s_cloud* in, const int32_t* flags, b2s_cloud* out, const int32_t* d_n_override) {
  const size_t n_max = in->n_max;
  const int32_t* d_n = d_n_override ? d_n_override : in->dn.as<int32_t>();
  B2S_TRY(h->offs.ensure((n_max + 2) * 4, h->stream));
  B2S_TRY(cloud_reserve(h, out, n_max, in->has_normals));
  B2S_TRY(scan_exclusive_i32(h, flags, h->offs.as<int32_t>(), d_n, n_max, nullptr));
  launch_pdl(compact_kernel, grid_for(n_max, VX_THREADS), VX_THREADS, 0, h->stream, 
      in->xyz.as<double>(), in->has_normals ? in->nrm.as<double>() : nullptr, d_n, flags, h->offs.as<int32_t>(),
      out->xyz.as<double>(), in->has_normals ? out->nrm.as<double>() : nullptr, out->dn.as<int32_t>());
  h->launches++;
  out->has_normals = in->has_normals;
  out->n_max = n_max;
  out->n_known = -1;
  B2S_CUDA(cudaGetLastError());
  return B2S_OK;
}

int32_t op_crop(b2s_handle* h, const b2s_cloud* in, const CropDev& crop, b2s_cloud* out) {
  const size_t n_max = in->n_max;
  B2S_TRY(h->flags.ensure((n_max + 1) * 4, h->stream));
  launch_pdl(crop_flags_kernel, grid_for(n_max, VX_THREADS), VX_THREADS, 0, h->stream, in->xyz.as<double>(), in->dn.as<int32_t>(), crop,
                                                                               h->flags.as<int32_t>());
  h->launches++;
  return compact_cloud(h, in, h->flags.as<int32_t>(), out);
}

template <typename K>
__device__ __forceinline__ K morton3(uint32_t x, uint32_t y, uint32_t z);
template <>
__device__ __forceinline__ uint32_t morton3<uint32_t>(uint32_t x, uint32_t y, uint32_t z) {
  return morton_part10(x) | (morton_part10(y) << 1) | (morton_part10(z) << 2);
}
template <>
__device__ __forceinline__ uint64_t morton3<uint64_t>(uint32_t x, uint32_t y, uint32_t z) {
  return morton_part21(x) | (morton_part21(y) << 1) | (morton_part21(z) << 2);
}

template <typename K>
__global__ void __launch_bounds__(VX_THREADS) voxel_keys_kernel(const double* __restrict__ xyz, const int32_t* __restrict__ d_n,
                                                                CropDev crop, int use_crop, const unsigned long long* __restrict__ bbox,
                                                                double voxel, int bits, K* __restrict__ keys, uint32_t* __restrict__ vals,
                                                                uint32_t* status) {
  pdl_wait();
  const int n = *d_n;
  const K invalid = (K)1 << (3 * bits);
  const double half = __dmul_rn(voxel, 0.5);
  const double vmx = __dsub_rn(ord_decode(bbox[0]), half), vmy = __dsub_rn(ord_decode(bbox[1]), half), vmz = __dsub_rn(ord_decode(bbox[2]), half);
  const double lim = (double)(1u << bits);
  for (int i = blockIdx.x * blockDim.x + threadIdx.x; i < n; i += gridDim.x * blockDim.x) {
    const double x = xyz[3 * i], y = xyz[3 * i + 1], z = xyz[3 * i + 2];
    K key = invalid;
    if ((x == x && y == y && z == z) && (!use_crop || crop_within(crop, x, y, z))) {
      const double fx = floor(__ddiv_rn(__dsub_rn(x, vmx), voxel)), fy = floor(__ddiv_rn(__dsub_rn(y, vmy), voxel)),
                   fz = floor(__ddiv_rn(__dsub_rn(z, vmz), voxel));
      if (fx >= 0.0 && fy >= 0.0 && fz >= 0.0 && fx < lim && fy < lim && fz < lim) key = morton3<K>((uint32_t)fx, (uint32_t)fy, (uint32_t)fz);
      else atomicOr(status, ST_KEY_OVERFLOW);
    }
    keys[i] = key;
    vals[i] = (uint32_t)i;
  }
}

template <typename K>
__global__ void __launch_bounds__(VX_THREADS) seg_head_kernel(const K* __restrict__ keys, const int32_t* __restrict__ d_n, int bits,
                                                              int singletons_for_invalid, int32_t* __restrict__ head) {
  pdl_wait();
  const int n = *d_n;
  const K invalid = (K)1 << (3 * bits);
  for (int j = blockIdx.x * blockDim.x + threadIdx.x; j < n; j += gridDim.x * blockDim.x) {
    const K k = keys[j];
    int hd;
    if (k >= invalid) hd = singletons_for_invalid;
    else hd = (j == 0 || keys[j - 1] != k) ? 1 : 0;
    head[j] = hd;
  }
}

template <typename K>
__global__ void __launch_bounds__(VX_THREADS) voxel_mean_kernel(const K* __restrict__ keys, const uint32_t* __restrict__ vals,
                                                                const int32_t* __restrict__ d_n, const int32_t* __restrict__ head,
                                                                const int32_t* __restrict__ offs, const double* __restrict__ xyz,
                                                                const double* __restrict__ nrm, double* __restrict__ oxyz,
                                                                double* __restrict__ onrm, int32_t* out_n, const int32_t* __restrict__ label,
                                                                const double* __restrict__ palette, double* __restrict__ ocol) {
  pdl_wait();
  const int n = *d_n;
  if (blockIdx.x == 0 && threadIdx.x == 0) *out_n = offs[n];
  for (int j = blockIdx.x * blockDim.x + threadIdx.x; j < n; j += gridDim.x * blockDim.x) {
    if (!head[j]) continue;
    const K k = keys[j];
    double sx = 0, sy = 0, sz = 0, nx = 0, ny = 0, nz = 0, cr = 0, cg = 0, cb = 0;
    int cnt = 0;
    for (int t = j; t < n && keys[t] == k; ++t) {
      const uint32_t i = vals[t];
      sx = __dadd_rn(sx, xyz[3 * i]); sy = __dadd_rn(sy, xyz[3 * i + 1]); sz = __dadd_rn(sz, xyz[3 * i + 2]);
      if (nrm) {
        const double a = nrm[3 * i], b = nrm[3 * i + 1], c = nrm[3 * i + 2];
        if (a == a && b == b && c == c) { nx = __dadd_rn(nx, a); ny = __dadd_rn(ny, b); nz = __dadd_rn(nz, c); }
      }
      if (label) {
        const double* pc = palette + 3 * label[i];
        cr = __dadd_rn(cr, pc[0]); cg = __dadd_rn(cg, pc[1]); cb = __dadd_rn(cb, pc[2]);
      }
      cnt++;
    }
    const int o = offs[j];
    const double c = (double)cnt;
    oxyz[3 * o] = __ddiv_rn(sx, c); oxyz[3 * o + 1] = __ddiv_rn(sy, c); oxyz[3 * o + 2] = __ddiv_rn(sz, c);
    if (nrm) { onrm[3 * o] = __ddiv_rn(nx, c); onrm[3 * o + 1] = __ddiv_rn(ny, c); onrm[3 * o + 2] = __ddiv_rn(nz, c); }
    if (label) { ocol[3 * o] = __ddiv_rn(cr, c); ocol[3 * o + 1] = __ddiv_rn(cg, c); ocol[3 * o + 2] = __ddiv_rn(cb, c); }
  }
}

static int bits_for(double extent, double voxel) {
  double cells = floor(extent / voxel) + 3.0;
  int b = 1;
  while ((double)(1u << b) < cells && b < 22) b++;
  return b;
}
int voxel_key_bits(double extent, double voxel) { return bits_for(extent, voxel); }

template <typename K>
static int32_t voxel_impl(b2s_handle* h, const b2s_cloud* in, const CropDev* crop, double voxel, int bits, b2s_cloud* out, VoxelScratch* own,
                          const int32_t* labels, const double* palette, double* rgb_out) {
  const size_t n_max = in->n_max > 0 ? in->n_max : 1;
  DevBuf& kb = own ? own->keys : h->keys;
  DevBuf& vb = own ? own->vals : h->vals;
  DevBuf& fb = own ? own->flags : h->flags;
  DevBuf& ob = own ? own->offs : h->offs;
  B2S_TRY(kb.ensure(n_max * sizeof(K) * 2, h->stream));
  B2S_TRY(vb.ensure(n_max * 4 * 2, h->stream));
  B2S_TRY(fb.ensure((n_max + 1) * 4, h->stream));
  B2S_TRY(ob.ensure((n_max + 2) * 4, h->stream));
  B2S_TRY(cloud_reserve(h, out, n_max, in->has_normals));
  K* keys = kb.as<K>(); K* keys_alt = keys + n_max;
  uint32_t* vals = vb.as<uint32_t>(); uint32_t* vals_alt = vals + n_max;
  const int32_t* d_n = in->dn.as<int32_t>();
  const int blocks = grid_for(n_max, VX_THREADS);
  CropDev cd = crop ? *crop : make_crop(nullptr);
  { ProfScope prof(h, PK_VOXEL);
  launch_pdl(voxel_keys_kernel<K>, blocks, VX_THREADS, 0, h->stream, in->xyz.as<double>(), d_n, cd, crop ? 1 : 0, h->misc.as<unsigned long long>(),
                                                             voxel, bits, keys, vals, h->status.as<uint32_t>());
  h->launches++; }
  if constexpr (sizeof(K) == 4) {
    B2S_TRY(radix_sort_pairs_u32(h, keys, vals, keys_alt, vals_alt, d_n, n_max, 3 * bits + 1, own));
  } else {
    B2S_TRY(radix_sort_pairs_u64(h, keys, vals, keys_alt, vals_alt, d_n, n_max, 3 * bits + 1, own));
  }
  ProfScope prof2(h, PK_VOXEL);
  launch_pdl(seg_head_kernel<K>, blocks, VX_THREADS, 0, h->stream, keys, d_n, bits, 0, fb.as<int32_t>());
  h->launches++;
  B2S_TRY(scan_exclusive_i32(h, fb.as<int32_t>(), ob.as<int32_t>(), d_n, n_max, nullptr, own ? &own->scan_state : nullptr));
  launch_pdl(voxel_mean_kernel<K>, blocks, VX_THREADS, 0, h->stream, keys, vals, d_n, fb.as<int32_t>(), ob.as<int32_t>(),
                                                             in->xyz.as<double>(), in->has_normals ? in->nrm.as<double>() : nullptr,
                                                             out->xyz.as<double>(), in->has_normals ? out->nrm.as<double>() : nullptr,
                                                             out->dn.as<int32_t>(), labels, palette, rgb_out);
  h->launches++;
  out->has_normals = in->has_normals;
  out->n_max = in->n_max;
  out->n_known = -1;
  B2S_CUDA(cudaGetLastError());
  return B2S_OK;
}

int32_t op_voxel_down_sample(b2s_handle* h, const b2s_cloud* in, const CropDev* crop, double voxel, b2s_cloud* out, int fixed_key_bits,
                             VoxelScratch* own, const int32_t* labels, const double* palette, double* rgb_out) {
  if (voxel <= 0.0) {
    if (crop) return op_crop(h, in, *crop, out);
    B2S_TRY(cloud_reserve(h, out, in->n_max, in->has_normals));
    B2S_CUDA(cudaMemcpyAsync(out->xyz.p, in->xyz.p, in->n_max * 24, cudaMemcpyDeviceToDevice, h->stream));
    if (in->has_normals) B2S_CUDA(cudaMemcpyAsync(out->nrm.p, in->nrm.p, in->n_max * 24, cudaMemcpyDeviceToDevice, h->stream));
    B2S_CUDA(cudaMemcpyAsync(out->dn.p, in->dn.p, 4, cudaMemcpyDeviceToDevice, h->stream));
    out->has_normals = in->has_normals; out->n_max = in->n_max; out->n_known = in->n_known;
    return B2S_OK;
  }
  B2S_TRY(h->misc.ensure(256, h->stream));
  unsigned long long* bbox = h->misc.as<unsigned long long>();
  B2S_TRY(bbox_reduce(h, in->xyz.as<double>(), in->dn.as<int32_t>(), in->n_max > 0 ? in->n_max : 1, crop, bbox));
  int bits;
  const bool bounded = crop && !crop->invert && !crop->pose_dev &&
                       (crop->kind == B2S_CROP_MAX_RADIUS || crop->kind == B2S_CROP_MINMAX_RADIUS);
  if (fixed_key_bits > 0) bits = fixed_key_bits;
  else if (bounded) bits = bits_for(2.0 * crop->rmax, voxel);
  else {
    unsigned long long hb[6];
    B2S_CUDA(cudaMemcpyAsync(hb, bbox, 48, cudaMemcpyDeviceToHost, h->stream));
    B2S_CUDA(cudaStreamSynchronize(h->stream));
    double ext = 0.0;
    for (int d = 0; d < 3; d++) { double e = ord_decode(hb[3 + d]) - ord_decode(hb[d]); if (e > ext) ext = e; }
    if (!(ext >= 0.0)) ext = 0.0;
    bits = bits_for(ext, voxel);
  }
  B2S_REQUIRE(bits <= 21, B2S_E_INVALID, "[VoxelDownSample] voxel_size is too small for the extent of the cloud");
  if (bits <= 10) return voxel_impl<uint32_t>(h, in, crop, voxel, bits, out, own, labels, palette, rgb_out);
  return voxel_impl<uint64_t>(h, in, crop, voxel, bits, out, own, labels, palette, rgb_out);
}

__device__ __forceinline__ uint32_t select_hash(uint32_t seed, double x, double y, double z) {
  const uint64_t a = (uint64_t)__double_as_longlong(x), b = (uint64_t)__double_as_longlong(y), c = (uint64_t)__double_as_longlong(z);
  uint64_t v = a * 0x9E3779B97F4A7C15ull;
  v ^= (b + 0x7F4A7C15F39CC060ull) * 0xC2B2AE3D27D4EB4Full;
  v ^= (c + 0x165667B19E3779F9ull) * 0xD6E8FEB86659FD93ull;
  v += (uint64_t)seed * 0x85EBCA77C2B2AE63ull;
  v ^= v >> 29; v *= 0xBF58476D1CE4E5B9ull; v ^= v >> 32; v *= 0x94D049BB133111EBull; v ^= v >> 29;
  return (uint32_t)(v >> 32);
}
__global__ void __launch_bounds__(VX_THREADS) select_keys_kernel(const double* __restrict__ xyz, const int32_t* __restrict__ d_n, uint32_t seed,
                                                                 uint32_t* __restrict__ keys, uint32_t* __restrict__ vals,
                                                                 int32_t* __restrict__ flags) {
  pdl_wait();
  const int n = *d_n;
  for (int i = blockIdx.x * blockDim.x + threadIdx.x; i < n; i += gridDim.x * blockDim.x) {
    keys[i] = select_hash(seed, xyz[3 * i], xyz[3 * i + 1], xyz[3 * i + 2]);
    vals[i] = (uint32_t)i;
    flags[i] = 0;
  }
}
__global__ void __launch_bounds__(VX_THREADS) select_mark_kernel(const int32_t* __restrict__ d_n, double ratio, const uint32_t* __restrict__ vals,
                                                                 int32_t* __restrict__ flags) {
  pdl_wait();
  const int n = *d_n;
  size_t k = (size_t)((double)n * ratio);
  if (k > (size_t)n) k = (size_t)n;
  for (int j = blockIdx.x * blockDim.x + threadIdx.x; j < (int)k; j += gridDim.x * blockDim.x) flags[vals[j]] = 1;
}

constexpr int SK_THREADS = 1024;
__global__ void __launch_bounds__(SK_THREADS) select_kth_kernel(const uint32_t* __restrict__ keys, const int32_t* __restrict__ d_n,
                                                                double ratio, uint32_t* __restrict__ sel) {
  pdl_wait();
  __shared__ int s_hist[256];
  __shared__ int s_scan[8];
  __shared__ uint32_t s_prefix;
  __shared__ int s_rem, s_cnt;
  const int tid = threadIdx.x, lane = tid & 31, warp = tid >> 5;
  const int n = *d_n;
  size_t k = (size_t)((double)n * ratio);
  if (k > (size_t)n) k = (size_t)n;
  if (k == 0) { if (tid < 4) sel[tid] = 0; return; }
  uint32_t prefix = 0;
  int rem = (int)k;
  for (int pass = 3; pass >= 0; --pass) {
    const int shift = 8 * pass;
    const uint32_t hi_mask = pass == 3 ? 0u : (0xFFFFFFFFu << (shift + 8));
    if (tid < 256) s_hist[tid] = 0;
    __syncthreads();
    for (int i = tid; i < n; i += SK_THREADS) {
      const uint32_t key = keys[i];
      if ((key & hi_mask) == prefix) atomicAdd(&s_hist[(key >> shift) & 0xFF], 1);
    }
    __syncthreads();
    int h = 0, inc = 0;
    if (tid < 256) {
      h = s_hist[tid];
      inc = h;
#pragma unroll
      for (int o = 1; o < 32; o <<= 1) { const int t = __shfl_up_sync(0xffffffffu, inc, o); if (lane >= o) inc += t; }
      if (lane == 31) s_scan[warp] = inc;
    }
    __syncthreads();
    if (tid < 256) {
      for (int w = 0; w < warp; ++w) inc += s_scan[w];
      const int exc = inc - h;
      if (exc < rem && rem <= inc) { s_prefix = prefix | ((uint32_t)tid << shift); s_rem = rem - exc; s_cnt = h; }
    }
    __syncthreads();
    prefix = s_prefix; rem = s_rem;
    __syncthreads();
  }
  if (tid == 0) { sel[0] = prefix; sel[1] = (uint32_t)rem; sel[2] = (uint32_t)s_cnt; sel[3] = (uint32_t)k; }
}

__global__ void __launch_bounds__(VX_THREADS) select_mark_kth_kernel(const int32_t* __restrict__ d_n, const uint32_t* __restrict__ keys,
                                                                     const uint32_t* __restrict__ sel, int32_t* __restrict__ flags) {
  pdl_wait();
  const int n = *d_n;
  const uint32_t kth = sel[0], need = sel[1], cnt_eq = sel[2], k = sel[3];
  for (int i = blockIdx.x * blockDim.x + threadIdx.x; i < n; i += gridDim.x * blockDim.x) {
    const uint32_t key = keys[i];
    int f = 0;
    if (k > 0) {
      if (key < kth) f = 1;
      else if (key == kth) {
        if (need == cnt_eq) f = 1;
        else {
          uint32_t before = 0;
          for (int j = 0; j < i; ++j) before += keys[j] == kth;
          f = before < need;
        }
      }
    }
    flags[i] = f;
  }
}

int32_t select_flags(b2s_handle* h, const b2s_cloud* in, double ratio, uint32_t seed) {
  B2S_REQUIRE(ratio >= 0.0 && ratio < 1.0, B2S_E_INVALID, "[RandomDownSample] sampling_ratio must be in [0, 1]");
  const size_t n_max = in->n_max > 0 ? in->n_max : 1;
  B2S_TRY(h->keys.ensure(n_max * 4 * 2, h->stream));
  B2S_TRY(h->vals.ensure(n_max * 4 * 2, h->stream));
  B2S_TRY(h->flags.ensure((n_max + 1) * 4, h->stream));
  uint32_t* keys = h->keys.as<uint32_t>(); uint32_t* keys_alt = keys + n_max;
  uint32_t* vals = h->vals.as<uint32_t>(); uint32_t* vals_alt = vals + n_max;
  const int blocks = grid_for(n_max, VX_THREADS);
  launch_pdl(select_keys_kernel, blocks, VX_THREADS, 0, h->stream, in->xyz.as<double>(), in->dn.as<int32_t>(), seed, keys, vals,
                                                           h->flags.as<int32_t>());
  h->launches++;
  if (n_max <= ((size_t)1 << 18)) {
    ProfScope prof(h, PK_SELECT);
    B2S_TRY(h->misc.ensure(256, h->stream));
    uint32_t* sel = h->misc.as<uint32_t>() + 32;
    launch_pdl(select_kth_kernel, 1, SK_THREADS, 0, h->stream, keys, in->dn.as<int32_t>(), ratio, sel);
    launch_pdl(select_mark_kth_kernel, blocks, VX_THREADS, 0, h->stream, in->dn.as<int32_t>(), keys, sel, h->flags.as<int32_t>());
    h->launches += 2;
    B2S_CUDA(cudaGetLastError());
    return B2S_OK;
  }
  B2S_TRY(radix_sort_pairs_u32(h, keys, vals, keys_alt, vals_alt, in->dn.as<int32_t>(), n_max, 32));
  launch_pdl(select_mark_kernel, blocks, VX_THREADS, 0, h->stream, in->dn.as<int32_t>(), ratio, vals, h->flags.as<int32_t>());
  h->launches++;
  B2S_CUDA(cudaGetLastError());
  return B2S_OK;
}

int32_t select_compact(b2s_handle* h, const b2s_cloud* in, double ratio, b2s_cloud* out) {
  B2S_TRY(compact_cloud(h, in, h->flags.as<int32_t>(), out));
  const size_t bound = (size_t)((double)in->n_max * ratio) + 1;
  if (bound < out->n_max) out->n_max = bound;
  return B2S_OK;
}

int32_t op_random_down_sample(b2s_handle* h, const b2s_cloud* in, double ratio, uint32_t seed, b2s_cloud* out) {
  B2S_REQUIRE(ratio >= 0.0, B2S_E_INVALID, "[RandomDownSample] sampling_ratio must be in [0, 1]");
  const size_t n_max = in->n_max > 0 ? in->n_max : 1;
  if (ratio >= 1.0) {
    B2S_TRY(cloud_reserve(h, out, n_max, in->has_normals));
    B2S_CUDA(cudaMemcpyAsync(out->xyz.p, in->xyz.p, n_max * 24, cudaMemcpyDeviceToDevice, h->stream));
    if (in->has_normals) B2S_CUDA(cudaMemcpyAsync(out->nrm.p, in->nrm.p, n_max * 24, cudaMemcpyDeviceToDevice, h->stream));
    B2S_CUDA(cudaMemcpyAsync(out->dn.p, in->dn.p, 4, cudaMemcpyDeviceToDevice, h->stream));
    out->has_normals = in->has_normals; out->n_max = in->n_max; out->n_known = in->n_known;
    return B2S_OK;
  }
  B2S_TRY(select_flags(h, in, ratio, seed));
  return select_compact(h, in, ratio, out);
}

__global__ void __launch_bounds__(VX_THREADS) transform_kernel(const double* __restrict__ xyz, const double* __restrict__ nrm,
                                                               const int32_t* __restrict__ d_n, const double* __restrict__ Tdev,
// ... 145 lines not shown
```

Baseline: 9243.

## Build normals grid index during voxel downsampling and widen radix digits to 11 bits

The scan-preprocessing path now counts grid cells inside the voxel mean kernel. It reuses the voxel bbox for the grid header and finishes the grid with a scan and scatter, so normal estimation skips its own grid build. Separately, the radix sort uses 11-bit digits for 25–33-bit keys, which cuts the number of passes, and shrinks the per-warp counters to uint16. This adds atomics to the mean kernel and makes the grid depend on the downsample bbox. It also adds a debug radix sort API.

```diff
diff --git a/include/b2s.h b/include/b2s.h
--- a/include/b2s.h
+++ b/include/b2s.h
@@ -191,6 +191,8 @@
 int32_t b2s_debug_nn_index(b2s_handle* h, double origin_cell[4], int32_t dims_n[5], int32_t* cell_start, size_t cap_cells, int32_t* orig,
                            size_t cap_pts);
 int32_t b2s_debug_submap_bbox(b2s_handle* h, const b2s_submap* sm, double box[6]);
+int32_t b2s_debug_radix_sort(b2s_handle* h, const uint64_t* keys, const uint32_t* vals, int32_t n, int32_t key_bits, uint64_t* keys_out,
+                             uint32_t* vals_out);
 
 typedef struct b2s_global_localization_params {
   double x_min, x_max, y_min, y_max;
diff --git a/open3d_slam_b200/_lib.py b/open3d_slam_b200/_lib.py
--- a/open3d_slam_b200/_lib.py
+++ b/open3d_slam_b200/_lib.py
@@ -182,7 +182,7 @@
     "b2s_default_global_optimization_params", "b2s_global_optimization", "b2s_cloud_transform_inplace",
     "b2s_submap_set_initial_map", "b2s_submap_set_initial_transform", "b2s_submap_set_merge_scans", "b2s_debug_nn_index",
     "b2s_assemble_map", "b2s_assemble_colored_map", "b2s_debug_pose_graph_solve", "b2s_debug_pose_graph_linearize",
-    "b2s_debug_estimate_normals", "b2s_debug_submap_bbox",
+    "b2s_debug_estimate_normals", "b2s_debug_submap_bbox", "b2s_debug_radix_sort",
     "b2s_default_global_localization_params", "b2s_submap_global_localization", "b2s_debug_global_localization_scores",
     "b2s_submaps_global_localization", "b2s_debug_submaps_global_localization_scores",
     "b2s_assemble_dense_maps",
diff --git a/open3d_slam_b200/csrc/c_api.cu b/open3d_slam_b200/csrc/c_api.cu
--- a/open3d_slam_b200/csrc/c_api.cu
+++ b/open3d_slam_b200/csrc/c_api.cu
@@ -115,18 +115,22 @@
   c0.center[0] = c0.center[1] = c0.center[2] = 0.0;
   CropDev wide = make_crop(&c0);
   const bool has_crop = c0.kind != B2S_CROP_NONE || c0.invert;
-  if (voxel_size > 0.0) B2S_TRY(op_voxel_down_sample(h, raw, has_crop ? &wide : nullptr, voxel_size, t0));
+  static const double cell_factor = getenv("B2S_NORMALS_CELL_FACTOR") ? atof(getenv("B2S_NORMALS_CELL_FACTOR")) : 4.0;
+  const double cell_hint = voxel_size > 0.0 ? cell_factor * voxel_size : 0.0;
+  static const bool own_index = getenv("B2S_NORMALS_OWN_INDEX") && atoi(getenv("B2S_NORMALS_OWN_INDEX")) != 0;
+  const bool index_built = voxel_size > 0.0 && !own_index && icp.knn_radius > 0.0;
+  if (voxel_size > 0.0)
+    B2S_TRY(op_voxel_down_sample(h, raw, has_crop ? &wide : nullptr, voxel_size, t0, 0, nullptr, nullptr, nullptr, nullptr,
+                                 index_built ? &h->grid_b : nullptr, normals_cell(icp.knn_radius, cell_hint)));
   else if (has_crop) B2S_TRY(op_crop(h, raw, wide, t0));
   else B2S_TRY(op_voxel_down_sample(h, raw, nullptr, 0.0, t0));
-  static const double cell_factor = getenv("B2S_NORMALS_CELL_FACTOR") ? atof(getenv("B2S_NORMALS_CELL_FACTOR")) : 4.0;
-  const double cell_hint = voxel_size > 0.0 ? cell_factor * voxel_size : 0.0;
   if (ratio < 1.0) {
     B2S_REQUIRE(ratio >= 0.0, B2S_E_INVALID, "[RandomDownSample] sampling_ratio must be in [0, 1]");
     B2S_TRY(select_flags(h, t0, ratio, seed));
-    B2S_TRY(op_estimate_normals(h, t0, icp.knn, icp.knn_radius, cell_hint, h->flags.as<int32_t>()));
+    B2S_TRY(op_estimate_normals(h, t0, icp.knn, icp.knn_radius, cell_hint, h->flags.as<int32_t>(), false, nullptr, index_built));
     B2S_TRY(select_compact(h, t0, ratio, out));
   } else {
-    B2S_TRY(op_estimate_normals(h, t0, icp.knn, icp.knn_radius, cell_hint));
+    B2S_TRY(op_estimate_normals(h, t0, icp.knn, icp.knn_radius, cell_hint, nullptr, false, nullptr, index_built));
     B2S_TRY(op_random_down_sample(h, t0, ratio, seed, out));
   }
   return B2S_OK;
@@ -1410,6 +1414,42 @@
   return rc;
 }
 
+int32_t b2s_debug_radix_sort(b2s_handle* h, const uint64_t* keys, const uint32_t* vals, int32_t n, int32_t key_bits, uint64_t* keys_out,
+                             uint32_t* vals_out) {
+  B2S_REQUIRE(h && keys && vals && keys_out && vals_out, B2S_E_INVALID, "null argument");
+  B2S_REQUIRE(n >= 1 && key_bits >= 1 && key_bits <= 64, B2S_E_INVALID, "n must be >= 1 and key_bits in 1..64");
+  LOCK(h);
+  const size_t m = (size_t)n;
+  const bool wide = key_bits > 32;
+  const size_t kw = wide ? 8 : 4;
+  std::vector<uint32_t> k32;
+  if (!wide) { k32.resize(m); for (size_t i = 0; i < m; i++) k32[i] = (uint32_t)keys[i]; }
+  DevBuf kb, vb, nb;
+  kb.tracked = vb.tracked = nb.tracked = false;
+  B2S_TRY(kb.ensure(2 * m * kw, h->stream));
+  B2S_TRY(vb.ensure(2 * m * 4, h->stream));
+  B2S_TRY(nb.ensure(4, h->stream));
+  B2S_CUDA(cudaMemcpyAsync(kb.p, wide ? (const void*)keys : (const void*)k32.data(), m * kw, cudaMemcpyHostToDevice, h->stream));
+  B2S_CUDA(cudaMemcpyAsync(vb.p, vals, m * 4, cudaMemcpyHostToDevice, h->stream));
+  B2S_CUDA(cudaMemcpyAsync(nb.p, &n, 4, cudaMemcpyHostToDevice, h->stream));
+  const void* res_k = nullptr;
+  uint32_t* v = vb.as<uint32_t>(); uint32_t* v_alt = v + m;
+  if (wide) {
+    uint64_t* k = kb.as<uint64_t>(); uint64_t* k_alt = k + m;
+    B2S_TRY(radix_sort_pairs_u64(h, k, v, k_alt, v_alt, nb.as<int32_t>(), m, key_bits));
+    res_k = k;
+  } else {
+    uint32_t* k = kb.as<uint32_t>(); uint32_t* k_alt = k + m;
+    B2S_TRY(radix_sort_pairs_u32(h, k, v, k_alt, v_alt, nb.as<int32_t>(), m, key_bits));
+    res_k = k;
+  }
+  B2S_CUDA(cudaMemcpyAsync(wide ? (void*)keys_out : (void*)k32.data(), res_k, m * kw, cudaMemcpyDeviceToHost, h->stream));
+  B2S_CUDA(cudaMemcpyAsync(vals_out, v, m * 4, cudaMemcpyDeviceToHost, h->stream));
+  B2S_CUDA(cudaStreamSynchronize(h->stream));
+  if (!wide) for (size_t i = 0; i < m; i++) keys_out[i] = k32[i];
+  return B2S_OK;
+}
+
 static int32_t check_assembly_args(b2s_handle* h, int32_t n, const b2s_submap* const* submaps, const b2s_cloud* out) {
   B2S_REQUIRE(h && out, B2S_E_INVALID, "null argument");
   B2S_REQUIRE(n >= 0, B2S_E_INVALID, "n_submaps must be >= 0");
diff --git a/open3d_slam_b200/csrc/common.cuh b/open3d_slam_b200/csrc/common.cuh
--- a/open3d_slam_b200/csrc/common.cuh
+++ b/open3d_slam_b200/csrc/common.cuh
@@ -362,6 +362,8 @@
 CropDev make_crop(const b2s_cropper* c, const double* pose_dev = nullptr);
 int32_t grid_build(b2s_handle* h, GridIndex* g, const b2s_cloud* cloud, double cell, const CropDev* patch, const int32_t* orig = nullptr,
                    const unsigned long long* map_box = nullptr, const CropDev* map_crop = nullptr);
+int32_t grid_begin_counted(b2s_handle* h, GridIndex* g, const b2s_cloud* cloud, double cell, const unsigned long long* box);
+int32_t grid_finish_counted(b2s_handle* h, GridIndex* g, const b2s_cloud* cloud);
 int32_t box_reset(b2s_handle* h, unsigned long long* box);
 bool tile_patch_usable(const b2s_submap* sm, const CropDev& crop);
 int32_t tile_patch_build(b2s_handle* h, b2s_submap* sm, const CropDev& crop, double cell, GridIndex* g);
@@ -377,7 +379,7 @@
 int32_t op_crop(b2s_handle* h, const b2s_cloud* in, const CropDev& crop, b2s_cloud* out);
 int32_t op_voxel_down_sample(b2s_handle* h, const b2s_cloud* in, const CropDev* crop, double voxel, b2s_cloud* out, int fixed_key_bits = 0,
                              VoxelScratch* own = nullptr, const int32_t* labels = nullptr, const double* palette = nullptr,
-                             double* rgb_out = nullptr);
+                             double* rgb_out = nullptr, GridIndex* index = nullptr, double index_cell = 0.0);
 int voxel_key_bits(double extent, double voxel);
 int32_t bbox_reduce(b2s_handle* h, const double* xyz, const int32_t* d_n, size_t n_max, const CropDev* crop, unsigned long long* bbox);
 int32_t op_assemble_map(b2s_handle* h, int n, const b2s_submap* const* submaps, double voxel, b2s_cloud* out, bool colored, double* rgb,
@@ -385,7 +387,8 @@
 int32_t op_assemble_dense_maps(b2s_handle* h, int n, const b2s_submap* const* submaps, b2s_cloud* out, int64_t* offsets);
 struct NormalsDebug { double* rec; int32_t* path; double* sel; };
 int32_t op_estimate_normals(b2s_handle* h, b2s_cloud* c, int knn, double radius, double cell_hint, const int32_t* flags = nullptr,
-                            bool with_prior = false, const NormalsDebug* dbg = nullptr);
+                            bool with_prior = false, const NormalsDebug* dbg = nullptr, bool index_built = false);
+double normals_cell(double radius, double cell_hint);
 int32_t select_flags(b2s_handle* h, const b2s_cloud* in, double ratio, uint32_t seed);
 int32_t select_compact(b2s_handle* h, const b2s_cloud* in, double ratio, b2s_cloud* out);
 int32_t op_random_down_sample(b2s_handle* h, const b2s_cloud* in, double ratio, uint32_t seed, b2s_cloud* out);
diff --git a/open3d_slam_b200/csrc/grid_index.cu b/open3d_slam_b200/csrc/grid_index.cu
--- a/open3d_slam_b200/csrc/grid_index.cu
+++ b/open3d_slam_b200/csrc/grid_index.cu
@@ -202,11 +202,7 @@
   return d;
 }
 
-int32_t grid_build(b2s_handle* h, GridIndex* g, const b2s_cloud* cloud, double cell, const CropDev* patch, const int32_t* orig,
-                   const unsigned long long* map_box, const CropDev* map_crop) {
-  B2S_REQUIRE(cell > 0.0, B2S_E_INVALID, "grid_build: cell size must be > 0");
-  static const bool bbox_pass = getenv("B2S_GRID_BBOX_PASS") && atoi(getenv("B2S_GRID_BBOX_PASS")) != 0;
-  const bool from_box = map_box && map_crop && !bbox_pass;
+static int32_t grid_reserve(b2s_handle* h, GridIndex* g, const b2s_cloud* cloud, size_t* n_alloc_out) {
   const size_t n_max = cloud->n_max > 0 ? cloud->n_max : 1;
   size_t n_alloc = cloud->xyz.cap / 24;
   if (n_alloc < n_max) n_alloc = n_max;
@@ -221,11 +217,34 @@
   B2S_TRY(g->bbox.ensure(64, h->stream));
   B2S_TRY(g->rank.ensure(n_alloc * 4, h->stream));
   B2S_TRY(g->pts.ensure(n_alloc * 32, h->stream));
+  *n_alloc_out = n_alloc;
+  return B2S_OK;
+}
+
+static int32_t grid_scan_scatter(b2s_handle* h, GridIndex* g, const b2s_cloud* cloud, const int32_t* orig) {
+  const size_t n_max = cloud->n_max > 0 ? cloud->n_max : 1;
+  int32_t* counts = g->cell_start.as<int32_t>();
+  GridHeader* hdr = g->hdr.as<GridHeader>();
+  B2S_TRY(scan_exclusive_i32(h, counts, counts + g->cap_cells + 4, &hdr->ncell, (size_t)g->cap_cells, nullptr));
+  launch_pdl(grid_scatter_kernel, grid_for(n_max, GB_THREADS), GB_THREADS, 0, h->stream, cloud->xyz.as<double>(), cloud->dn.as<int32_t>(), hdr,
+             grid_starts(g), g->rank.as<int32_t>(), g->pts.as<double4>(), orig);
+  h->launches++;
+  B2S_CUDA(cudaGetLastError());
+  return B2S_OK;
+}
+
+int32_t grid_build(b2s_handle* h, GridIndex* g, const b2s_cloud* cloud, double cell, const CropDev* patch, const int32_t* orig,
+                   const unsigned long long* map_box, const CropDev* map_crop) {
+  B2S_REQUIRE(cell > 0.0, B2S_E_INVALID, "grid_build: cell size must be > 0");
+  static const bool bbox_pass = getenv("B2S_GRID_BBOX_PASS") && atoi(getenv("B2S_GRID_BBOX_PASS")) != 0;
+  const bool from_box = map_box && map_crop && !bbox_pass;
+  const size_t n_max = cloud->n_max > 0 ? cloud->n_max : 1;
+  size_t n_alloc;
+  B2S_TRY(grid_reserve(h, g, cloud, &n_alloc));
   CropDev cd = patch ? *patch : make_crop(nullptr);
   const int use_crop = patch ? 1 : 0;
   const int blocks = grid_for(n_max, GB_THREADS);
   int32_t* counts = g->cell_start.as<int32_t>();
-  int32_t* starts = counts + g->cap_cells + 4;
   const int32_t* d_n = cloud->dn.as<int32_t>();
   GridHeader* hdr = g->hdr.as<GridHeader>();
   ProfScope prof(h, PK_GRID);
@@ -241,32 +260,25 @@
   launch_pdl(grid_zero_kernel, 4 * device_sms(), 256, 0, h->stream, hdr, counts);
   launch_pdl(grid_count_kernel, blocks, GB_THREADS, 0, h->stream, cloud->xyz.as<double>(), d_n, cd, use_crop, hdr, counts, g->rank.as<int32_t>());
   h->launches += 2;
-  B2S_TRY(scan_exclusive_i32(h, counts, starts, &hdr->ncell, (size_t)g->cap_cells, nullptr));
-  launch_pdl(grid_scatter_kernel, blocks, GB_THREADS, 0, h->stream, cloud->xyz.as<double>(), d_n, hdr, starts, g->rank.as<int32_t>(),
-             g->pts.as<double4>(), orig);
-  h->launches++;
+  return grid_scan_scatter(h, g, cloud, orig);
+}
+
+int32_t grid_begin_counted(b2s_handle* h, GridIndex* g, const b2s_cloud* cloud, double cell, const unsigned long long* box) {
+  B2S_REQUIRE(cell > 0.0, B2S_E_INVALID, "grid_build: cell size must be > 0");
+  size_t n_alloc;
+  B2S_TRY(grid_reserve(h, g, cloud, &n_alloc));
+  GridHeader* hdr = g->hdr.as<GridHeader>();
+  ProfScope prof(h, PK_GRID);
+  launch_pdl(grid_header_kernel, 1, 32, 0, h->stream, box, cell, g->cap_cells, hdr);
+  launch_pdl(grid_zero_kernel, 4 * device_sms(), 256, 0, h->stream, hdr, g->cell_start.as<int32_t>());
+  h->launches += 2;
   B2S_CUDA(cudaGetLastError());
   return B2S_OK;
 }
 
-
-static int32_t grid_reserve(b2s_handle* h, GridIndex* g, const b2s_cloud* cloud, size_t* n_alloc_out) {
-  const size_t n_max = cloud->n_max > 0 ? cloud->n_max : 1;
-  size_t n_alloc = cloud->xyz.cap / 24;
-  if (n_alloc < n_max) n_alloc = n_max;
-  size_t want = n_alloc * 8 + 4096;
-  if (want > (size_t)1 << 21) want = (size_t)1 << 21;
-  if (want < (size_t)1 << 16) want = (size_t)1 << 16;
-  if ((size_t)g->cap_cells < want) {
-    B2S_TRY(g->cell_start.ensure((want + 8) * 4 * 2, h->stream));
-    g->cap_cells = (int32_t)want;
-  }
-  B2S_TRY(g->hdr.ensure(sizeof(GridHeader), h->stream));
-  B2S_TRY(g->bbox.ensure(64, h->stream));
-  B2S_TRY(g->rank.ensure(n_alloc * 4, h->stream));
-  B2S_TRY(g->pts.ensure(n_alloc * 32, h->stream));
-  *n_alloc_out = n_alloc;
-  return B2S_OK;
+int32_t grid_finish_counted(b2s_handle* h, GridIndex* g, const b2s_cloud* cloud) {
+  ProfScope prof(h, PK_GRID);
+  return grid_scan_scatter(h, g, cloud, nullptr);
 }
 
 int32_t grid_build_batch(b2s_handle* h, GridIndex* const* g, const b2s_cloud* const* clouds, int n, double cell) {
diff --git a/open3d_slam_b200/csrc/normals.cu b/open3d_slam_b200/csrc/normals.cu
--- a/open3d_slam_b200/csrc/normals.cu
+++ b/open3d_slam_b200/csrc/normals.cu
@@ -466,15 +466,19 @@
   }
 }
 
+double normals_cell(double radius, double cell_hint) {
+  double cell = cell_hint > 0.0 ? cell_hint : radius / 4.0;
+  if (cell < radius / 16.0) cell = radius / 16.0;
+  return cell;
+}
+
 int32_t op_estimate_normals(b2s_handle* h, b2s_cloud* c, int knn, double radius, double cell_hint, const int32_t* flags, bool with_prior,
-                            const NormalsDebug* dbg) {
+                            const NormalsDebug* dbg, bool index_built) {
   B2S_REQUIRE(radius > 0.0, B2S_E_INVALID, "maxRadiusNormalEstimation_ must be > 0");
   B2S_REQUIRE(knn > 0, B2S_E_INVALID, "knnNormalEstimation_ must be > 0");
   B2S_REQUIRE(knn <= 32, B2S_E_UNSUPPORTED, "knn > 32 is not supported by the register-resident k-best list yet");
   B2S_REQUIRE(!with_prior || c->has_normals, B2S_E_NO_NORMALS, "prior normals requested for a cloud without normals");
-  double cell = cell_hint > 0.0 ? cell_hint : radius / 4.0;
-  if (cell < radius / 16.0) cell = radius / 16.0;
-  B2S_TRY(grid_build(h, &h->grid_b, c, cell, nullptr));
+  if (!index_built) B2S_TRY(grid_build(h, &h->grid_b, c, normals_cell(radius, cell_hint), nullptr));
   const size_t n_max = c->n_max > 0 ? c->n_max : 1;
   B2S_TRY(c->nrm.ensure(n_max * 24, h->stream, with_prior));
   int blocks = (int)((n_max + NK_THREADS - 1) / NK_THREADS);
diff --git a/open3d_slam_b200/csrc/runtime.cu b/open3d_slam_b200/csrc/runtime.cu
--- a/open3d_slam_b200/csrc/runtime.cu
+++ b/open3d_slam_b200/csrc/runtime.cu
@@ -286,34 +286,38 @@
 constexpr int RS_TILE = RS_THREADS * RS_ITEMS;
 constexpr int RS_WARPS = RS_THREADS / 32;
 
-template <typename K>
+__host__ __device__ constexpr int sort_digit_bits(int key_bits) { return key_bits >= 25 && key_bits <= 33 ? 11 : 8; }
+
+template <typename K, int DB>
 __global__ void __launch_bounds__(RS_THREADS) rs_hist_kernel(const K* __restrict__ keys, const int32_t* __restrict__ d_n, int shift,
                                                              int32_t* __restrict__ hist, int nblocks) {
+  constexpr int NB = 1 << DB;
   pdl_wait();
-  __shared__ int s_h[256];
-  s_h[threadIdx.x] = 0;
+  __shared__ int s_h[NB];
+  for (int d = threadIdx.x; d < NB; d += RS_THREADS) s_h[d] = 0;
   __syncthreads();
   const int n = *d_n;
   const int base = blockIdx.x * RS_TILE;
 #pragma unroll
   for (int k = 0; k < RS_ITEMS; k++) {
     int i = base + k * RS_THREADS + threadIdx.x;
-    if (i < n) atomicAdd(&s_h[(int)((keys[i] >> shift) & 0xFF)], 1);
-  }
-  __syncthreads();
-  hist[threadIdx.x * nblocks + blockIdx.x] = s_h[threadIdx.x];
-}
-
-template <typename K>
+    if (i < n) atomicAdd(&s_h[(int)((keys[i] >> shift) & (NB - 1))], 1);
+  }
+  __syncthreads();
+  for (int d = threadIdx.x; d < NB; d += RS_THREADS) hist[d * nblocks + blockIdx.x] = s_h[d];
+}
+
+template <typename K, int DB>
 __global__ void __launch_bounds__(RS_THREADS) rs_scatter_kernel(const K* __restrict__ keys_in, const uint32_t* __restrict__ vals_in,
                                                                 K* __restrict__ keys_out, uint32_t* __restrict__ vals_out,
                                                                 const int32_t* __restrict__ d_n, int shift,
                                                                 const int32_t* __restrict__ offs, int nblocks) {
+  constexpr int NB = 1 << DB;
   pdl_wait();
-  __shared__ int s_cnt[RS_WARPS][256];
-  __shared__ int s_base[256];
+  __shared__ uint16_t s_cnt[RS_WARPS][NB];
+  __shared__ int s_base[NB];
   const int lane = threadIdx.x & 31, warp = threadIdx.x >> 5;
-  for (int i = threadIdx.x; i < RS_WARPS * 256; i += RS_THREADS) (&s_cnt[0][0])[i] = 0;
+  for (int i = threadIdx.x; i < RS_WARPS * NB; i += RS_THREADS) (&s_cnt[0][0])[i] = 0;
   __syncthreads();
   const int n = *d_n;
   const int wbase = blockIdx.x * RS_TILE + warp * 32 * RS_ITEMS;
@@ -324,33 +328,32 @@
     int i = wbase + k * 32 + lane;
     bool valid = i < n;
     key[k] = valid ? keys_in[i] : (K)0;
-    int d = valid ? (int)((key[k] >> shift) & 0xFF) : 256 + lane;
+    int d = valid ? (int)((key[k] >> shift) & (NB - 1)) : NB + lane;
     unsigned peers = __match_any_sync(0xffffffffu, d);
     int prior = valid ? s_cnt[warp][d] : 0;
     __syncwarp();
     lrank[k] = prior + __popc(peers & ((1u << lane) - 1u));
-    if (valid && (peers & ((1u << lane) - 1u)) == 0) s_cnt[warp][d] = prior + __popc(peers);
+    if (valid && (peers & ((1u << lane) - 1u)) == 0) s_cnt[warp][d] = (uint16_t)(prior + __popc(peers));
     __syncwarp();
   }
   __syncthreads();
-  {
-    const int d = threadIdx.x;
-    int run = offs[d * nblocks + blockIdx.x];
-#pragma unroll
-    for (int w = 0; w < RS_WARPS; w++) { int c = s_cnt[w][d]; s_cnt[w][d] = run; run += c; }
+  for (int d = threadIdx.x; d < NB; d += RS_THREADS) {
+    s_base[d] = offs[d * nblocks + blockIdx.x];
+    int run = 0;
+#pragma unroll
+    for (int w = 0; w < RS_WARPS; w++) { int c = s_cnt[w][d]; s_cnt[w][d] = (uint16_t)run; run += c; }
   }
   __syncthreads();
 #pragma unroll
   for (int k = 0; k < RS_ITEMS; k++) {
     int i = wbase + k * 32 + lane;
     if (i < n) {
-      int d = (int)((key[k] >> shift) & 0xFF);
-      int pos = s_cnt[warp][d] + lrank[k];
+      int d = (int)((key[k] >> shift) & (NB - 1));
+      int pos = s_base[d] + s_cnt[warp][d] + lrank[k];
       keys_out[pos] = key[k];
       vals_out[pos] = vals_in[i];
     }
   }
-  (void)s_base;
 }
 
 constexpr int CS_CTAS = 8;
@@ -360,18 +363,31 @@
 constexpr int CS_TILE = CS_THREADS * CS_ITEMS;
 
 template <typename K>
+constexpr size_t cluster_sort_smem(int db) {
+  const size_t cnt = (size_t)CS_WARPS * (1 << db) * 2, stage = (size_t)CS_TILE * (sizeof(K) + 4);
+  return (size_t)(4 * (1 << db) + CS_WARPS) * 4 + (cnt > stage ? cnt : stage);
+}
+
+template <typename K, int DB>
 __global__ void __cluster_dims__(CS_CTAS, 1, 1) __launch_bounds__(CS_THREADS, 1)
     cluster_sort_kernel(K* __restrict__ keys_a, uint32_t* __restrict__ vals_a, K* __restrict__ keys_b, uint32_t* __restrict__ vals_b,
                         const int32_t* __restrict__ d_n, int passes) {
+  constexpr int NB = 1 << DB;
+  constexpr int DPT = NB > CS_THREADS ? NB / CS_THREADS : 1;
+  constexpr int DT = NB / DPT;
   pdl_wait();
   namespace cg = cooperative_groups;
   cg::cluster_group cluster = cg::this_cluster();
   const int rank = (int)cluster.block_rank();
   extern __shared__ int cs_smem[];
   int* s_hist = cs_smem;
-  int* s_base = s_hist + 256;
-  int* s_scan = s_base + 256;
-  int* s_cnt = s_scan + CS_WARPS;
+  int* s_base = s_hist + NB;
+  int* s_shift = s_base + NB;
+  int* s_start = s_shift + NB;
+  int* s_scan = s_start + NB;
+  uint16_t* s_cnt = reinterpret_cast<uint16_t*>(s_scan + CS_WARPS);
+  K* s_key = reinterpret_cast<K*>(s_cnt);
+  uint32_t* s_val = reinterpret_cast<uint32_t*>(s_key + CS_TILE);
   const int tid = threadIdx.x, lane = tid & 31, warp = tid >> 5;
   const int n = *d_n;
   const int tiles_total = (n + CS_TILE - 1) / CS_TILE;
@@ -382,34 +398,41 @@
     const uint32_t* vin = (p & 1) ? vals_b : vals_a;
     K* kout = (p & 1) ? keys_a : keys_b;
     uint32_t* vout = (p & 1) ? vals_a : vals_b;
-    const int shift = 8 * p;
-    if (tid < 256) s_hist[tid] = 0;
+    const int shift = DB * p;
+    for (int d = tid; d < NB; d += CS_THREADS) s_hist[d] = 0;
     __syncthreads();
-    for (int i = lo + tid; i < hi; i += CS_THREADS) atomicAdd(&s_hist[(int)((kin[i] >> shift) & 0xFF)], 1);
+    for (int i = lo + tid; i < hi; i += CS_THREADS) atomicAdd(&s_hist[(int)((kin[i] >> shift) & (NB - 1))], 1);
     cluster.sync();
     {
-      int tot = 0, mine = 0;
-      if (tid < 256) {
-        for (int r = 0; r < CS_CTAS; ++r) {
-          const int c = cluster.map_shared_rank(s_hist, r)[tid];
-          if (r < rank) mine += c;
-          tot += c;
+      int tot[DPT], mine[DPT], sum = 0;
+#pragma unroll
+      for (int j = 0; j < DPT; ++j) {
+        tot[j] = 0; mine[j] = 0;
+        if (tid < DT) {
+#pragma unroll
+          for (int r = 0; r < CS_CTAS; ++r) {
+            const int c = cluster.map_shared_rank(s_hist, r)[tid * DPT + j];
+            if (r < rank) mine[j] += c;
+            tot[j] += c;
+          }
         }
-      }
-      int inc = tot;
+        sum += tot[j];
+      }
+      int inc = sum;
 #pragma unroll
       for (int o = 1; o < 32; o <<= 1) { const int t = __shfl_up_sync(0xffffffffu, inc, o); if (lane >= o) inc += t; }
-      if (lane == 31 && warp < 8) s_scan[warp] = inc;
-      __syncthreads();
-      if (tid < 256) {
-        int woff = 0;
-        for (int w = 0; w < warp; ++w) woff += s_scan[w];
-        s_base[tid] = woff + inc - tot + mine;
+      if (lane == 31 && warp < DT / 32) s_scan[warp] = inc;
+      __syncthreads();
+      if (tid < DT) {
+        int run = inc - sum;
+        for (int w = 0; w < warp; ++w) run += s_scan[w];
+#pragma unroll
+        for (int j = 0; j < DPT; ++j) { s_base[tid * DPT + j] = run + mine[j]; run += tot[j]; }
       }
     }
     __syncthreads();
     for (int t0 = lo; t0 < hi; t0 += CS_TILE) {
-      for (int i = tid; i < CS_WARPS * 256; i += CS_THREADS) s_cnt[i] = 0;
+      for (int i = tid; i < CS_WARPS * NB / 8; i += CS_THREADS) reinterpret_cast<int4*>(s_cnt)[i] = make_int4(0, 0, 0, 0);
       __syncthreads();
       const int wbase = t0 + warp * 32 * CS_ITEMS;
       K key[CS_ITEMS];
@@ -423,30 +446,65 @@
       for (int k = 0; k < CS_ITEMS; k++) {
         const int i = wbase + k * 32 + lane;
         const bool valid = i < hi;
-        const int d = valid ? (int)((key[k] >> shift) & 0xFF) : 256 + lane;
+        const int d = valid ? (int)((key[k] >> shift) & (NB - 1)) : NB + lane;
         const unsigned peers = __match_any_sync(0xffffffffu, d);
-        const int prior = valid ? s_cnt[warp * 256 + d] : 0;
+        const int prior = valid ? s_cnt[warp * NB + d] : 0;
         __syncwarp();
         lrank[k] = prior + __popc(peers & ((1u << lane) - 1u));
-        if (valid && (peers & ((1u << lane) - 1u)) == 0) s_cnt[warp * 256 + d] = prior + __popc(peers);
+        if (valid && (peers & ((1u << lane) - 1u)) == 0) s_cnt[warp * NB + d] = (uint16_t)(prior + __popc(peers));
         __syncwarp();
       }
       __syncthreads();
-      if (tid < 256) {
-        int run = s_base[tid];
-        for (int w = 0; w < CS_WARPS; w++) { const int c = s_cnt[w * 256 + tid]; s_cnt[w * 256 + tid] = run; run += c; }
-        s_base[tid] = run;
+      {
+        int tcnt[DPT], sum = 0;
+#pragma unroll
+        for (int j = 0; j < DPT; ++j) {
+          int run = 0;
+          if (tid < DT) {
+            const int d = tid * DPT + j;
+#pragma unroll
+            for (int w = 0; w < CS_WARPS; w++) { const int c = s_cnt[w * NB + d]; s_cnt[w * NB + d] = (uint16_t)run; run += c; }
+          }
+          tcnt[j] = run;
+          sum += run;
+        }
+        int inc = sum;
+#pragma unroll
+        for (int o = 1; o < 32; o <<= 1) { const int t = __shfl_up_sync(0xffffffffu, inc, o); if (lane >= o) inc += t; }
+        if (lane == 31 && warp < DT / 32) s_scan[warp] = inc;
+        __syncthreads();
+        if (tid < DT) {
+          int start = inc - sum;
+          for (int w = 0; w < warp; ++w) start += s_scan[w];
+#pragma unroll
+          for (int j = 0; j < DPT; ++j) {
+            const int d = tid * DPT + j;
+            s_start[d] = start;
+            s_shift[d] = s_base[d] - start;
+            s_base[d] += tcnt[j];
+            start += tcnt[j];
+          }
+        }
+      }
+      __syncthreads();
+#pragma unroll
+      for (int k = 0; k < CS_ITEMS; k++) {
+        const int d = (int)((key[k] >> shift) & (NB - 1));
+        if (wbase + k * 32 + lane < hi) lrank[k] += s_start[d] + s_cnt[warp * NB + d];
       }
       __syncthreads();
 #pragma unroll
       for (int k = 0; k < CS_ITEMS; k++) {
         const int i = wbase + k * 32 + lane;
-        if (i < hi) {
-          const int d = (int)((key[k] >> shift) & 0xFF);
-          const int pos = s_cnt[warp * 256 + d] + lrank[k];
-          kout[pos] = key[k];
-          vout[pos] = vin[i];
-        }
+        if (i < hi) { s_key[lrank[k]] = key[k]; s_val[lrank[k]] = vin[i]; }
+      }
+      __syncthreads();
+      const int tn = min(CS_TILE, hi - t0);
+      for (int j = tid; j < tn; j += CS_THREADS) {
+        const K kk = s_key[j];
+        const int pos = j + s_shift[(int)((kk >> shift) & (NB - 1))];
+        kout[pos] = kk;
+        vout[pos] = s_val[j];
       }
       __syncthreads();
     }
@@ -455,20 +513,14 @@
   }
 }
 
-static bool g_cs_attr32 = false, g_cs_attr64 = false;
-
-template <typename K>
+template <typename K, int DB>
 static int32_t cluster_sort_impl(b2s_handle* h, K*& keys, uint32_t*& vals, K*& keys_alt, uint32_t*& vals_alt, const int32_t* d_n, int key_bits) {
-  int passes = (key_bits + 7) / 8;
-  if (passes < 1) passes = 1;
-  const size_t smem = (size_t)(256 + 256 + CS_WARPS + CS_WARPS * 256) * sizeof(int);
-  bool& attr = sizeof(K) == 4 ? g_cs_attr32 : g_cs_attr64;
-  if (!attr) {
-    B2S_CUDA(cudaFuncSetAttribute(cluster_sort_kernel<K>, cudaFuncAttributeMaxDynamicSharedMemorySize, (int)smem));
-    attr = true;
-  }
+  const int passes = key_bits > DB ? (key_bits + DB - 1) / DB : 1;
+  constexpr size_t smem = cluster_sort_smem<K>(DB);
+  static const cudaError_t attr = cudaFuncSetAttribute(cluster_sort_kernel<K, DB>, cudaFuncAttributeMaxDynamicSharedMemorySize, (int)smem);
+  B2S_CUDA(attr);
   ProfScope prof(h, PK_SORT);
-  launch_pdl(cluster_sort_kernel<K>, CS_CTAS, CS_THREADS, smem, h->stream, keys, vals, keys_alt, vals_alt, d_n, passes);
+  launch_pdl(cluster_sort_kernel<K, DB>, CS_CTAS, CS_THREADS, smem, h->stream, keys, vals, keys_alt, vals_alt, d_n, passes);
   h->launches++;
   B2S_CUDA(cudaGetLastError());
   if (passes & 1) {
@@ -483,26 +535,26 @@
   return v;
 }
 
-template <typename K>
+template <typename K, int DB>
 static int32_t radix_sort_impl(b2s_handle* h, K*& keys, uint32_t*& vals, K*& keys_alt, uint32_t*& vals_alt, const int32_t* d_n,
                                size_t n_max, int key_bits, VoxelScratch* own) {
-  if (!use_multi_kernel_sort() && n_max <= ((size_t)3 << 18)) return cluster_sort_impl<K>(h, keys, vals, keys_alt, vals_alt, d_n, key_bits);
+  if (!use_multi_kernel_sort() && n_max <= ((size_t)3 << 18)) return cluster_sort_impl<K, DB>(h, keys, vals, keys_alt, vals_alt, d_n, key_bits);
+  constexpr int NB = 1 << DB;
   int nblocks = (int)((n_max + RS_TILE - 1) / RS_TILE);
   if (nblocks < 1) nblocks = 1;
-  size_t hist_n = (size_t)256 * nblocks;
+  size_t hist_n = (size_t)NB * nblocks;
   DevBuf& hb = own ? own->sort_hist : h->sort.hist;
   B2S_TRY(hb.ensure((hist_n + 8) * 4 * 2, h->stream));
   int32_t* hist = hb.as<int32_t>();
   int32_t* offs = hist + ((hist_n + 4) & ~(size_t)3);
-  int passes = (key_bits + 7) / 8;
-  if (passes < 1) passes = 1;
+  const int passes = key_bits > DB ? (key_bits + DB - 1) / DB : 1;
   ProfScope prof(h, PK_SORT);
   for (int p = 0; p < passes; p++) {
-    int shift = 8 * p;
-    launch_pdl(rs_hist_kernel<K>, nblocks, RS_THREADS, 0, h->stream, keys, d_n, shift, hist, nblocks);
+    int shift = DB * p;
+    launch_pdl(rs_hist_kernel<K, DB>, nblocks, RS_THREADS, 0, h->stream, keys, d_n, shift, hist, nblocks);
     h->launches++;
     B2S_TRY(scan_impl(h, hist, offs, nullptr, (int32_t)hist_n, hist_n, nullptr, own ? &own->scan_state : nullptr));
-    launch_pdl(rs_scatter_kernel<K>, nblocks, RS_THREADS, 0, h->stream, keys, vals, keys_alt, vals_alt, d_n, shift, offs, nblocks);
+    launch_pdl(rs_scatter_kernel<K, DB>, nblocks, RS_THREADS, 0, h->stream, keys, vals, keys_alt, vals_alt, d_n, shift, offs, nblocks);
     h->launches++;
     K* tk = keys; keys = keys_alt; keys_alt = tk;
     uint32_t* tv = vals; vals = vals_alt; vals_alt = tv;
@@ -513,11 +565,13 @@
 
 int32_t radix_sort_pairs_u32(b2s_handle* h, uint32_t*& keys, uint32_t*& vals, uint32_t*& keys_alt, uint32_t*& vals_alt,
                              const int32_t* d_n, size_t n_max, int key_bits, VoxelScratch* own) {
-  return radix_sort_impl<uint32_t>(h, keys, vals, keys_alt, vals_alt, d_n, n_max, key_bits, own);
+  if (sort_digit_bits(key_bits) == 11) return radix_sort_impl<uint32_t, 11>(h, keys, vals, keys_alt, vals_alt, d_n, n_max, key_bits, own);
+  return radix_sort_impl<uint32_t, 8>(h, keys, vals, keys_alt, vals_alt, d_n, n_max, key_bits, own);
 }
 int32_t radix_sort_pairs_u64(b2s_handle* h, uint64_t*& keys, uint32_t*& vals, uint64_t*& keys_alt, uint32_t*& vals_alt,
                              const int32_t* d_n, size_t n_max, int key_bits, VoxelScratch* own) {
-  return radix_sort_impl<uint64_t>(h, keys, vals, keys_alt, vals_alt, d_n, n_max, key_bits, own);
-}
-
-}
+  if (sort_digit_bits(key_bits) == 11) return radix_sort_impl<uint64_t, 11>(h, keys, vals, keys_alt, vals_alt, d_n, n_max, key_bits, own);
+  return radix_sort_impl<uint64_t, 8>(h, keys, vals, keys_alt, vals_alt, d_n, n_max, key_bits, own);
+}
+
+}
diff --git a/open3d_slam_b200/csrc/voxel.cu b/open3d_slam_b200/csrc/voxel.cu
--- a/open3d_slam_b200/csrc/voxel.cu
+++ b/open3d_slam_b200/csrc/voxel.cu
@@ -167,16 +167,27 @@
   }
 }
 
+__device__ __forceinline__ int mean_cell(const GridHeader& g, double x, double y, double z) {
+  return (grid_axis_cell(z, g.origin[2], g.inv_cell, g.dims[2]) * g.dims[1] + grid_axis_cell(y, g.origin[1], g.inv_cell, g.dims[1])) * g.dims[0] +
+         grid_axis_cell(x, g.origin[0], g.inv_cell, g.dims[0]);
+}
+
 template <typename K>
 __global__ void __launch_bounds__(VX_THREADS) voxel_mean_kernel(const K* __restrict__ keys, const uint32_t* __restrict__ vals,
                                                                 const int32_t* __restrict__ d_n, const int32_t* __restrict__ head,
                                                                 const int32_t* __restrict__ offs, const double* __restrict__ xyz,
                                                                 const double* __restrict__ nrm, double* __restrict__ oxyz,
                                                                 double* __restrict__ onrm, int32_t* out_n, const int32_t* __restrict__ label,
-                                                                const double* __restrict__ palette, double* __restrict__ ocol) {
+                                                                const double* __restrict__ palette, double* __restrict__ ocol,
+                                                                const GridHeader* __restrict__ ghdr, int32_t* gcounts, int32_t* __restrict__ grank) {
   pdl_wait();
   const int n = *d_n;
   if (blockIdx.x == 0 && threadIdx.x == 0) *out_n = offs[n];
+  __shared__ GridHeader g;
+  if (ghdr) {
+    if (threadIdx.x == 0) g = *ghdr;
+    __syncthreads();
+  }
   for (int j = blockIdx.x * blockDim.x + threadIdx.x; j < n; j += gridDim.x * blockDim.x) {
     if (!head[j]) continue;
     const K k = keys[j];
@@ -197,7 +208,9 @@
     }
     const int o = offs[j];
     const double c = (double)cnt;
-    oxyz[3 * o] = __ddiv_rn(sx, c); oxyz[3 * o + 1] = __ddiv_rn(sy, c); oxyz[3 * o + 2] = __ddiv_rn(sz, c);
+    const double mx = __ddiv_rn(sx, c), my = __ddiv_rn(sy, c), mz = __ddiv_rn(sz, c);
+    oxyz[3 * o] = mx; oxyz[3 * o + 1] = my; oxyz[3 * o + 2] = mz;
+    if (ghdr) grank[o] = (mx == mx && my == my && mz == mz) ? atomicAdd(&gcounts[mean_cell(g, mx, my, mz)], 1) : -1;
     if (nrm) { onrm[3 * o] = __ddiv_rn(nx, c); onrm[3 * o + 1] = __ddiv_rn(ny, c); onrm[3 * o + 2] = __ddiv_rn(nz, c); }
     if (label) { ocol[3 * o] = __ddiv_rn(cr, c); ocol[3 * o + 1] = __ddiv_rn(cg, c); ocol[3 * o + 2] = __ddiv_rn(cb, c); }
   }
@@ -213,7 +226,7 @@
 
 template <typename K>
 static int32_t voxel_impl(b2s_handle* h, const b2s_cloud* in, const CropDev* crop, double voxel, int bits, b2s_cloud* out, VoxelScratch* own,
-                          const int32_t* labels, const double* palette, double* rgb_out) {
+                          const int32_t* labels, const double* palette, double* rgb_out, GridIndex* index, double index_cell) {
   const size_t n_max = in->n_max > 0 ? in->n_max : 1;
   DevBuf& kb = own ? own->keys : h->keys;
   DevBuf& vb = own ? own->vals : h->vals;
@@ -224,6 +237,7 @@
   B2S_TRY(fb.ensure((n_max + 1) * 4, h->stream));
   B2S_TRY(ob.ensure((n_max + 2) * 4, h->stream));
   B2S_TRY(cloud_reserve(h, out, n_max, in->has_normals));
+  if (index) B2S_TRY(grid_begin_counted(h, index, out, index_cell, h->misc.as<unsigned long long>()));
   K* keys = kb.as<K>(); K* keys_alt = keys + n_max;
   uint32_t* vals = vb.as<uint32_t>(); uint32_t* vals_alt = vals + n_max;
   const int32_t* d_n = in->dn.as<int32_t>();
@@ -245,17 +259,23 @@
   launch_pdl(voxel_mean_kernel<K>, blocks, VX_THREADS, 0, h->stream, keys, vals, d_n, fb.as<int32_t>(), ob.as<int32_t>(),
                                                              in->xyz.as<double>(), in->has_normals ? in->nrm.as<double>() : nullptr,
                                                              out->xyz.as<double>(), in->has_normals ? out->nrm.as<double>() : nullptr,
-                                                             out->dn.as<int32_t>(), labels, palette, rgb_out);
+                                                             out->dn.as<int32_t>(), labels, palette, rgb_out,
+                                                             index ? index->hdr.as<GridHeader>() : nullptr,
+                                                             index ? index->cell_start.as<int32_t>() : nullptr,
+                                                             index ? index->rank.as<int32_t>() : nullptr);
   h->launches++;
   out->has_normals = in->has_normals;
   out->n_max = in->n_max;
   out->n_known = -1;
   B2S_CUDA(cudaGetLastError());
+  if (index) B2S_TRY(grid_finish_counted(h, index, out));
   return B2S_OK;
 }
 
 int32_t op_voxel_down_sample(b2s_handle* h, const b2s_cloud* in, const CropDev* crop, double voxel, b2s_cloud* out, int fixed_key_bits,
-                             VoxelScratch* own, const int32_t* labels, const double* palette, double* rgb_out) {
+                             VoxelScratch* own, const int32_t* labels, const double* palette, double* rgb_out, GridIndex* index,
+                             double index_cell) {
+  B2S_REQUIRE(!index || voxel > 0.0, B2S_E_INVALID, "op_voxel_down_sample: an index needs a voxel size > 0");
   if (voxel <= 0.0) {
     if (crop) return op_crop(h, in, *crop, out);
     B2S_TRY(cloud_reserve(h, out, in->n_max, in->has_normals));
@@ -283,8 +303,8 @@
     bits = bits_for(ext, voxel);
   }
   B2S_REQUIRE(bits <= 21, B2S_E_INVALID, "[VoxelDownSample] voxel_size is too small for the extent of the cloud");
-  if (bits <= 10) return voxel_impl<uint32_t>(h, in, crop, voxel, bits, out, own, labels, palette, rgb_out);
-  return voxel_impl<uint64_t>(h, in, crop, voxel, bits, out, own, labels, palette, rgb_out);
+  if (bits <= 10) return voxel_impl<uint32_t>(h, in, crop, voxel, bits, out, own, labels, palette, rgb_out, index, index_cell);
+  return voxel_impl<uint64_t>(h, in, crop, voxel, bits, out, own, labels, palette, rgb_out, index, index_cell);
 }
 
 __device__ __forceinline__ uint32_t select_hash(uint32_t seed, double x, double y, double z) {
```

New measurement: 9361, median of 6. 1.3% higher.
